# chiy48308/audio_feature_extraction

Hardware: AMD Instinct MI355X
Metric: audio frames/sec (sr=22050, n_fft=1024, hop=256, n_mfcc=13) (higher is better)
Workload: dtype f32; 1 GPU; 1000x10s clips @22050 Hz per GPU, frame_length=1024, hop_length=256, n_mfcc=13, n_mels=128, hamming, pre-emphasis 0.97 + trim 30 dB + RMS (BASELINE configs[1]); clips_per_gpu=1000, frames_per_gpu_step=862000, input=HBM-resident float32

## Files before the change

### audio_feature_extraction_amd/_native.py

```python
from __future__ import annotations

import ctypes as C
import weakref
import os
import threading

import numpy as np

_HERE = os.path.dirname(os.path.abspath(__file__))
LIB_PATH = os.environ.get("AFX_LIB") or os.path.join(_HERE, "libafx.so")

AFX_OK = 0
CLIP_OK, CLIP_TOO_SHORT, CLIP_NONFINITE = 0, 1, 2
WINDOW_HAMMING, WINDOW_HANN = 0, 1
FMT_F32, FMT_S16 = 0, 1
MEM_HOST, MEM_DEVICE = 0, 1
FLAG_PREEMPH, FLAG_TRIM = 1, 2
DTW_OK, DTW_NONFINITE, DTW_NO_PATH = 0, 1, 2
DTW_METRICS = {"euclidean": 0, "sqeuclidean": 1, "cosine": 2}
DTW_BACKTRACK, DTW_STORE_D = 1, 2
DTW_MAX_DIM = 128
HPSS_STORE_SPEC = 4
HPSS_BINS = 1025
CHROMA_STORE_HIST = 8
CHROMA_HIST = 102
SMP_U8, SMP_S16, SMP_S24, SMP_S32, SMP_F32, SMP_F64 = range(6)
SMP_KINDS = {"u8": SMP_U8, "s16": SMP_S16, "s24": SMP_S24, "s32": SMP_S32, "f32": SMP_F32, "f64": SMP_F64}
SMP_BYTES = np.array([1, 2, 3, 4, 4, 8], np.int64)
SMP_OF_WAV = {(1, 8): SMP_U8, (1, 16): SMP_S16, (1, 24): SMP_S24, (1, 32): SMP_S32, (3, 32): SMP_F32, (3, 64): SMP_F64}
DECODE_MAX_CHANNELS = 7
K_NAMES = ("trim_blocks", "trim_decide", "frames", "dct", "stats")
K_FRAMES = 2

SYMBOLS = (
    "afx_version", "afx_device_count", "afx_last_error", "afx_init", "afx_destroy",
    "afx_malloc", "afx_free", "afx_host_alloc", "afx_host_free", "afx_memcpy_h2d", "afx_memcpy_d2h", "afx_synchronize",
    "afx_default_params", "afx_plan_create", "afx_plan_destroy", "afx_build_tables", "afx_build_mel_schedule",
    "afx_extract_batch", "afx_extract_submit", "afx_extract_collect", "afx_f0_batch", "afx_zcr_batch", "afx_spectral_batch", "afx_f0_build_tables", "afx_f0_dispatch", "afx_preprocess", "afx_plan_set_timing", "afx_plan_get_timings", "afx_plan_get_intervals",
    "afx_wav_probe", "afx_wav_read_s16", "afx_batch_geometry", "afx_dtw_batch", "afx_hpss_batch",
    "afx_resample_design", "afx_resample_batch", "afx_rfft_host", "afx_wav_read_raw", "afx_decode_batch",
    "afx_chroma_batch", "afx_chroma_filters",
)


class AfxError(RuntimeError):
    pass


class Params(C.Structure):
    _fields_ = [
        ("sr", C.c_int32), ("n_fft", C.c_int32), ("hop", C.c_int32), ("n_mfcc", C.c_int32),
        ("n_mels", C.c_int32), ("window", C.c_int32), ("preemph", C.c_float),
        ("trim_top_db", C.c_float), ("trim_frame", C.c_int32), ("trim_hop", C.c_int32),
        ("top_db", C.c_float), ("amin", C.c_float), ("delta_width", C.c_int32),
        ("reserved", C.c_int32),
        ("fmin", C.c_float), ("fmax", C.c_float), ("htk", C.c_int32), ("lifter", C.c_float),
    ]


_lib = None
_lock = threading.Lock()


def lib() -> C.CDLL:
    global _lib
    if _lib is not None:
        return _lib
    with _lock:
        if _lib is not None:
            return _lib
        if not os.path.exists(LIB_PATH):
            raise AfxError(
                f"{LIB_PATH} not found: build it with `python -c 'import __graft_entry__ as g; g.build()'` "
                "or `make -C audio_feature_extraction_amd/csrc` (no CPU fallback exists)")
        L = C.CDLL(LIB_PATH)
        vp, i32, i64p, f32p, i32p = C.c_void_p, C.c_int, C.POINTER(C.c_int64), C.POINTER(C.c_float), C.POINTER(C.c_int32)
        L.afx_version.restype = i32
        L.afx_device_count.restype = i32
        L.afx_last_error.restype = C.c_char_p
        L.afx_init.argtypes = [i32, C.POINTER(vp)]
        L.afx_destroy.argtypes = [vp]; L.afx_destroy.restype = None
        L.afx_malloc.argtypes = [vp, C.c_size_t, C.POINTER(vp)]
        L.afx_free.argtypes = [vp, vp]
        L.afx_host_alloc.argtypes = [vp, C.c_size_t, C.POINTER(vp)]
        L.afx_host_free.argtypes = [vp, vp]
        L.afx_memcpy_h2d.argtypes = [vp, vp, vp, C.c_size_t]
        L.afx_memcpy_d2h.argtypes = [vp, vp, vp, C.c_size_t]
        L.afx_synchronize.argtypes = [vp]
        L.afx_default_params.argtypes = [C.POINTER(Params)]; L.afx_default_params.restype = None
        L.afx_plan_create.argtypes = [vp, C.POINTER(Params), C.POINTER(vp)]
        L.afx_plan_destroy.argtypes = [vp]; L.afx_plan_destroy.restype = None
        L.afx_build_tables.argtypes = [C.POINTER(Params), vp, vp, vp]
        L.afx_build_mel_schedule.argtypes = [C.POINTER(Params), vp, vp, vp]
        L.afx_extract_batch.argtypes = [vp, vp, i32, i32, vp, vp, i32, i32, vp, vp, vp, vp, vp, vp]
        L.afx_extract_submit.argtypes = [vp, vp, i32, i32, vp, vp, i32, i32, vp, vp, vp, vp, vp, vp]
        L.afx_extract_collect.argtypes = [vp]
        L.afx_f0_batch.argtypes = [vp, vp, i32, i32, vp, vp, i32, i32, C.c_double, C.c_double, vp, vp, vp, vp]
        L.afx_zcr_batch.argtypes = [vp, vp, i32, i32, vp, vp, i32, i32, vp, vp, vp]
        L.afx_spectral_batch.argtypes = [vp, vp, i32, i32, vp, vp, i32, i32, vp, vp, vp]
        L.afx_f0_build_tables.argtypes = [i32, i32, i32, C.c_double, C.c_double, vp, vp, vp, vp]
        L.afx_f0_dispatch.argtypes = [i32, i32, i32, C.c_double, C.c_double, vp]
        L.afx_preprocess.argtypes = [vp, vp, C.c_int64, vp, i64p, i64p, i32p]
        L.afx_plan_set_timing.argtypes = [vp, i32]
        L.afx_plan_get_timings.argtypes = [vp, vp, vp, i32]
        L.afx_plan_get_intervals.argtypes = [vp, i32, vp, vp, i32, i32p]
        L.afx_batch_geometry.argtypes = [C.POINTER(Params), vp, vp, i32, vp, vp]
        L.afx_wav_probe.argtypes = [vp, i32, i32, vp, vp, vp, vp]
        L.afx_wav_read_s16.argtypes = [vp, i32, i32, vp, vp, vp, C.c_int64, vp, vp]
        L.afx_dtw_batch.argtypes = [vp, vp, i32, vp, vp, vp, vp, vp, i32, i32, i32, vp, vp, vp, vp, vp, vp, vp]
        L.afx_hpss_batch.argtypes = [vp, vp, i32, i32, vp, vp, i32, i32, vp, vp, vp, vp, vp, vp]
        if hasattr(L, "afx_resample_batch"):
            L.afx_resample_design.argtypes = [i32, i32, vp, vp]
            L.afx_resample_batch.argtypes = [vp, vp, i32, i32, vp, vp, i32, i32, i32, vp, i32, vp, i32, vp, vp]
        if hasattr(L, "afx_decode_batch"):
            L.afx_wav_read_raw.argtypes = [vp, i32, i32, vp, vp, vp, C.c_int64, vp, vp]
            L.afx_decode_batch.argtypes = [vp, vp, i32, vp, vp, vp, vp, i32, vp, i32, vp]
        if hasattr(L, "afx_chroma_batch"):
            L.afx_chroma_batch.argtypes = [vp, vp, i32, i32, vp, vp, i32, i32, vp, vp, vp, vp, vp, vp, vp, vp, vp]
            L.afx_chroma_filters.argtypes = [i32, C.c_double, vp]
        if hasattr(L, "afx_rfft_host"):
            L.afx_rfft_host.argtypes = [i32, vp, vp]
        _lib = L
    return _lib


def _path_array(paths):
    arr = (C.c_char_p * len(paths))()
    arr[:] = [os.fsencode(p) for p in paths]
    return arr


def wav_probe(paths, threads: int = 16) -> dict:
    n = len(paths)
    info = np.zeros((n, 4), np.int32)
    frames, off, status = np.zeros(n, np.int64), np.zeros(n, np.int64), np.zeros(n, np.int32)
    if n:
        arr = _path_array(paths)
        _check(lib().afx_wav_probe(arr, n, int(threads), info.ctypes.data, frames.ctypes.data, off.ctypes.data,
                                   status.ctypes.data), "afx_wav_probe")
    return {"tag": info[:, 0], "channels": info[:, 1], "rate": info[:, 2], "bits": info[:, 3],
            "frames": frames, "data_off": off, "status": status}


def wav_read_s16(paths, data_off, frames, out: np.ndarray, offsets, threads: int = 16) -> np.ndarray:
    n = len(paths)
    status = np.zeros(n, np.int32)
    if n:
        if out.dtype != np.int16 or not out.flags.c_contiguous:
            raise ValueError("out must be C-contiguous int16")
        data_off = np.ascontiguousarray(data_off, np.int64)
        frames = np.ascontiguousarray(frames, np.int64)
        offsets = np.ascontiguousarray(offsets, np.int64)
        arr = _path_array(paths)
        _check(lib().afx_wav_read_s16(arr, n, int(threads), data_off.ctypes.data, frames.ctypes.data, out.ctypes.data,
                                      int(out.size), offsets.ctypes.data, status.ctypes.data), "afx_wav_read_s16")
    return status


def wav_read_raw(paths, data_off, nbytes, out: np.ndarray, offsets, threads: int = 16) -> np.ndarray:
    n = len(paths)
    status = np.zeros(n, np.int32)
    if not hasattr(lib(), "afx_wav_read_raw"):
        raise NotImplementedError("this libafx has no afx_wav_read_raw")
    if n:
        if out.dtype != np.uint8 or not out.flags.c_contiguous:
            raise ValueError("out must be C-contiguous uint8")
        data_off = np.ascontiguousarray(data_off, np.int64)
        nbytes = np.ascontiguousarray(nbytes, np.int64)
        offsets = np.ascontiguousarray(offsets, np.int64)
        if not (data_off.shape[0] == nbytes.shape[0] == offsets.shape[0] == n):
            raise ValueError("data_off, nbytes and offsets must have one entry per file")
        arr = _path_array(paths)
        _check(lib().afx_wav_read_raw(arr, n, int(threads), data_off.ctypes.data, nbytes.ctypes.data, out.ctypes.data,
                                      int(out.size), offsets.ctypes.data, status.ctypes.data), "afx_wav_read_raw")
    return status


def wav_sample_kinds(probe: dict) -> np.ndarray:
    kinds = np.full(probe["status"].shape[0], -1, np.int32)
    for (tag, bits), k in SMP_OF_WAV.items():
        kinds[(probe["tag"] == tag) & (probe["bits"] == bits)] = k
    kinds[(probe["status"] != 0) | (probe["channels"] < 1) | (probe["channels"] > DECODE_MAX_CHANNELS) | (probe["rate"] <= 0)] = -1
    return kinds


def batch_geometry(p: "Params", offsets, lengths) -> dict:
    offsets = np.ascontiguousarray(offsets, np.int64)
    lengths = np.ascontiguousarray(lengths, np.int64)
    n = int(offsets.shape[0])
    rec = np.zeros((max(n, 1), 4), np.int64)
    tot = np.zeros(4, np.int64)
    _check(lib().afx_batch_geometry(C.byref(p), offsets.ctypes.data, lengths.ctypes.data, n, rec.ctypes.data, tot.ctypes.data),
           "afx_batch_geometry")
    rec = rec[:n]
    return {"frame_base": rec[:, 0], "tmax": rec[:, 1], "tpad": rec[:, 2], "blk_base": rec[:, 3],
            "frame_slots": int(tot[0]), "blocks": int(tot[1]), "trim_blocks": int(tot[2]), "max_tmax": int(tot[3])}


def f0_build_tables(sr: int, n_fft: int, hop: int, fmin: float, fmax: float) -> dict:
    info = np.zeros(8, np.int32)
    _check(lib().afx_f0_build_tables(sr, n_fft, hop, fmin, fmax, info.ctypes.data, None, None, None), "afx_f0_build_tables")
    band, nb = int(info[3]), int(info[2])
    w = 2 * band + 1
    beta, lt, freqs = np.zeros(100), np.zeros(2 * w * w), np.zeros(nb)
    _check(lib().afx_f0_build_tables(sr, n_fft, hop, fmin, fmax, info.ctypes.data, beta.ctypes.data, lt.ctypes.data,
                                     freqs.ctypes.data), "afx_f0_build_tables")
    keys = ("min_period", "max_period", "n_bins", "band", "cap", "n_lag", "R", "slots")
    return {**{k: int(v) for k, v in zip(keys, info)}, "beta": beta, "lt": lt.reshape(2, w, w), "freqs": freqs}


F0_DISPATCH_KEYS = ("energy_lpw", "epb", "yin_n", "yin_fpb", "yin_sh", "vit_nbt", "vit_bandt", "vit_tpt", "bt_depth",
                    "band", "n_bins", "yin_lds")


def f0_dispatch(sr: int, n_fft: int, hop: int, fmin: float, fmax: float) -> dict:
    out = np.zeros(len(F0_DISPATCH_KEYS), np.int32)
    _check(lib().afx_f0_dispatch(int(sr), int(n_fft), int(hop), float(fmin), float(fmax), out.ctypes.data), "afx_f0_dispatch")
    return {k: int(v) for k, v in zip(F0_DISPATCH_KEYS, out)}


def resample_design(sr_in: int, sr_out: int) -> dict:
    info = np.zeros(4, np.int32)
    _check(lib().afx_resample_design(int(sr_in), int(sr_out), info.ctypes.data, None), "afx_resample_design")
    taps = np.zeros(int(info[2]), np.float64)
    _check(lib().afx_resample_design(int(sr_in), int(sr_out), info.ctypes.data, taps.ctypes.data), "afx_resample_design")
    return {"up": int(info[0]), "down": int(info[1]), "n_taps": int(info[2]), "half": int(info[3]), "taps": taps}


def rfft_host(x) -> np.ndarray:
    x = np.ascontiguousarray(x, np.float32).reshape(-1)
    out = np.zeros(2 * (x.size // 2 + 1), np.float32)
    _check(lib().afx_rfft_host(int(x.size), x.ctypes.data, out.ctypes.data), "afx_rfft_host")
    return out.view(np.complex64)


def chroma_filters(sr: int, tuning: float = 0.0) -> np.ndarray:
    if not hasattr(lib(), "afx_chroma_filters"):
        raise NotImplementedError("this libafx has no afx_chroma_filters")
    out = np.zeros((12, HPSS_BINS), np.float32)
    _check(lib().afx_chroma_filters(int(sr), float(tuning), out.ctypes.data), "afx_chroma_filters")
    return out


def resample_lengths(lengths, sr_in: int, sr_out: int) -> np.ndarray:
    sr_in = np.asarray(sr_in, np.int64)
    g = np.gcd(sr_in, int(sr_out))
    up, down = int(sr_out) // g, sr_in // g
    return (np.asarray(lengths, np.int64) * up + down - 1) // down


def _check(rc: int, what: str):
    if rc != AFX_OK:
        msg = lib().afx_last_error().decode("utf-8", "replace")
        if rc == -5:
            raise NotImplementedError(f"{what}: {msg}")
        if rc == -1:
            raise ValueError(f"{what}: {msg}")
        raise AfxError(f"{what} failed ({rc}): {msg}")


def device_count() -> int:
    return int(lib().afx_device_count())


def _ptr(a):
    return None if a is None else a.ctypes.data


def packed_offsets(counts, align: int = 1) -> np.ndarray:
    counts = np.asarray(counts, np.int64).reshape(-1)
    if align > 1:
        counts = (counts + (align - 1)) // align * align
    out = np.zeros(counts.shape[0], np.int64)
    if counts.shape[0] > 1:
        np.cumsum(counts[:-1], out=out[1:])
    return out


def _clip_arrays(offsets, lengths):
    offsets = np.ascontiguousarray(offsets, np.int64).reshape(-1)
    lengths = np.ascontiguousarray(lengths, np.int64).reshape(-1)
    n = int(offsets.shape[0])
    if lengths.shape[0] != n:
        raise ValueError("offsets and lengths must have one entry per clip")
    return offsets, lengths, n


def _sample_fmt(samples, fmt):
    if fmt is not None:
        return fmt
    if isinstance(samples, np.ndarray):
        return FMT_S16 if samples.dtype == np.int16 else FMT_F32
    raise ValueError("fmt is required for device-resident samples")


def _sample_source(samples, fmt, offsets, lengths, mem=None):
    if mem is None:
        mem = MEM_HOST if isinstance(samples, np.ndarray) else MEM_DEVICE
    if mem != MEM_HOST:
        return (samples.ptr if isinstance(samples, DeviceBuffer) else int(samples)), MEM_DEVICE
    want = np.int16 if fmt == FMT_S16 else np.float32
# ... 449 lines not shown
```

### audio_feature_extraction_amd/csrc/afx_api.cpp

```cpp
#include <algorithm>
#include <cmath>
#include <cstdio>
#include <cstdlib>
#include <cstring>
#include <atomic>
#include <mutex>
#include <string>
#include <vector>

#include <hip/hip_runtime.h>

#include "afx_device.h"
#include "afx_devenv.h"
#include "afx_frames3.h"
#include "afx_internal.h"
#include "afx_plan.h"

namespace afx {
DevEnv::DevEnv() {
  if (const char* v = getenv("AFX_DEBUG_SKIP")) debug_skip = atoi(v) & 127;
  if (const char* v = getenv("AFX_F0_DEBUG")) f0_debug = atoi(v);
  stamps = getenv("AFX_DEBUG_STAMPS") != nullptr;
  f3_debug = getenv("AFX_F3_DEBUG") != nullptr;
  no_spec = getenv("AFX_NO_SPEC") != nullptr;
  no_tickets = getenv("AFX_NO_TICKETS") != nullptr;
  no_frames3 = getenv("AFX_NO_FRAMES3") != nullptr;
  no_frames3s = getenv("AFX_NO_FRAMES3S") != nullptr;
  no_frames3d = getenv("AFX_NO_FRAMES3D") != nullptr;
  f3_generic_mel = getenv("AFX_F3_GENERIC_MEL") != nullptr;
  no_dct16l = getenv("AFX_NO_DCT16L") != nullptr;
  host_blocks = getenv("AFX_HOST_BLOCKS") != nullptr;
  no_fused_tail = getenv("AFX_NO_FUSED_TAIL") != nullptr;
  if (const char* v = getenv("AFX_F3_WAVES")) f3_waves = atoi(v);
  if (const char* v = getenv("AFX_TAIL_MODE")) tail_mode = atoi(v);
  if (const char* v = getenv("AFX_TAIL_SKIP")) tail_skip = atoi(v) & 7;
  if (const char* v = getenv("AFX_TEST_CHUNK_CLIPS")) chunk_clips = std::max(1, std::min(32768, atoi(v)));
  if (const char* v = getenv("AFX_TEST_F0_CHUNK_FRAMES")) f0_chunk_frames = std::max<int64_t>(64, atoll(v));
  if (const char* v = getenv("AFX_TEST_DTW_BUDGET")) dtw_budget = std::max<int64_t>(1, atoll(v));
  if (const char* v = getenv("AFX_TEST_HPSS_BUDGET")) hpss_budget = std::max<int64_t>(1, atoll(v));
  if (const char* v = getenv("AFX_TEST_CHROMA_BUDGET")) chroma_budget = std::max<int64_t>(1, atoll(v));
  f0_dump = getenv("AFX_F0_DUMP");
}
const DevEnv& dev_env() { static const DevEnv e; return e; }
}

extern "C" int afx_device_count(void) {
  int n = 0;
  if (hipGetDeviceCount(&n) != hipSuccess) return 0;
  return n;
}

extern "C" int afx_init(int device, afx_ctx** out) {
  if (!out) { set_error("afx_init: null out"); return AFX_ERR_INVALID; }
  *out = nullptr;
  int n = afx_device_count();
  if (n <= 0) { set_error("no HIP device visible"); return AFX_ERR_NO_DEVICE; }
  if (device < 0 || device >= n) { set_error("device index out of range"); return AFX_ERR_INVALID; }
  HIP_TRY(hipSetDevice(device));
  afx_ctx* c = new afx_ctx();
  c->device = device;
  hipError_t e = hipStreamCreateWithFlags(&c->stream, hipStreamNonBlocking);
  if (e != hipSuccess) { delete c; set_error(std::string("hipStreamCreate: ") + hipGetErrorString(e)); return AFX_ERR_HIP; }
  *out = c;
  return AFX_OK;
}

extern "C" void afx_destroy(afx_ctx* ctx) {
  if (!ctx) return;
  (void)hipSetDevice(ctx->device);
  for (DevBuf* b : {&ctx->dtw_raw, &ctx->dtw_feats, &ctx->dtw_norms, &ctx->dtw_pairs, &ctx->dtw_codes, &ctx->dtw_rows, &ctx->dtw_d,
                    &ctx->dtw_path, &ctx->dtw_cost, &ctx->dtw_status, &ctx->dtw_len, &ctx->rs_g, &ctx->rs_tstart, &ctx->rs_clips,
                    &ctx->rs_in, &ctx->rs_out, &ctx->dc_clips, &ctx->dc_in, &ctx->dc_out})
    release(*b);
  if (ctx->stream) (void)hipStreamDestroy(ctx->stream);
  delete ctx;
}

extern "C" int afx_malloc(afx_ctx* ctx, size_t bytes, void** out) {
  if (!ctx || !out) { set_error("afx_malloc: null argument"); return AFX_ERR_INVALID; }
  HIP_TRY(hipSetDevice(ctx->device));
  hipError_t e = hipMalloc(out, bytes ? bytes : 1);
  if (e != hipSuccess) { set_error(std::string("hipMalloc: ") + hipGetErrorString(e)); return e == hipErrorOutOfMemory ? AFX_ERR_NOMEM : AFX_ERR_HIP; }
  return AFX_OK;
}

extern "C" int afx_free(afx_ctx* ctx, void* d) {
  if (!ctx) { set_error("afx_free: null ctx"); return AFX_ERR_INVALID; }
  HIP_TRY(hipSetDevice(ctx->device));
  if (d) HIP_TRY(hipFree(d));
  return AFX_OK;
}

extern "C" int afx_host_alloc(afx_ctx* ctx, size_t bytes, void** out) {
  if (!ctx || !out) { set_error("afx_host_alloc: null argument"); return AFX_ERR_INVALID; }
  *out = nullptr;
  HIP_TRY(hipSetDevice(ctx->device));
  hipError_t e = hipHostMalloc(out, bytes ? bytes : 1, hipHostMallocPortable);
  if (e != hipSuccess) { set_error(std::string("hipHostMalloc: ") + hipGetErrorString(e)); *out = nullptr; return e == hipErrorOutOfMemory ? AFX_ERR_NOMEM : AFX_ERR_HIP; }
  return AFX_OK;
}

extern "C" int afx_host_free(afx_ctx* ctx, void* h) {
  if (!ctx) { set_error("afx_host_free: null ctx"); return AFX_ERR_INVALID; }
  HIP_TRY(hipSetDevice(ctx->device));
  if (h) HIP_TRY(hipHostFree(h));
  return AFX_OK;
}

extern "C" int afx_memcpy_h2d(afx_ctx* ctx, void* dst, const void* src, size_t bytes) {
  if (!ctx || (!dst && bytes) || (!src && bytes)) { set_error("afx_memcpy_h2d: null argument"); return AFX_ERR_INVALID; }
  HIP_TRY(hipSetDevice(ctx->device));
  HIP_TRY(hipMemcpyAsync(dst, src, bytes, hipMemcpyHostToDevice, ctx->stream));
  HIP_TRY(hipStreamSynchronize(ctx->stream));
  return AFX_OK;
}

// ... 148 lines not shown

static int device_ref(afx_plan* pl, hipEvent_t* out) {
  std::lock_guard<std::mutex> lk(g_ref_mu);
  const int d = pl->device;
  if (d < 0 || d >= 64) { set_error("device index out of range for timing"); return AFX_ERR_INVALID; }
  if (!g_ref_set[d]) {
    HIP_TRY(hipEventCreate(&g_ref[d]));
    HIP_TRY(hipEventRecord(g_ref[d], pl->ctx->stream));
    HIP_TRY(hipEventSynchronize(g_ref[d]));
    g_ref_set[d] = true;
  }
  *out = g_ref[d];
  return AFX_OK;
}

extern "C" int afx_plan_set_timing(afx_plan* pl, int enable) {
  if (!pl) { set_error("afx_plan_set_timing: null plan"); return AFX_ERR_INVALID; }
  HIP_TRY(hipSetDevice(pl->device));
  if (enable) { hipEvent_t r; int rc = device_ref(pl, &r); if (rc != AFX_OK) return rc; }
  if (enable && !pl->ev_ready) {
    for (int k = 0; k < AFX_K_COUNT; ++k) { HIP_TRY(hipEventCreate(&pl->ev[k][0])); HIP_TRY(hipEventCreate(&pl->ev[k][1])); }
    pl->ev_ready = true;
  }
  pl->timing = enable != 0;
  pl->timing_frames_only = enable == 2;
  return AFX_OK;
}

extern "C" int afx_plan_get_timings(afx_plan* pl, float* ms, int32_t* launches, int reset) {
  if (!pl) { set_error("afx_plan_get_timings: null plan"); return AFX_ERR_INVALID; }
  for (int k = 0; k < AFX_K_COUNT; ++k) {
    if (ms) ms[k] = (float)pl->ms_sum[k];
    if (launches) launches[k] = pl->launches[k];
    if (reset) { pl->ms_sum[k] = 0.0; pl->launches[k] = 0; pl->spans[k].clear(); }
  }
  return AFX_OK;
}

extern "C" int afx_plan_get_intervals(afx_plan* pl, int slot, double* start_ms, double* end_ms, int cap, int32_t* count) {
  if (!pl || slot < 0 || slot >= AFX_K_COUNT || cap < 0 || !count) { set_error("afx_plan_get_intervals: invalid argument"); return AFX_ERR_INVALID; }
  const auto& v = pl->spans[slot];
  const int n = (int)std::min<size_t>(v.size(), (size_t)cap);
  for (int i = 0; i < n; ++i) {
    if (start_ms) start_ms[i] = v[v.size() - n + i].first;
    if (end_ms) end_ms[i] = v[v.size() - n + i].second;
  }
  *count = (int32_t)v.size();
  return AFX_OK;
}

int prepare_descriptors(afx_plan* pl, const int64_t* offsets, const int64_t* lengths, int n) {
  const bool same = (int)pl->c_len.size() == n &&
                    std::memcmp(pl->c_len.data(), lengths, n * sizeof(int64_t)) == 0 &&
                    std::memcmp(pl->c_off.data(), offsets, n * sizeof(int64_t)) == 0;
  if (same) return AFX_OK;
  const int hop = pl->p.hop, th = pl->p.trim_hop;
  pl->h_clips.resize(n);
  BatchGeom g;
  {
    std::string why;
    if (!build_clip_descs(hop, th, offsets, lengths, n, pl->h_clips.data(), g, why)) { set_error(why); return AFX_ERR_INVALID; }
  }
  const int64_t nblk = g.nblocks;
  pl->total_tpad = g.total_tpad; pl->total_tblk = g.total_tblk; pl->max_tblocks = g.max_tblocks; pl->max_tmax = g.max_tmax;
  pl->nblocks = g.nblocks;
  int rc;
  if ((rc = ensure(pl->clips, n * sizeof(ClipDesc))) != AFX_OK) return rc;
  if ((rc = ensure(pl->blocks, std::max<size_t>((size_t)nblk, 1) * sizeof(BlockDesc))) != AFX_OK) return rc;
  hipStream_t s = pl->ctx->stream;
  if (pl->clips_ev_pending) { HIP_TRY(hipEventSynchronize(pl->clips_ev)); pl->clips_ev_pending = false; }
  if (pl->h_clips_pin_cap < (size_t)n) {
    if (pl->h_clips_pin) (void)hipHostFree(pl->h_clips_pin);
    pl->h_clips_pin = nullptr; pl->h_clips_pin_cap = 0;
    const size_t want = (size_t)n + (size_t)n / 4 + 64;
    HIP_TRY(hipHostMalloc((void**)&pl->h_clips_pin, want * sizeof(ClipDesc), hipHostMallocDefault));
    pl->h_clips_pin_cap = want;
  }
  if (!pl->clips_ev) HIP_TRY(hipEventCreateWithFlags(&pl->clips_ev, hipEventDisableTiming));
  std::memcpy(pl->h_clips_pin, pl->h_clips.data(), (size_t)n * sizeof(ClipDesc));
  HIP_TRY(hipMemcpyAsync(pl->clips.p, pl->h_clips_pin, n * sizeof(ClipDesc), hipMemcpyHostToDevice, s));
  HIP_TRY(hipEventRecord(pl->clips_ev, s));
  pl->clips_ev_pending = true;
  if (pl->use_f3) {
    const size_t nb_alloc = (size_t)std::max<int64_t>(nblk, 1);
    if ((rc = ensure(pl->blocks_spec, nb_alloc * sizeof(BlockDesc))) != AFX_OK) return rc;
    if ((rc = ensure(pl->blockmax, nb_alloc * sizeof(float))) != AFX_OK) return rc;
    if ((rc = ensure(pl->items, (size_t)n * kF3ItemsPerClip * sizeof(BlockDesc))) != AFX_OK) return rc;
    if ((rc = ensure(pl->n_items, 16)) != AFX_OK) return rc;
    if (!dev_env().host_blocks) {
      HIP_TRY(launch_build_blocks3(s, (const ClipDesc*)pl->clips.p, n, (int)nblk, (BlockDesc*)pl->blocks_spec.p, pl->kp));
    } else {
      const int per = pl->kp.rms_sub, half = pl->p.n_fft / 2;
      pl->h_blocks.resize(nb_alloc);
      for (int i = 0; i < n; ++i) {
        const ClipDesc& c = pl->h_clips[i];
        const int64_t ntb = (c.len + th - 1) / th;
        for (int b = 0; b < c.tpad / kFramesPerBlock; ++b) {
          const int64_t gs = (int64_t)b * kFramesPerBlock * hop - half;
          const int t0 = b * kFramesPerBlock;
          pl->h_blocks[(size_t)c.blk_base + b] = make_block(c, i, gs, t0, 0, c.len, c.len, t0, c.tmax, c.len >= 2 && t0 < c.tmax,
                                                            (int32_t)(c.tblk_base * per), (int32_t)(ntb * per));
        }
      }
      HIP_TRY(hipMemcpyAsync(pl->blocks_spec.p, pl->h_blocks.data(), pl->h_blocks.size() * sizeof(BlockDesc), hipMemcpyHostToDevice, s));
      HIP_TRY(hipStreamSynchronize(s));
    }
  }
  pl->c_off.assign(offsets, offsets + n);
  pl->c_len.assign(lengths, lengths + n);
  return AFX_OK;
}

int null_arg(const char* who) {
  set_error(std::string(who) + ": null/invalid argument");
  return AFX_ERR_INVALID;
}

int check_sample_format(const char* who, int sample_fmt, int mem_kind) {
  if (sample_fmt != AFX_FMT_F32 && sample_fmt != AFX_FMT_S16) { set_error(std::string(who) + ": unknown sample format"); return AFX_ERR_INVALID; }
  if (mem_kind != AFX_MEM_HOST && mem_kind != AFX_MEM_DEVICE) { set_error(std::string(who) + ": unknown mem_kind"); return AFX_ERR_INVALID; }
  return AFX_OK;
}

int check_batch_args(const char* who, afx_plan* pl, const void* samples, int sample_fmt, int mem_kind,
                     const int64_t* offsets, const int64_t* lengths, int n_clips, bool empty_ok) {
  const bool need = n_clips > 0 || !empty_ok;
  if (!pl || n_clips < 0 || (need && (!offsets || !lengths)) || (!samples && n_clips > 0)) return null_arg(who);
  return check_sample_format(who, sample_fmt, mem_kind);
}

int check_clip_ranges(const char* who, const int64_t* offsets, const int64_t* lengths, const int64_t* out_offsets, int n_clips,
                      int64_t max_off) {
  for (int i = 0; i < n_clips; ++i) {
    if (offsets[i] < 0 || lengths[i] < 0 || offsets[i] > max_off || (out_offsets && (out_offsets[i] < 0 || out_offsets[i] > max_off))) {
      set_error(std::string(who) + ": clip " + std::to_string(i) + ": offsets and lengths must be >= 0");
      return AFX_ERR_INVALID;
    }
    if (lengths[i] > ((int64_t)1 << 31)) {
      set_error(std::string(who) + ": clip " + std::to_string(i) + ": more than 2^31 samples is not supported");
      return AFX_ERR_UNSUPPORTED;
    }
  }
  return AFX_OK;
}

int begin_plan_call(const char* who, afx_plan* pl) {
  (void)hipGetLastError();
  HIP_TRY(hipSetDevice(pl->device));
  if (pl->pend.active) { set_error(std::string(who) + ": the plan has a submitted batch that has not been collected"); return AFX_ERR_INVALID; }
  return AFX_OK;
}

int stage_samples(afx_plan* pl, DevBuf& buf, const void* samples, int sample_fmt, int mem_kind, const int64_t* offsets,
                  const int64_t* lengths, int n, const void** d_samples) {
  *d_samples = samples;
  if (mem_kind != AFX_MEM_HOST) return AFX_OK;
  const size_t esz = sample_fmt == AFX_FMT_S16 ? 2 : 4;
  int64_t hi = 0;
  for (int i = 0; i < n; ++i) hi = std::max(hi, offsets[i] + lengths[i]);
  int rc;
  if ((rc = ensure(buf, (size_t)hi * esz + 16)) != AFX_OK) return rc;
  if (hi > 0) HIP_TRY(hipMemcpyAsync(buf.p, samples, (size_t)hi * esz, hipMemcpyHostToDevice, pl->ctx->stream));
  *d_samples = buf.p;
  return AFX_OK;
}

int run_preprocess(afx_plan* pl, const void* d_samples, int n, const KParams& kp, bool f0_prep) {
  hipStream_t s = pl->ctx->stream;
  int64_t hi = 0, max_len = 0;
  for (int i = 0; i < n; ++i) { hi = std::max(hi, pl->c_off[i] + pl->c_len[i]); max_len = std::max(max_len, pl->c_len[i]); }
  int rc;
  if ((rc = ensure(pl->info, n * sizeof(ClipInfo))) != AFX_OK) return rc;
  if ((rc = ensure(pl->bsum, std::max<int64_t>(pl->total_tblk, 1) * 4 * sizeof(float))) != AFX_OK) return rc;
  if (f0_prep && (rc = ensure(pl->f0_ysig, (size_t)std::max<int64_t>(hi, 1) * sizeof(float))) != AFX_OK) return rc;
  const ClipDesc* d_clips = (const ClipDesc*)pl->clips.p;
  ClipInfo* d_info = (ClipInfo*)pl->info.p;
  HIP_TRY(hipMemsetAsync(d_info, 0, n * sizeof(ClipInfo), s));
  pl->info_clean_n = 0;
  HIP_TRY(launch_trim_blocks(s, d_samples, d_clips, d_info, (float*)pl->bsum.p, n, pl->max_tblocks, kp));
  HIP_TRY(launch_trim_decide(s, d_clips, d_info, (const float*)pl->bsum.p, (BlockDesc*)pl->blocks.p, nullptr, n, kp));
  if (f0_prep) HIP_TRY(launch_f0_prep(s, d_samples, d_clips, d_info, (float*)pl->f0_ysig.p, n, max_len, kp));
  return AFX_OK;
}

int rebase_offsets(const afx_plan* pl, const char* what, const int64_t* offs, int n, int64_t per_frame,
                   std::vector<int64_t>& rebased, int64_t* lo, int64_t* hi) {
// ... 8 lines not shown
  return AFX_OK;
}

int upload_frame_range(afx_plan* pl, const int64_t* rebased, int n, DevBuf& d_offs, DevBuf& out, size_t bytes, int fill) {
  hipStream_t s = pl->ctx->stream;
  int rc;
  if ((rc = ensure(out, bytes)) != AFX_OK) return rc;
  if ((rc = ensure(d_offs, n * sizeof(int64_t))) != AFX_OK) return rc;
  HIP_TRY(hipMemcpyAsync(d_offs.p, rebased, n * sizeof(int64_t), hipMemcpyHostToDevice, s));
  HIP_TRY(hipMemsetAsync(out.p, fill, bytes, s));
  return AFX_OK;
}

int run_spectral(afx_plan* pl, const void* d_signal, int n, const KParams& kp, const int64_t* h_offsets, size_t count,
                 const SpecBands& sb) {
  hipStream_t s = pl->ctx->stream;
  int rc;
  if ((rc = ensure(pl->info, n * sizeof(ClipInfo))) != AFX_OK) return rc;
  if ((rc = upload_frame_range(pl, h_offsets, n, pl->frame_offs, pl->frames, count * sizeof(float), 0)) != AFX_OK) return rc;
  HIP_TRY(hipMemsetAsync(pl->info.p, 0, n * sizeof(ClipInfo), s));
  pl->info_clean_n = 0;
  if (pl->nblocks > 0)
    HIP_TRY(launch_spectral(s, d_signal, (ClipInfo*)pl->info.p, (const BlockDesc*)pl->blocks_spec.p, pl->nblocks, pl->f3, kp,
                            (float*)pl->frames.p, (const int64_t*)pl->frame_offs.p, sb, pl->n_cu));
  return AFX_OK;
}

int statuses_from_info(afx_plan* pl, int n, int32_t* out_status) {
  hipStream_t s = pl->ctx->stream;
  std::vector<ClipInfo> h_info(n);
  HIP_TRY(hipMemcpyAsync(h_info.data(), pl->info.p, n * sizeof(ClipInfo), hipMemcpyDeviceToHost, s));
  HIP_TRY(hipStreamSynchronize(s));
  for (int i = 0; i < n; ++i) out_status[i] = h_info[i].nonfinite ? AFX_CLIP_NONFINITE : AFX_CLIP_OK;
  return AFX_OK;
}

#define TIMED(slot, call)                                                      \
  do {                                                                         \
    const bool timed_ = pl->timing && (!pl->timing_frames_only || (slot) == AFX_K_FRAMES);   \
    if (timed_) HIP_TRY(hipEventRecord(pl->ev[slot][0], s));                   \
    HIP_TRY(call);                                                             \
    if (timed_) { HIP_TRY(hipEventRecord(pl->ev[slot][1], s)); pl->launches[slot]++; } \
  } while (0)

static int chunk_enqueue(afx_plan* pl, const void* samples, int fmt, int mem_kind,
                         const int64_t* offsets, const int64_t* lengths, int n, int flags,
                         float* out_stats, int32_t* out_status, int64_t* out_trim, int32_t* out_nframes,
                         float* out_frames, const int64_t* frame_offsets, bool by_event) {
  hipStream_t s = pl->ctx->stream;
  if (pl->pend.active) { set_error("the plan has a submitted batch that has not been collected (afx_extract_collect)"); return AFX_ERR_INVALID; }
  const int K = pl->p.n_mfcc, M = pl->p.n_mels;
  const int nstat = 4 * K + 3;
  int rc;
  if ((rc = prepare_descriptors(pl, offsets, lengths, n)) != AFX_OK) return rc;

  const void* d_samples = nullptr;
  if ((rc = stage_samples(pl, pl->samples, samples, fmt, mem_kind, offsets, lengths, n, &d_samples)) != AFX_OK) return rc;
  {
    const size_t before = pl->info.cap;
    if ((rc = ensure(pl->info, n * sizeof(ClipInfo))) != AFX_OK) return rc;
    if (pl->info.cap != before) pl->info_clean_n = 0;
  }
  if ((rc = ensure(pl->bsum, std::max<int64_t>(pl->total_tblk, 1) * 4 * sizeof(float))) != AFX_OK) return rc;
  if ((rc = ensure(pl->logmel, (size_t)(pl->total_tpad + kFramesPerBlock) * M * sizeof(float))) != AFX_OK) return rc;
  if ((rc = ensure(pl->rms, (size_t)pl->total_tpad * sizeof(float))) != AFX_OK) return rc;
  if ((rc = ensure(pl->mfcc, (size_t)pl->total_tpad * K * sizeof(float))) != AFX_OK) return rc;
  float* d_frames = nullptr;
  int64_t f_lo = 0, f_hi = 0;
  if (out_frames) {
    if (!frame_offsets) { set_error("out_frames given without frame_offsets"); return AFX_ERR_INVALID; }
    if ((rc = rebase_offsets(pl, "frame", frame_offsets, n, 3 * K + 1, pl->h_rebased, &f_lo, &f_hi)) != AFX_OK) return rc;
    if ((rc = upload_frame_range(pl, pl->h_rebased.data(), n, pl->frame_offs, pl->frames, (size_t)(f_hi - f_lo) * sizeof(float), 0)) != AFX_OK) return rc;
    d_frames = (float*)pl->frames.p;
  }

  KParams kp = pl->kp;
  kp.flags = flags; kp.fmt = fmt;
  kp.flags |= dev_env().debug_skip << 8;
  const ClipDesc* d_clips = (const ClipDesc*)pl->clips.p;
  ClipInfo* d_info = (ClipInfo*)pl->info.p;

  {
    const size_t before = pl->n_items.cap;
    if ((rc = ensure(pl->n_items, 16)) != AFX_OK) return rc;
    if (pl->n_items.cap != before) pl->info_clean_n = 0;
  }
  if (pl->info_clean_n < n) {
    HIP_TRY(hipMemsetAsync(d_info, 0, n * sizeof(ClipInfo), s));
    HIP_TRY(hipMemsetAsync(pl->n_items.p, 0, 16, s));
  }
  pl->info_clean_n = 0;
  const bool want_stamps = dev_env().stamps && !frames_mr_shape(kp.n_fft);
  const bool f3 = pl->use_f3 && !want_stamps && (!(kp.flags & 0x7f00) || dev_env().f3_debug);
  bool no_spec = dev_env().no_spec;
  if (f3 && no_spec && kp.rms_sub > 1 && kp.trim_hop / kp.rms_sub != 256) no_spec = false;
  if (!f3) kp.rms_sub = 0;
  const bool fused_tail = f3 && pl->nblocks > 0 && !out_frames && !dev_env().no_fused_tail && tail_eligible(kp, pl->dt) &&
                          (n >= 32 || pl->max_tmax <= 2048);
  const F3Launch f3l{s, d_samples, d_info, pl->f3, kp, (float*)pl->logmel.p, pl->n_cu};
  if (f3 && !no_spec && pl->nblocks > 0) {
    const int max_items = n * kF3ItemsPerClip;
    F3Launch spec = f3l;
    spec.blocks = (const BlockDesc*)pl->blocks_spec.p; spec.nblocks = pl->nblocks; spec.spec = true;
    spec.blockmax = (float*)pl->blockmax.p; spec.bsum = (float*)pl->bsum.p;
    spec.work_ctr = dev_env().no_tickets ? nullptr : (int*)pl->n_items.p + 1;
    TIMED(AFX_K_FRAMES, launch_frames3_any(spec));
    TIMED(AFX_K_TRIM_DECIDE, launch_trim_decide3(s, d_clips, d_info, (const float*)pl->bsum.p, (const float*)pl->blockmax.p,
                                                 (BlockDesc*)pl->items.p, (int*)pl->n_items.p, max_items, (float*)pl->rms.p, n, kp));
    F3Launch redo = f3l;
    redo.blocks = (const BlockDesc*)pl->items.p; redo.nblocks = max_items; redo.nblocks_dev = (const int*)pl->n_items.p;
    TIMED(AFX_K_TRIM_BLOCKS, launch_frames3_any(redo));
    if (!fused_tail)
      TIMED(AFX_K_DCT, launch_dct(s, d_clips, d_info, pl->dt, kp, (const float*)pl->logmel.p, (float*)pl->mfcc.p, n, pl->max_tmax, true, true));
  } else {
  TIMED(AFX_K_TRIM_BLOCKS, launch_trim_blocks(s, d_samples, d_clips, d_info, (float*)pl->bsum.p, n, pl->max_tblocks, kp));
  TIMED(AFX_K_TRIM_DECIDE, launch_trim_decide(s, d_clips, d_info, (const float*)pl->bsum.p, (BlockDesc*)pl->blocks.p, (float*)pl->rms.p, n, kp, d_samples));
  if (pl->nblocks > 0) {
    const int grid = std::min(pl->nblocks, pl->n_cu * 2);
    unsigned long long* d_stamps = nullptr;
    if (want_stamps) {
      if ((rc = ensure(pl->stamps, (size_t)grid * kWaves * kStampPhases * 8)) != AFX_OK) return rc;
      d_stamps = (unsigned long long*)pl->stamps.p;
      HIP_TRY(hipMemsetAsync(d_stamps, 0, (size_t)grid * kWaves * kStampPhases * 8, s));
    }
    if (f3) {
      F3Launch all = f3l;
      all.blocks = (const BlockDesc*)pl->blocks.p; all.nblocks = pl->nblocks;
      TIMED(AFX_K_FRAMES, launch_frames3_any(all));
    }
    else if (frames_mr_shape(kp.n_fft))
      TIMED(AFX_K_FRAMES, launch_frames_mr(s, d_samples, d_info, (const BlockDesc*)pl->blocks.p, pl->nblocks,
                                           pl->dt, kp, (float*)pl->logmel.p, (float*)pl->rms.p, grid));
    else
      TIMED(AFX_K_FRAMES, launch_frames(s, d_samples, d_info, (const BlockDesc*)pl->blocks.p, pl->nblocks,
                                        pl->dt, kp, (float*)pl->logmel.p, (float*)pl->rms.p, grid, d_stamps));
    if (want_stamps) {
      std::vector<unsigned long long> h((size_t)grid * kWaves * kStampPhases);
      HIP_TRY(hipMemcpyAsync(h.data(), d_stamps, h.size() * 8, hipMemcpyDeviceToHost, s));
      HIP_TRY(hipStreamSynchronize(s));
      static const char* names[kStampPhases] = {"stage", "bar1", "fft", "prefetch", "bar2", "mel", "bar3", "melfin", "x0", "x1", "x2", "x3"};
      double tot[kStampPhases] = {}, wv[kWaves][kStampPhases] = {};
      for (int g = 0; g < grid; ++g)
        for (int w = 0; w < kWaves; ++w)
          for (int ph = 0; ph < kStampPhases; ++ph) {
            const double v = (double)h[((size_t)g * kWaves + w) * kStampPhases + ph];
            tot[ph] += v; wv[w][ph] += v;
          }
      const double per = (double)pl->nblocks * kWaves;
      fprintf(stderr, "[afx stamps] cycles per block (avg over waves):");
      double all = 0;
      for (int ph = 0; ph < kStampPhases; ++ph) { fprintf(stderr, " %s=%.0f", names[ph], tot[ph] / per); all += tot[ph] / per; }
      fprintf(stderr, " total=%.0f\n", all);
      for (int w = 0; w < kWaves; ++w) {
        fprintf(stderr, "[afx stamps]   wave %d:", w);
        for (int ph = 0; ph < kStampPhases; ++ph) fprintf(stderr, " %s=%.0f", names[ph], wv[w][ph] / pl->nblocks);
        fprintf(stderr, "\n");
      }
    }
    if (!fused_tail)
      TIMED(AFX_K_DCT, launch_dct(s, d_clips, d_info, pl->dt, kp, (const float*)pl->logmel.p, (float*)pl->mfcc.p, n, pl->max_tmax, f3));
  }
  }
  const int tail_spec = (f3 && !no_spec) ? 1 : 0;
  const size_t stats_bytes = (size_t)n * nstat * sizeof(float), info_bytes = (size_t)n * sizeof(ClipInfo);
  if (pl->h_pin_cap < stats_bytes + info_bytes) {
    HIP_TRY(hipStreamSynchronize(s));
    if (pl->h_pin) (void)hipHostFree(pl->h_pin);
    pl->h_pin = nullptr; pl->h_pin_cap = 0; pl->h_pin_dev = nullptr;
    const size_t want = (stats_bytes + info_bytes) * 5 / 4 + 256;
    HIP_TRY(hipHostMalloc(&pl->h_pin, want, hipHostMallocMapped));
    HIP_TRY(hipHostGetDevicePointer(&pl->h_pin_dev, pl->h_pin, 0));
    pl->h_pin_cap = want;
  }
  const size_t info_at = (stats_bytes + 15) & ~(size_t)15;
  if (fused_tail)
    TIMED(AFX_K_DCT, launch_tail(s, d_clips, d_info, pl->dt, kp, (const float*)pl->logmel.p, (const float*)pl->rms.p,
                                 (float*)pl->h_pin_dev, (ClipInfo*)((char*)pl->h_pin_dev + info_at), n, tail_spec, pl->n_cu));
  else
  TIMED(AFX_K_STATS, launch_stats(s, d_clips, d_info, kp, (const float*)pl->mfcc.p, (const float*)pl->rms.p,
                                  (float*)pl->h_pin_dev, d_frames, (const int64_t*)pl->frame_offs.p, n,
                                  (ClipInfo*)((char*)pl->h_pin_dev + info_at)));
  if (out_frames && f_hi > f_lo)
    HIP_TRY(hipMemcpyAsync(out_frames + f_lo, d_frames, (size_t)(f_hi - f_lo) * sizeof(float), hipMemcpyDeviceToHost, s));
  if (by_event) {
    if (!pl->done) HIP_TRY(hipEventCreateWithFlags(&pl->done, hipEventDisableTiming));
    if (!pl->flag) {
      void* h = nullptr;
      HIP_TRY(hipHostMalloc(&h, 64, hipHostMallocMapped));
      std::memset(h, 0, 64);
      pl->flag = (volatile unsigned*)h;
      HIP_TRY(hipHostGetDevicePointer((void**)&pl->flag_dev, h, 0));
    }
  }
  HIP_TRY(launch_finish(s, d_info, n, (int*)pl->n_items.p, by_event ? pl->flag_dev : nullptr, by_event ? ++pl->seq : 0u));
  pl->info_clean_n = n;
  if (by_event) HIP_TRY(hipEventRecord(pl->done, s));
  pl->pend.active = true; pl->pend.n = n; pl->pend.stats_bytes = stats_bytes;
  pl->pend.out_stats = out_stats; pl->pend.out_status = out_status; pl->pend.out_trim = out_trim; pl->pend.out_nframes = out_nframes;
  return AFX_OK;
}

static int chunk_finish(afx_plan* pl, bool by_event) {
  if (!pl->pend.active) { set_error("afx_extract_collect: nothing submitted"); return AFX_ERR_INVALID; }
  hipStream_t s = pl->ctx->stream;
  pl->pend.active = false;
  if (by_event) {
    for (unsigned it = 1; *pl->flag != pl->seq; ++it) {
      if ((it & 0xfff) == 0) {
        const hipError_t q = hipEventQuery(pl->done);
        if (q == hipSuccess) break;
        if (q != hipErrorNotReady) { set_error(std::string("afx_extract_collect: ") + hipGetErrorString(q)); return AFX_ERR_HIP; }
      }
#if defined(__x86_64__)
      __builtin_ia32_pause();
#endif
    }
    std::atomic_thread_fence(std::memory_order_acquire);
  } else {
    HIP_TRY(hipStreamSynchronize(s));
  }
  const int n = pl->pend.n;
  const size_t stats_bytes = pl->pend.stats_bytes;
  float* out_stats = pl->pend.out_stats; int32_t* out_status = pl->pend.out_status;
  int64_t* out_trim = pl->pend.out_trim; int32_t* out_nframes = pl->pend.out_nframes;
  const float* h_stats = (const float*)pl->h_pin;
  const ClipInfo* h_info = (const ClipInfo*)((char*)pl->h_pin + ((stats_bytes + 15) & ~(size_t)15));
  if (pl->timing) {
    for (int k = 0; k < AFX_K_COUNT; ++k) {
      if (pl->nblocks == 0 && (k == AFX_K_FRAMES || k == AFX_K_DCT)) continue;
      if (pl->launches[k] == 0) continue;
      float ms = 0.f, t0 = 0.f;
      if (hipEventElapsedTime(&ms, pl->ev[k][0], pl->ev[k][1]) == hipSuccess) {
        pl->ms_sum[k] += ms;
        hipEvent_t ref;
        if (device_ref(pl, &ref) == AFX_OK && hipEventElapsedTime(&t0, ref, pl->ev[k][0]) == hipSuccess) {
          if (pl->spans[k].size() >= kMaxSpans) pl->spans[k].erase(pl->spans[k].begin(), pl->spans[k].begin() + kMaxSpans / 2);
          pl->spans[k].emplace_back((double)t0, (double)t0 + (double)ms);
        }
      }
    }
  }
  std::memcpy(out_stats, h_stats, stats_bytes);
  for (int i = 0; i < n; ++i) {
    const ClipInfo& ci = h_info[i];
    out_status[i] = ci.status;
    if (out_trim) { out_trim[2 * i] = ci.start; out_trim[2 * i + 1] = ci.end; }
    if (out_nframes) out_nframes[i] = ci.T;
  }
  return AFX_OK;
}

static int extract_chunk(afx_plan* pl, const void* samples, int fmt, int mem_kind,
                         const int64_t* offsets, const int64_t* lengths, int n, int flags,
                         float* out_stats, int32_t* out_status, int64_t* out_trim, int32_t* out_nframes,
                         float* out_frames, const int64_t* frame_offsets) {
  int rc = chunk_enqueue(pl, samples, fmt, mem_kind, offsets, lengths, n, flags, out_stats, out_status, out_trim, out_nframes,
                         out_frames, frame_offsets, false);
  if (rc != AFX_OK) return rc;
  return chunk_finish(pl, false);
}

extern "C" int afx_extract_submit(afx_plan* pl, const void* samples, int sample_fmt, int mem_kind,
                                  const int64_t* offsets, const int64_t* lengths, int n_clips, int flags,
                                  float* out_stats, int32_t* out_status, int64_t* out_trim,
                                  int32_t* out_nframes, float* out_frames, const int64_t* frame_offsets) {
  if (!out_stats || !out_status) return null_arg("afx_extract_submit");
  int rc = check_batch_args("afx_extract_submit", pl, samples, sample_fmt, mem_kind, offsets, lengths, n_clips);
  if (rc != AFX_OK) return rc;
  if (n_clips == 0) { set_error("afx_extract_submit: empty batch"); return AFX_ERR_INVALID; }
  if (n_clips > dev_env().chunk_clips) { set_error("afx_extract_submit: more clips than one chunk holds; use afx_extract_batch"); return AFX_ERR_UNSUPPORTED; }
  if (pl->pend.active) { set_error("afx_extract_submit: the plan's previous batch has not been collected"); return AFX_ERR_INVALID; }
  (void)hipGetLastError();
  HIP_TRY(hipSetDevice(pl->device));
  rc = chunk_enqueue(pl, samples, sample_fmt, mem_kind, offsets, lengths, n_clips, flags, out_stats, out_status, out_trim,
                     out_nframes, out_frames, frame_offsets, true);
  return rc;
}
// ... 31 lines not shown
```

### audio_feature_extraction_amd/csrc/afx_devenv.h

```cpp
#pragma once
#include <cstdint>

namespace afx {

struct DevEnv {
  int debug_skip = 0, f0_debug = 0;
  bool stamps = false, f3_debug = false, no_spec = false, no_tickets = false;
  bool no_frames3 = false, no_frames3s = false, no_frames3d = false;
  bool f3_generic_mel = false;
  bool no_dct16l = false;
  bool host_blocks = false;
  bool no_fused_tail = false;
  int tail_mode = 0;
  int tail_skip = 0;
  int f3_waves = 0;
  int chunk_clips = 32768;
  int64_t f0_chunk_frames = 1280 * 1024;
  int64_t dtw_budget = (int64_t)2 << 30;
  int64_t hpss_budget = (int64_t)2 << 30;
  int64_t chroma_budget = (int64_t)2 << 30;
  const char* f0_dump = nullptr;
  DevEnv();
};
const DevEnv& dev_env();

}
```

### audio_feature_extraction_amd/csrc/afx_device.h

```cpp
#pragma once
#include <cstddef>
#include <cstdint>

#include <hip/hip_runtime_api.h>

#include "afx.h"
#include "afx_consts.h"

namespace afx {

constexpr int kFramesPerBlock = 16;
constexpr int kWaves = 4;

struct ClipDesc {
  int64_t off;
  int64_t len;
  int64_t frame_base;
  int64_t tblk_base;
  int32_t tmax;
  int32_t tpad;
  int32_t blk_base;
  int32_t pad_;
};

// ... 13 lines not shown
__host__ __device__ inline BlockDesc make_block(const ClipDesc& cd, int clip, int64_t gs, int64_t frame, int64_t start,
                                                int64_t end, int64_t N, int t0, int T, bool active, int32_t bsum_base,
                                                int32_t bsum_n) {
  const int64_t lim = (int64_t)1 << 30;
  auto rel = [&](int64_t x) { const int64_t r = x - gs; return (int32_t)(r < -lim ? -lim : (r > lim ? lim : r)); };
  BlockDesc d;
  d.sample_base = cd.off + gs; d.frame_slot = cd.frame_base + frame; d.clip_off = cd.off;
  d.keep_lo = rel(start); d.keep_hi = rel(end);
  d.have_lo = rel(0); d.have_hi = rel(N);
  d.clip = clip; d.t0 = t0; d.T = T;
  d.active = active ? 1 : 0;
  d.bsum_base = bsum_base; d.bsum_n = bsum_n;
  return d;
}

struct ClipInfo {
  int64_t start, end;
  int32_t T;
  int32_t status;
  uint32_t lmax_ord;
  uint32_t nonfinite;
};

struct DevTables {
  const float* window;
  const float* tw;
  const float* post;
  const float4* mel_coef;
  const float* mel_koff;
  const int4* mel_grp;
  const int4* mel_items;
  int32_t mel_item_cnt[4];
  int32_t mel_n_slots;
  const float* dctA;
  const float* dctP;
  const float* dctS;
  int32_t n_groups;
  int32_t n_cgroups;
};

struct KParams {
  int32_t n_fft, hop, n_mels, n_mfcc;
  int32_t trim_frame, trim_hop;
  float preemph_b1;
  float trim_top_db, top_db, amin;
  int32_t flags;
  int32_t fmt;
  int32_t rms_sub;
};

template <typename K>
inline hipError_t set_lds_limit(K kernel, size_t bytes) {
  return hipFuncSetAttribute(reinterpret_cast<const void*>(kernel), hipFuncAttributeMaxDynamicSharedMemorySize, (int)bytes);
}
template <auto Kernel>
inline hipError_t allow_lds_once() {
  static bool done[64] = {};
  int dev = 0;
  hipError_t e = hipGetDevice(&dev);
  if (e != hipSuccess) return e;
  if (dev < 0 || dev >= 64 || done[dev]) return hipSuccess;
  if ((e = set_lds_limit(Kernel, 160 * 1024)) == hipSuccess) done[dev] = true;
  return e;
}

size_t frames_lds_bytes(int n_fft, int hop);

hipError_t launch_trim_blocks(hipStream_t s, const void* samples, const ClipDesc* clips, ClipInfo* info,
                              float* bsum, int n_clips, int max_tblocks, const KParams& kp);
hipError_t launch_trim_decide(hipStream_t s, const ClipDesc* clips, ClipInfo* info, const float* bsum,
                              BlockDesc* blocks, float* rms_rows, int n_clips, const KParams& kp,
                              const void* samples = nullptr);
hipError_t launch_frames(hipStream_t s, const void* samples, ClipInfo* info,
                         const BlockDesc* blocks, int nblocks, const DevTables& tb, const KParams& kp,
                         float* logmel, float* rms_rows, int grid, unsigned long long* stamps = nullptr);
constexpr int kStampPhases = 12;
bool frames_mr_shape(int n_fft);
size_t frames_mr_lds_bytes(int n_fft, int hop);
hipError_t launch_frames_mr(hipStream_t s, const void* samples, ClipInfo* info, const BlockDesc* blocks, int nblocks,
                            const DevTables& tb, const KParams& kp, float* logmel, float* rms_rows, int grid);
hipError_t launch_dct(hipStream_t s, const ClipDesc* clips, const ClipInfo* info, const DevTables& tb,
                      const KParams& kp, const float* logmel, float* mfcc, int n_clips, int max_tmax,
                      bool frame_major = false, bool spec = false);
hipError_t launch_finish(hipStream_t s, ClipInfo* info, int n_clips, int* counters, unsigned* flag_dev, unsigned seq);
hipError_t launch_stats(hipStream_t s, const ClipDesc* clips, const ClipInfo* info, const KParams& kp,
                        const float* mfcc, const float* rms_rows, float* stats, float* frames_out,
                        const int64_t* frame_offsets, int n_clips, ClipInfo* info_out = nullptr);
hipError_t launch_preemph(hipStream_t s, const float* y, float* out, int64_t n, float b1);
bool tail_eligible(const KParams& kp, const DevTables& tb);
hipError_t launch_tail(hipStream_t s, const ClipDesc* clips, const ClipInfo* info, const DevTables& tb, const KParams& kp,
                       const float* logmel, const float* rms_rows, float* stats, ClipInfo* info_out, int n_clips, int spec,
                       int n_cu);

}
```

### audio_feature_extraction_amd/csrc/afx_frames3.h

```cpp
#pragma once
#include <cstdint>
#include <vector>

#include <hip/hip_runtime_api.h>

#include "afx_device.h"

namespace afx {

constexpr int kF3ExFloats = 2176;
constexpr int kF3TabFloats = 2048;
constexpr int kF3MaxRounds = 8;
constexpr int kF3KernelRounds = 4;
constexpr int kF3MaxBatches = 8;

struct HostF3Mel {
  int32_t rounds = 0;
  int32_t nb[kF3MaxRounds] = {};
  int32_t width[kF3MaxRounds] = {};
  int32_t woff[kF3MaxRounds] = {};
  std::vector<float> w;
  std::vector<int32_t> meta;
  bool usable = false;
};

struct F3Tables {
  const float* window;
  const float* w1024;
  const float* w2048;
  const float* mel_w;
  const int32_t* mel_meta;
  int32_t mel_rounds;
  int32_t mel_wfloats;
  int32_t mel_all_own;
  int32_t mel_own_w1;
  uint32_t mel_rp[kF3MaxRounds];
};

void build_f3_mel(const std::vector<float>& mel_dense, int n_mels, int n_bins, int max_slot, int lanes, int align, HostF3Mel& out);

size_t frames3_lds_bytes(int waves, const F3Tables& ft);
bool frames3_eligible(const KParams& kp, const F3Tables& ft);
int frames3_waves(const F3Tables& ft);
struct F3Launch {
  hipStream_t s;
  const void* samples;
  ClipInfo* info;
  const F3Tables& ft;
  const KParams& kp;
  float* logmel;
  int n_cu;
  const BlockDesc* blocks = nullptr;
  int nblocks = 0;
  const int* nblocks_dev = nullptr;
  float* blockmax = nullptr;
  float* bsum = nullptr;
  bool spec = false;
  int* work_ctr = nullptr;
};
inline int f3_grid(const F3Launch& L, int waves) {
  const int want = (L.nblocks + waves - 1) / waves;
  return want < 1 ? 1 : (want < L.n_cu ? want : L.n_cu);
}
size_t frames3s_lds_bytes(int waves, const F3Tables& ft);
size_t frames3d_lds_bytes(int waves, const F3Tables& ft);
hipError_t launch_frames3(const F3Launch& L);
hipError_t launch_frames3s(const F3Launch& L);
hipError_t launch_frames3d(const F3Launch& L);
hipError_t launch_frames3_any(const F3Launch& L);
struct SpecBands {
  int32_t lo[8], hi[8], cnt[8];
  float hz_per_bin, roll_percent;
};
constexpr int kSpecFloats = 17;
hipError_t launch_spectral(hipStream_t s, const void* samples, ClipInfo* info, const BlockDesc* blocks, int nblocks,
                           const F3Tables& ft, const KParams& kp, float* desc_out, const int64_t* desc_offs,
                           const SpecBands& sb, int n_cu);
hipError_t launch_build_blocks3(hipStream_t s, const ClipDesc* clips, int n_clips, int nblocks, BlockDesc* blocks,
                                const KParams& kp);
constexpr int kF3ItemsPerClip = 6;
hipError_t launch_trim_decide3(hipStream_t s, const ClipDesc* clips, ClipInfo* info, const float* bsum, const float* blockmax,
                               BlockDesc* items, int* n_items, int max_items, float* rms_rows, int n_clips, const KParams& kp);

}
```

### audio_feature_extraction_amd/csrc/afx_frames3.hip

```cpp
#include <hip/hip_runtime.h>

#include <cstdlib>
#include <type_traits>

#include "afx_device.h"
#include "afx_devenv.h"
#include "afx_frames3.h"
#include "afx_frames3_dev.h"

namespace afx {

size_t frames3_lds_bytes(int waves, const F3Tables& ft) {
  return (size_t)(waves * kF3ExFloats + kF3TabFloats + ft.mel_wfloats + ft.mel_rounds * 64 + 1024) * sizeof(float);
}

#ifdef AFX_F3_DEBUG
__device__ unsigned long long g_f3_stamps[4 * 8192];
__device__ unsigned long long g_f3_blk[65536];
#endif

template <int FMT, int WAVES, int NB0, int NB1, bool SPEC>
__global__ __launch_bounds__(WAVES * 64) void k_frames3(const void* __restrict__ samples,
                                                        ClipInfo* __restrict__ info,
                                                        const BlockDesc* __restrict__ blocks, int nblocks,
                                                        const int* __restrict__ nblocks_dev,
                                                        F3Tables ft, KParams kp,
                                                        float* __restrict__ logmel,
                                                        float* __restrict__ blockmax,
                                                        float* __restrict__ bsum,
                                                        int* __restrict__ work_ctr) {
  constexpr int N = 1024, HOP = 256;
  extern __shared__ __attribute__((aligned(16))) float smem[];
  if (nblocks_dev) {
    nblocks = *nblocks_dev;
    if (nblocks <= 0) return;
  }
  const int tid = threadIdx.x, lane = tid & 63;
  const int wave = __builtin_amdgcn_readfirstlane(tid >> 6);
#ifdef AFX_F3_DEBUG
  const unsigned long long stamp0 = wall_clock64();
#endif
  float* const tabs = smem + WAVES * kF3ExFloats;
  float4* const T2q = reinterpret_cast<float4*>(tabs);
  float4* const T3q = reinterpret_cast<float4*>(tabs + 256);
  const int mel_wfloats = NB0 > 0 ? (NB0 + NB1) * 256 : ft.mel_wfloats;
  const int mel_rounds = NB0 > 0 ? 2 : ft.mel_rounds;
  float* const MW = tabs + kF3TabFloats;
  int* const MM = reinterpret_cast<int*>(MW + mel_wfloats);
  v2* const E = reinterpret_cast<v2*>(smem + wave * kF3ExFloats);
  float* const XB = reinterpret_cast<float*>(E);

  {
    const v2* w1024 = reinterpret_cast<const v2*>(ft.w1024);
    auto W = [&](int m) { const v2 v = w1024[m & 511]; return (m & 512) ? -v : v; };
    if (tid < 64) {
      const int rr = tid >> 4, c = tid & 15;
      const v2 a = W(8 * (2 * rr) * c), b = W(8 * (2 * rr + 1) * c);
      T2q[tid] = float4{a.x, a.y, b.x, b.y};
      const int jbt = tid ? 128 - tid : 64;
#pragma unroll
      for (int r = 1; r < 8; ++r) { const v2 ta = W(tid * r), tb = W(jbt * r); T3q[(r - 1) * 64 + tid] = float4{ta.x, ta.y, tb.x, tb.y}; }
    }
    for (int i = tid; i < mel_wfloats; i += WAVES * 64) MW[i] = ft.mel_w[i];
    for (int i = tid; i < mel_rounds * 64; i += WAVES * 64) MM[i] = ft.mel_meta[i];
    for (int i = lane; i < kF3ExFloats; i += 64) XB[i] = 0.f;
  }
  float4* const WT = reinterpret_cast<float4*>(MM + mel_rounds * 64);
  if (tid < 64) {
    float wreg[16];
#pragma unroll
    for (int u = 0; u < 16; ++u) wreg[u] = 0.5f * ft.window[u < 8 ? lane + 64 * u : (64 - lane) + 64 * (15 - u)];
#pragma unroll
    for (int v = 0; v < 4; ++v) WT[v * 64 + lane] = float4{wreg[4 * v], wreg[4 * v + 1], wreg[4 * v + 2], wreg[4 * v + 3]};
  }
  __syncthreads();
  const v2 H = {0.70710678118654752440f, 0.70710678118654752440f};
  const v2 W1 = {0.92387953251128675613f, -0.38268343236508977173f};
  const v2 W3 = {0.38268343236508977173f, -0.92387953251128675613f};
  const bool pre = (kp.flags & AFX_FLAG_PREEMPH) != 0;
  const float b1 = pre ? kp.preemph_b1 : 0.f;
  const int M = kp.n_mels;
  const int jb = lane ? 128 - lane : 64;
  v2* const e1w = E + lane;
  const v2* const e1r = E + 66 * (lane & 15) + (lane >> 4);
  v2* const e2w = E + 128 * (lane >> 4) + (lane & 15);
  v2* const ea = E + lane;
  v2* const eb = E + jb;

  using sample_t = sample_of<FMT>;
  const int n_rounds = mel_rounds;
  const int meta0 = MM[lane], meta1 = MM[64 + lane];
  const unsigned mf0 = (meta0 >> 11) & 511, mf1 = (meta1 >> 11) & 511;
  const float amin = kp.amin;

  float bs = 0.f;
  unsigned long long bsmask = 0;
  auto sub2 = [&](float x, float y, int idx, unsigned long long two) -> bool {
    const float m = f3_sum2(x, y);
    const unsigned long long sel = two << idx;
    bs = f3_sel(bs, m, sel);
    bsmask |= sel;
    return __any(!(fabsf(m) < INFINITY));
  };
  auto flag_nonfinite = [&](const BlockDesc& bd, bool bad_rows) {
    if (__any(bad_rows) && lane == 0) atomicOr(&info[bd.clip].nonfinite, 1u);
  };
  auto sub_store = [&](const BlockDesc& bd) {
    const int j = bd.t0 + lane;
    if (((bsmask >> lane) & 1) && j < bd.bsum_n) bsum[bd.bsum_base + j] = bs;
    bsmask = 0;
  };

  const int total_waves = gridDim.x * WAVES, wg = blockIdx.x * WAVES + wave;
#ifdef AFX_F3_DEBUG
  const unsigned long long stamp1 = wall_clock64();
#endif
  F3Runs runs = f3_runs_init(work_ctr, nblocks, total_waves, wg, true);
  do {
  const int b_hi = runs.b_hi;
  for (int b = runs.b_lo; b < b_hi; ++b) {
    BlockDesc bd = blocks[b];
    if (!bd.active) continue;
    bool first = true;
    v2 Ra[8], Rb[8];
    for (;;) {
    const int Tleft = bd.T - bd.t0;
    const int npairs = Tleft >= 16 ? 8 : (Tleft + 1) >> 1;
    bool chain = false;
    if (SPEC && npairs == 8 && b + 1 < b_hi) {
      const BlockDesc* nx = blocks + b + 1;
      chain = nx->active && nx->clip == bd.clip && nx->t0 == bd.t0 + 16;
    }
    const int64_t sbase = bd.sample_base;
    const sample_t* const sp = (const sample_t*)samples + sbase;
    auto interior = [&](int j0, int j1) -> bool {
      return (j0 - 1 >= bd.have_lo) && (j1 <= bd.have_hi) && (j0 >= bd.keep_lo) && (j1 <= bd.keep_hi);
    };
    auto interior_r = [&](int j0, int j1) -> bool {
      const BlockDesc& r = blocks[f3_opaque(b)];
      return (j0 - 1 >= r.have_lo) && (j1 <= r.have_hi) && (j0 >= r.keep_lo) && (j1 <= r.keep_hi);
    };
    auto edge_sample = [&](int j) -> float {
      const BlockDesc& bd = blocks[f3_opaque(b)];
      const int lo = bd.have_lo, hi = bd.have_hi - 1;
      const int jc = j < lo ? lo : (j > hi ? hi : j), jp = (j - 1) < lo ? lo : ((j - 1) > hi ? hi : (j - 1));
      const float y = (jc == j) ? ld_raw<FMT>(samples, sbase + jc) : 0.f;
      const float yp = (jp == j - 1) ? ld_raw<FMT>(samples, sbase + jp) : 0.f;
      float v = y;
      if (pre) {
        v = preemph1(y, yp, b1);
        if (j == lo) v = preemph0(ld_raw<FMT>(samples, bd.clip_off), ld_raw<FMT>(samples, bd.clip_off + 1));
      }
      return (j >= bd.keep_lo && j < bd.keep_hi) ? v : 0.f;
    };

    if (first) {
      float rows[20];
      if (interior(0, N + HOP)) {
        float y[20], yp[20];
#pragma unroll
        for (int u = 0; u < 20; ++u) { y[u] = ld_row<FMT>(sp, 64 * u + lane); yp[u] = ld_row<FMT>(sp - 1, 64 * u + lane); }
#pragma unroll
        for (int u = 0; u < 20; ++u) rows[u] = preemph1(y[u], yp[u], b1);
      } else {
#pragma unroll 1
        for (int u = 0; u < 20; ++u) XB[64 * u + lane] = edge_sample(64 * u + lane);
#pragma unroll
        for (int u = 0; u < 20; ++u) rows[u] = XB[64 * u + lane];
      }
#pragma unroll
      for (int u = 0; u < 8; ++u) { Ra[u] = v2{rows[u], rows[u + 4]}; Rb[u] = v2{rows[u + 8], rows[u + 12]}; }
      if constexpr (SPEC) {
        auto sq4 = [&](int r) { float q = rows[r] * rows[r]; q = fmaf(rows[r + 1], rows[r + 1], q); q = fmaf(rows[r + 2], rows[r + 2], q); return fmaf(rows[r + 3], rows[r + 3], q); };
        auto bad4 = [&](int r) { return !(isfinite(rows[r]) && isfinite(rows[r + 1]) && isfinite(rows[r + 2]) && isfinite(rows[r + 3])); };
        if (sub2(sq4(12), sq4(16), 1, 3ull)) flag_nonfinite(bd, bad4(12) || bad4(16));
        if (bd.t0 == 0 && sub2(0.f, sq4(8), 0, 1ull)) flag_nonfinite(bd, bad4(8));
      }
    }
    float lmax = -INFINITY;
    float* const tile = logmel + bd.frame_slot * (int64_t)M;
    const bool blk_int = interior(0, 512 * 8 + 768 + 512);

    auto pair_body = [&](v2 (&P)[8], v2 (&Q)[8], const int p) __attribute__((always_inline)) {
      v2 z[16];
#pragma unroll
      for (int v = 0; v < 4; ++v) {
        const float4 w = ldv4(WT + v * 64 + lane);
        const v2* const src = v < 2 ? P + 4 * v : Q + 4 * (v - 2);
        z[4 * v] = src[0] * v2{w.x, w.x}; z[4 * v + 1] = src[1] * v2{w.y, w.y};
        z[4 * v + 2] = src[2] * v2{w.z, w.z}; z[4 * v + 3] = src[3] * v2{w.w, w.w};
      }
      const bool more = p + 1 < npairs || chain;
      const int jn = 512 * (p + 1) + 768;
      const bool nint = more && (blk_int || interior_r(jn, jn + 512));

      f3_dft16(z, H, W1, W3);
      if (!F3_SKIP(0x200)) {
#pragma unroll
      for (int k = 0; k < 16; ++k) stv(e1w + 66 * k, z[k]);
#pragma unroll
// ... 107 lines not shown
        }
        }
      } else {
#pragma unroll 1
      for (int rd = 0; rd < (F3_SKIP(0x400) ? 0 : n_rounds); ++rd) {
        const uint32_t rp = ft.mel_rp[rd];
        const int meta = MM[rd * 64 + lane];
        const float4* pp = reinterpret_cast<const float4*>(E + (meta & 2047));
        const float4* ww = reinterpret_cast<const float4*>(MW + (rp >> 8)) + lane;
        const int nb = rp & 15, wd = (rp >> 4) & 15;
        v2 a0 = {0.f, 0.f}, a1 = {0.f, 0.f};
#define F3_BATCH(i)                                                                  \
        if (nb > (i)) {                                                              \
          const float4 c = ww[64 * (i)];                                             \
          const float4 q0 = pp[2 * (i)], q1 = pp[2 * (i) + 1];                       \
          a0 = v2{q0.x, q0.y} * v2{c.x, c.x} + a0; a1 = v2{q0.z, q0.w} * v2{c.y, c.y} + a1; \
          a0 = v2{q1.x, q1.y} * v2{c.z, c.z} + a0; a1 = v2{q1.z, q1.w} * v2{c.w, c.w} + a1; \
        }
        F3_BATCH(0) F3_BATCH(1) F3_BATCH(2) F3_BATCH(3) F3_BATCH(4) F3_BATCH(5) F3_BATCH(6) F3_BATCH(7)
#undef F3_BATCH
        v2 acc = a0 + a1;
        if (wd >= 2) { acc.x += AFX_DPP_F(acc.x, 0xB1, false); acc.y += AFX_DPP_F(acc.y, 0xB1, false); }
        if (wd >= 4) { acc.x += AFX_DPP_F(acc.x, 0x4E, false); acc.y += AFX_DPP_F(acc.y, 0x4E, false); }
        if (wd >= 8) { acc.x += AFX_DPP_F(acc.x, 0x141, false); acc.y += AFX_DPP_F(acc.y, 0x141, false); }
        const float L0 = 3.01029995663981195f * __builtin_amdgcn_logf(f3_max(acc.x, amin));
        const float L1 = 3.01029995663981195f * __builtin_amdgcn_logf(f3_max(acc.y, amin));
        if (meta & (1 << 20)) {
          const unsigned m = (meta >> 11) & 511;
          if (vA) rowA[m] = L0;
          if (vB) rowA[M + m] = L1;
          if (vA) lmax = f3_max(lmax, L0);
          if (vB) lmax = f3_max(lmax, L1);
        }
      }
      }

      __builtin_amdgcn_s_setprio(0);
      if (more) {
        float n[8];
        if (nint) {
#pragma unroll
          for (int u = 0; u < 8; ++u) n[u] = preemph1(ny[u], nyp[u], b1);
        } else {
          const int jn_e = f3_opaque(jn);
#pragma unroll 1
          for (int u = 0; u < 8; ++u) XB[64 * u + lane] = edge_sample(jn_e + 64 * u + lane);
#pragma unroll
          for (int u = 0; u < 8; ++u) n[u] = XB[64 * u + lane];
        }
#pragma unroll
        for (int i = 0; i < 4; ++i) { P[i] = v2{Q[4 + i].y, n[i]}; P[4 + i] = v2{n[i], n[4 + i]}; }
        if constexpr (SPEC) {
          v2 q = P[4] * P[4]; q = P[5] * P[5] + q; q = P[6] * P[6] + q; q = P[7] * P[7] + q;
          if (sub2(q.x, q.y, 2 * p + 3, 3ull)) {
            bool bad = false;
#pragma unroll
            for (int u = 0; u < 8; ++u) bad |= !isfinite(n[u]);
            flag_nonfinite(blocks[f3_opaque(b)], bad);
          }
        }
      }
    };

#pragma unroll 1
    for (int p = 0; p < npairs; p += 2) {
      pair_body(Ra, Rb, p);
      if (p + 1 < npairs) pair_body(Rb, Ra, p + 1);
    }
    {
      const float mx = f3_wave_max(lmax);
      const BlockDesc& be = blocks[f3_opaque(b)];
      if constexpr (SPEC) { if (lane == 0) blockmax[b] = mx; sub_store(be); }
      else { if (lane == 0 && mx > -INFINITY) atomicMax(&info[be.clip].lmax_ord, f2ord(mx)); }
    }
#ifdef AFX_F3_DEBUG
    if (SPEC && lane == 0 && b < 65536) g_f3_blk[b] = wall_clock64();
#endif
    if (!chain) break;
    first = false;
    ++b;
    bd = blocks[b];
    }
  }
  } while (f3_runs_next(runs, work_ctr, nblocks, (int)(gridDim.x * WAVES), lane));
#ifdef AFX_F3_DEBUG
  if (SPEC && lane == 0 && wg < 8192) {
    g_f3_stamps[4 * wg] = stamp0; g_f3_stamps[4 * wg + 1] = stamp1; g_f3_stamps[4 * wg + 2] = wall_clock64();
    g_f3_stamps[4 * wg + 3] = (unsigned long long)__builtin_amdgcn_s_getreg((31 << 11) | 4) |
                              ((unsigned long long)__builtin_amdgcn_s_getreg((31 << 11) | 20) << 32);
  }
#endif
}

#ifdef AFX_F3_DEBUG
extern "C" __attribute__((visibility("default"))) int afx_debug_f3_stamps(unsigned long long* out, int n_waves) {
  return (int)hipMemcpyFromSymbol(out, HIP_SYMBOL(g_f3_stamps), sizeof(unsigned long long) * 4 * (size_t)n_waves);
}
extern "C" __attribute__((visibility("default"))) int afx_debug_f3_blocks(unsigned long long* out, int n_blocks) {
  return (int)hipMemcpyFromSymbol(out, HIP_SYMBOL(g_f3_blk), sizeof(unsigned long long) * (size_t)n_blocks);
}
#endif

bool frames3_eligible(const KParams& kp, const F3Tables& ft) {
  const int per = kp.hop > 0 ? kp.trim_hop / kp.hop : 0;
  if (!(ft.mel_rounds > 0 && kp.n_mels <= 512 && kp.hop > 0 && kp.trim_hop % kp.hop == 0 && per >= 1 && per <= 4) ||
      dev_env().no_frames3)
    return false;
  if (kp.n_fft == 1024 && kp.hop == 256) return frames3_lds_bytes(12, ft) <= 160 * 1024;
  if (kp.n_fft == 2048 && kp.hop == 512) return frames3s_lds_bytes(12, ft) <= 160 * 1024 && !dev_env().no_frames3s;
  if (kp.n_fft == 512 && kp.hop == 128) return frames3d_lds_bytes(12, ft) <= 160 * 1024 && !dev_env().no_frames3d;
  return false;
}

hipError_t launch_frames3_any(const F3Launch& L) {
  if (L.kp.n_fft == 2048) return launch_frames3s(L);
  if (L.kp.n_fft == 512) return launch_frames3d(L);
  return launch_frames3(L);
}

int frames3_waves(const F3Tables& ft) {
  const int forced = dev_env().f3_waves;
  if (forced == 12 || forced == 16) return frames3_lds_bytes(forced, ft) <= 160 * 1024 ? forced : 12;
  return frames3_lds_bytes(16, ft) <= 160 * 1024 ? 16 : 12;
}

template <int FMT, int WAVES, int NB0, int NB1, bool SPEC>
static hipError_t launch_frames3_t(const F3Launch& L) {
  const hipError_t e = allow_lds_once<k_frames3<FMT, WAVES, NB0, NB1, SPEC>>();
  if (e != hipSuccess) return e;
  hipLaunchKernelGGL((k_frames3<FMT, WAVES, NB0, NB1, SPEC>), dim3(f3_grid(L, WAVES)), dim3(WAVES * 64), frames3_lds_bytes(WAVES, L.ft), L.s,
                     L.samples, L.info, L.blocks, L.nblocks, L.nblocks_dev, L.ft, L.kp, L.logmel, L.blockmax, L.bsum, L.work_ctr);
  return hipGetLastError();
}

template <int FMT, int WAVES, bool SPEC>
static hipError_t launch_frames3_w(const F3Launch& L) {
  const F3Tables& ft = L.ft;
  const bool two = ft.mel_rounds == 2 && ((ft.mel_rp[0] >> 4) & 15) == 1 && ((ft.mel_rp[1] >> 4) & 15) == 1 && ft.mel_all_own &&
                   ft.mel_wfloats == (int)((ft.mel_rp[0] & 15) + (ft.mel_rp[1] & 15)) * 256 && (ft.mel_rp[1] >> 8) == (ft.mel_rp[0] & 15) * 256 &&
                   !dev_env().f3_generic_mel;
  const int nb0 = ft.mel_rp[0] & 15, nb1 = ft.mel_rp[1] & 15;
  if (two && nb0 == 2 && nb1 == 7)
    return launch_frames3_t<FMT, WAVES, 2, 7, SPEC>(L);
  return launch_frames3_t<FMT, WAVES, 0, 0, SPEC>(L);
}

hipError_t launch_frames3(const F3Launch& L) {
  const int waves = frames3_waves(L.ft);
#define AFX_F3_GO(FMT, W) (L.spec ? launch_frames3_w<FMT, W, true>(L) : launch_frames3_w<FMT, W, false>(L))
  if (L.kp.fmt == AFX_FMT_S16) return waves == 16 ? AFX_F3_GO(AFX_FMT_S16, 16) : AFX_F3_GO(AFX_FMT_S16, 12);
  return waves == 16 ? AFX_F3_GO(AFX_FMT_F32, 16) : AFX_F3_GO(AFX_FMT_F32, 12);
#undef AFX_F3_GO
}

}
```

### audio_feature_extraction_amd/csrc/afx_frames3_dev.h

```cpp
#pragma once
#include <hip/hip_runtime.h>

#include <cstdint>

#include "afx_device.h"
#include "afx_frames3.h"
#include "afx_wave.h"

namespace afx {

typedef float v2 __attribute__((ext_vector_type(2)));

__device__ __forceinline__ v2 add_mi(v2 a, v2 b) {
  v2 d; asm("v_pk_add_f32 %0, %1, %2 op_sel:[0,1] op_sel_hi:[1,0] neg_hi:[0,1]" : "=v"(d) : "v"(a), "v"(b)); return d;
}
__device__ __forceinline__ v2 add_pi(v2 a, v2 b) {
  v2 d; asm("v_pk_add_f32 %0, %1, %2 op_sel:[0,1] op_sel_hi:[1,0] neg_lo:[0,1]" : "=v"(d) : "v"(a), "v"(b)); return d;
}
__device__ __forceinline__ v2 cmul(v2 v, v2 w) {
  v2 t, d;
  asm("v_pk_mul_f32 %0, %1, %2 op_sel_hi:[1,0]" : "=v"(t) : "v"(v), "v"(w));
  asm("v_pk_fma_f32 %0, %1, %2, %3 op_sel:[1,1,0] op_sel_hi:[0,1,1] neg_lo:[1,0,0]" : "=v"(d) : "v"(v), "v"(w), "v"(t));
  return d;
}
__device__ __forceinline__ void cmul2(v2& a, v2 wa, v2& b, v2 wb) {
  v2 ta, tb, da, db;
  asm("v_pk_mul_f32 %0, %1, %2 op_sel_hi:[1,0]" : "=v"(ta) : "v"(a), "v"(wa));
  asm("v_pk_mul_f32 %0, %1, %2 op_sel_hi:[1,0]" : "=v"(tb) : "v"(b), "v"(wb));
  asm("v_pk_fma_f32 %0, %1, %2, %3 op_sel:[1,1,0] op_sel_hi:[0,1,1] neg_lo:[1,0,0]" : "=v"(da) : "v"(a), "v"(wa), "v"(ta));
  asm("v_pk_fma_f32 %0, %1, %2, %3 op_sel:[1,1,0] op_sel_hi:[0,1,1] neg_lo:[1,0,0]" : "=v"(db) : "v"(b), "v"(wb), "v"(tb));
  a = da; b = db;
}
__device__ __forceinline__ v2 cmul_s(v2 v, v2 w) {
  v2 t, d;
  asm("v_pk_mul_f32 %0, %1, %2 op_sel_hi:[1,0]" : "=v"(t) : "v"(v), "s"(w));
  asm("v_pk_fma_f32 %0, %1, %2, %3 op_sel:[1,1,0] op_sel_hi:[0,1,1] neg_lo:[1,0,0]" : "=v"(d) : "v"(v), "s"(w), "v"(t));
  return d;
}
__device__ __forceinline__ void cmul2_s(v2& a, v2 wa, v2& b, v2 wb) {
  v2 ta, tb, da, db;
  asm("v_pk_mul_f32 %0, %1, %2 op_sel_hi:[1,0]" : "=v"(ta) : "v"(a), "s"(wa));
  asm("v_pk_mul_f32 %0, %1, %2 op_sel_hi:[1,0]" : "=v"(tb) : "v"(b), "s"(wb));
  asm("v_pk_fma_f32 %0, %1, %2, %3 op_sel:[1,1,0] op_sel_hi:[0,1,1] neg_lo:[1,0,0]" : "=v"(da) : "v"(a), "s"(wa), "v"(ta));
  asm("v_pk_fma_f32 %0, %1, %2, %3 op_sel:[1,1,0] op_sel_hi:[0,1,1] neg_lo:[1,0,0]" : "=v"(db) : "v"(b), "s"(wb), "v"(tb));
  a = da; b = db;
}
__device__ __forceinline__ v2 fma_mi(v2 e, v2 H, v2 b) {
  v2 d; asm("v_pk_fma_f32 %0, %1, %2, %3 op_sel:[1,0,0] op_sel_hi:[0,0,1] neg_hi:[1,0,0]" : "=v"(d) : "v"(e), "s"(H), "v"(b)); return d;
}
__device__ __forceinline__ v2 fma_pi(v2 e, v2 H, v2 b) {
  v2 d; asm("v_pk_fma_f32 %0, %1, %2, %3 op_sel:[1,0,0] op_sel_hi:[0,0,1] neg_lo:[1,0,0]" : "=v"(d) : "v"(e), "s"(H), "v"(b)); return d;
}
__device__ __forceinline__ v2 sqsum(v2 s, v2 d) {
  v2 t, r;
  asm("v_pk_mul_f32 %0, %1, %1" : "=v"(t) : "v"(s));
  asm("v_pk_fma_f32 %0, %1, %1, %2 op_sel:[1,1,0] op_sel_hi:[0,0,1]" : "=v"(r) : "v"(d), "v"(t));
  return r;
}

__device__ __forceinline__ void sqsum2(v2 s0, v2 d0, v2 s1, v2 d1, v2& r0, v2& r1) {
  v2 t0, t1;
  asm("v_pk_mul_f32 %0, %1, %1" : "=v"(t0) : "v"(s0));
  asm("v_pk_mul_f32 %0, %1, %1" : "=v"(t1) : "v"(s1));
  asm("v_pk_fma_f32 %0, %1, %1, %2 op_sel:[1,1,0] op_sel_hi:[0,0,1]" : "=v"(r0) : "v"(d0), "v"(t0));
  asm("v_pk_fma_f32 %0, %1, %1, %2 op_sel:[1,1,0] op_sel_hi:[0,0,1]" : "=v"(r1) : "v"(d1), "v"(t1));
}
__device__ __forceinline__ float f3_max(float a, float b) {
  float r; asm("v_max_f32 %0, %1, %2" : "=v"(r) : "v"(a), "v"(b)); return r;
}

typedef const volatile v2 __attribute__((address_space(3))) * f3_lds_cv2;
__device__ __forceinline__ v2 ldv(const v2* p) { return *(f3_lds_cv2)(p); }
typedef volatile v2 __attribute__((address_space(3))) * f3_lds_v2;
__device__ __forceinline__ void stv(v2* p, v2 v) { *(f3_lds_v2)(p) = v; }
typedef const volatile float4 __attribute__((address_space(3))) * f3_lds_cv4;
__device__ __forceinline__ float4 ldv4(const float4* p) {
  const float __attribute__((ext_vector_type(4))) v = *(const volatile float __attribute__((ext_vector_type(4))) __attribute__((address_space(3)))*)(p);
  return float4{v.x, v.y, v.z, v.w};
}

__device__ __forceinline__ v2 f3_mel_mul_lo(v2 q, v2 c) {
  v2 d; asm("v_pk_mul_f32 %0, %1, %2 op_sel_hi:[1,0]" : "=v"(d) : "v"(q), "v"(c)); return d;
}
__device__ __forceinline__ v2 f3_mel_mul_hi(v2 q, v2 c) {
  v2 d; asm("v_pk_mul_f32 %0, %1, %2 op_sel:[0,1] op_sel_hi:[1,1]" : "=v"(d) : "v"(q), "v"(c)); return d;
}
__device__ __forceinline__ v2 f3_mel_fma_lo(v2 q, v2 c, v2 a) {
  v2 d; asm("v_pk_fma_f32 %0, %1, %2, %3 op_sel_hi:[1,0,1]" : "=v"(d) : "v"(q), "v"(c), "v"(a)); return d;
}
__device__ __forceinline__ v2 f3_mel_fma_hi(v2 q, v2 c, v2 a) {
  v2 d; asm("v_pk_fma_f32 %0, %1, %2, %3 op_sel:[0,1,0] op_sel_hi:[1,1,1]" : "=v"(d) : "v"(q), "v"(c), "v"(a)); return d;
}

__device__ __forceinline__ void f3_dft4(v2& x0, v2& x1, v2& x2, v2& x3) {
  const v2 a = x0 + x2, b = x0 - x2, c = x1 + x3, e = x1 - x3;
  x0 = a + c; x2 = a - c; x1 = add_mi(b, e); x3 = add_pi(b, e);
}

__device__ __forceinline__ void f3_dft8(v2* x, const v2 H) {
  v2 e0 = x[0], e1 = x[2], e2 = x[4], e3 = x[6];
  v2 o0 = x[1], o1 = x[3], o2 = x[5], o3 = x[7];
  f3_dft4(e0, e1, e2, e3);
  f3_dft4(o0, o1, o2, o3);
  const v2 q1 = add_mi(o1, o1);
  const v2 q3 = add_pi(o3, o3);
  x[0] = e0 + o0; x[4] = e0 - o0;
  x[1] = q1 * H + e1; x[5] = e1 - q1 * H;
  x[2] = add_mi(e2, o2); x[6] = add_pi(e2, o2);
  x[3] = e3 - q3 * H; x[7] = q3 * H + e3;
}

__device__ __forceinline__ void f3_dft16(v2* x, const v2 H, const v2 W1, const v2 W3) {
  v2 t0[4], t1[4], t2[4], t3[4];
#pragma unroll
  for (int n2 = 0; n2 < 4; ++n2) {
    v2 a = x[n2], b = x[n2 + 4], c = x[n2 + 8], d = x[n2 + 12];
    f3_dft4(a, b, c, d);
    t0[n2] = a; t1[n2] = b; t2[n2] = c; t3[n2] = d;
  }
  {
    f3_dft4(t0[0], t0[1], t0[2], t0[3]);
    x[0] = t0[0]; x[4] = t0[1]; x[8] = t0[2]; x[12] = t0[3];
  }
  {
    v2 p1 = t1[1], p3 = t1[3];
    cmul2_s(p1, W1, p3, W3);
    const v2 q = add_mi(t1[2], t1[2]);
    const v2 a = q * H + t1[0], b = t1[0] - q * H, c = p1 + p3, e = p1 - p3;
    x[1] = a + c; x[9] = a - c; x[5] = add_mi(b, e); x[13] = add_pi(b, e);
  }
  {
    const v2 q1 = add_mi(t2[1], t2[1]), q3 = add_pi(t2[3], t2[3]);
    const v2 a = add_mi(t2[0], t2[2]), b = add_pi(t2[0], t2[2]);
    const v2 c = q1 - q3, e = q1 + q3;
    x[2] = c * H + a; x[10] = a - c * H; x[6] = fma_mi(e, H, b); x[14] = fma_pi(e, H, b);
  }
  {
    v2 p1 = t3[1], m3 = t3[3];
    cmul2_s(p1, W3, m3, W1);
    const v2 q = add_pi(t3[2], t3[2]);
    const v2 a = t3[0] - q * H, b = q * H + t3[0], c = p1 - m3, e = p1 + m3;
    x[3] = a + c; x[11] = a - c; x[7] = add_mi(b, e); x[15] = add_pi(b, e);
  }
}

__device__ __forceinline__ int f3_opaque(int x) { asm volatile("" : "+s"(x)); return x; }
#ifdef AFX_F3_DEBUG
#define F3_SKIP(bit) ((kp.flags & (bit)) != 0)
#else
#define F3_SKIP(bit) false
#endif
struct F3Runs {
  int b_lo, b_hi, stride;
};
__device__ __forceinline__ F3Runs f3_runs_init(const int* work_ctr, int nblocks, int total_waves, int wg, bool contiguous) {
  F3Runs r;
  r.stride = 1;
  if (work_ctr) {
    const int C0 = nblocks / (2 * total_waves);
    r.b_lo = wg * C0; r.b_hi = r.b_lo + C0;
  } else if (contiguous) {
    r.b_lo = (int)((long long)wg * nblocks / total_waves); r.b_hi = (int)((long long)(wg + 1) * nblocks / total_waves);
  } else {
    r.b_lo = wg; r.b_hi = nblocks; r.stride = total_waves;
  }
  return r;
}
__device__ __forceinline__ bool f3_runs_next(F3Runs& r, int* work_ctr, int nblocks, int total_waves, int lane) {
  if (!work_ctr) return false;
  int t = 0;
  if (lane == 0) t = atomicAdd(work_ctr, 1);
  t = __builtin_amdgcn_readfirstlane(t);
  const int C0 = nblocks / (2 * total_waves), dyn0 = total_waves * C0;
  const int cA = C0 / 2 > 1 ? C0 / 2 : 1, cB = C0 / 3 > 1 ? C0 / 3 : 1;
  int c = 1;
  if (t < total_waves) { r.b_lo = dyn0 + cA * t; c = cA; }
  else if (t < 2 * total_waves) { r.b_lo = dyn0 + cA * total_waves + cB * (t - total_waves); c = cB; }
  else r.b_lo = dyn0 + (cA + cB) * total_waves + (t - 2 * total_waves);
  if (r.b_lo >= nblocks) return false;
  r.b_hi = r.b_lo + c < nblocks ? r.b_lo + c : nblocks;
  return true;
}

__device__ __forceinline__ float f3_add_xor16(float v) {
  const auto r = __builtin_amdgcn_permlane16_swap(__float_as_uint(v), __float_as_uint(v), false, false);
  return __uint_as_float(r[0]) + __uint_as_float(r[1]);
}
__device__ __forceinline__ float f3_add_xor32(float v) {
  const auto r = __builtin_amdgcn_permlane32_swap(__float_as_uint(v), __float_as_uint(v), false, false);
  return __uint_as_float(r[0]) + __uint_as_float(r[1]);
}
__device__ __forceinline__ float f3_sel(float a, float b, unsigned long long mask) {
  float d; asm("v_cndmask_b32_e64 %0, %1, %2, %3" : "=v"(d) : "v"(a), "v"(b), "s"(mask)); return d;
}
__device__ __forceinline__ float f3_sum2(float x, float y) {
  x += AFX_DPP_F(x, 0xB1, false); y += AFX_DPP_F(y, 0xB1, false);
  float m = f3_sel(y, x, 0xAAAAAAAAAAAAAAAAull);
  m += AFX_DPP_F(m, 0x4E, false);
  m += AFX_DPP_F(m, 0x124, false); m += AFX_DPP_F(m, 0x128, false);
  return f3_add_xor32(f3_add_xor16(m));
}

template <int FMT>
__device__ __forceinline__ float f3_edge_sample(const void* samples, const BlockDesc& bd, int64_t sbase, bool pre, float b1, int j) {
  const int lo = bd.have_lo, hi = bd.have_hi - 1;
  const int jc = j < lo ? lo : (j > hi ? hi : j), jp = (j - 1) < lo ? lo : ((j - 1) > hi ? hi : (j - 1));
  const float y = (jc == j) ? ld_raw<FMT>(samples, sbase + jc) : 0.f;
  const float yp = (jp == j - 1) ? ld_raw<FMT>(samples, sbase + jp) : 0.f;
  float v = y;
  if (pre) {
    v = preemph1(y, yp, b1);
    if (j == lo) v = preemph0(ld_raw<FMT>(samples, bd.clip_off), ld_raw<FMT>(samples, bd.clip_off + 1));
  }
  return (j >= bd.keep_lo && j < bd.keep_hi) ? v : 0.f;
}
struct F3Max { __device__ float operator()(float a, float b) const { return f3_max(a, b); } };
__device__ __forceinline__ float f3_wave_max(float v) {
  v = row_reduce(v, F3Max());
  return fmaxf(fmaxf(row_total(v, 0), row_total(v, 1)), fmaxf(row_total(v, 2), row_total(v, 3)));
}

}
```

### audio_feature_extraction_amd/csrc/afx_frames3d.hip

```cpp
#include <hip/hip_runtime.h>

#include <cstdlib>
#include <type_traits>

#include "afx_device.h"
#include "afx_devenv.h"
#include "afx_frames3.h"
#include "afx_frames3_dev.h"

namespace afx {

constexpr int kF3dTabFloats = 256 + 768 + 512;

size_t frames3d_lds_bytes(int waves, const F3Tables& ft) {
  return (size_t)(waves * kF3ExFloats + kF3dTabFloats + ft.mel_wfloats + ft.mel_rounds * 64) * sizeof(float);
}

template <int FMT, int WAVES, bool SPEC, int NBS>
__global__ __launch_bounds__(WAVES * 64) void k_frames3d(const void* __restrict__ samples,
                                                         ClipInfo* __restrict__ info,
                                                         const BlockDesc* __restrict__ blocks, int nblocks,
                                                         const int* __restrict__ nblocks_dev,
                                                         F3Tables ft, KParams kp,
                                                         float* __restrict__ logmel,
                                                         float* __restrict__ blockmax,
                                                         float* __restrict__ bsum, int* __restrict__ work_ctr) {
  constexpr int N = 512, HOP = 128;
  extern __shared__ __attribute__((aligned(16))) float smem[];
  if (nblocks_dev) {
    nblocks = *nblocks_dev;
    if (nblocks <= 0) return;
  }
  const int tid = threadIdx.x, lane = tid & 63;
  const int wave = __builtin_amdgcn_readfirstlane(tid >> 6);
  const int lp = lane & 31, half = lane >> 5;
  float* const tabs = smem + WAVES * kF3ExFloats;
  v2* const T2 = reinterpret_cast<v2*>(tabs);
  v2* const T3 = reinterpret_cast<v2*>(tabs + 256);
  v2* const WT = reinterpret_cast<v2*>(tabs + 256 + 768);
  float* const MW = tabs + kF3dTabFloats;
  int* const MM = reinterpret_cast<int*>(MW + ft.mel_wfloats);
  v2* const Ew = reinterpret_cast<v2*>(smem + wave * kF3ExFloats);
  v2* const E = Ew + half * (kF3ExFloats / 4);
  float* const XBw = reinterpret_cast<float*>(Ew);

  {
    const v2* w512 = reinterpret_cast<const v2*>(ft.w1024);
    auto W = [&](int m) { const v2 v = w512[m & 255]; return (m & 256) ? -v : v; };
    if (tid < 128) T2[tid] = W(4 * (tid >> 4) * (tid & 15));
    if (tid < 32) {
      const int j[4] = {tid, tid ? 128 - tid : 64, tid + 32, 96 - tid};
#pragma unroll
      for (int a = 1; a < 4; ++a)
#pragma unroll
        for (int k = 0; k < 4; ++k) T3[((a - 1) * 4 + k) * 32 + tid] = W(a * j[k]);
#pragma unroll
      for (int v = 0; v < 8; ++v) {
        auto wn = [&](int u) { const int n = tid + 32 * u; return 0.5f * ft.window[n < N ? n : 0]; };
        WT[v * 32 + tid] = v2{wn(2 * v), wn(2 * v + 1)};
      }
    }
    for (int i = tid; i < ft.mel_wfloats; i += WAVES * 64) MW[i] = ft.mel_w[i];
    for (int i = tid; i < ft.mel_rounds * 64; i += WAVES * 64) MM[i] = ft.mel_meta[i];
    for (int i = lane; i < kF3ExFloats; i += 64) XBw[i] = 0.f;
  }
  __syncthreads();

  const v2 H = {0.70710678118654752440f, 0.70710678118654752440f};
  const v2 W1 = {0.92387953251128675613f, -0.38268343236508977173f};
  const v2 W3 = {0.38268343236508977173f, -0.92387953251128675613f};
  const bool pre = (kp.flags & AFX_FLAG_PREEMPH) != 0;
  const float b1 = kp.preemph_b1;
  const int M = kp.n_mels;
  const int jb0 = lp ? 128 - lp : 64, ja1 = lp + 32, jb1 = 96 - lp;
  v2* const e1w = E + lp;
  const v2* const e1r = E + 34 * (lp & 15) + (lp >> 4);
  v2* const e2w = E + 128 * (lp >> 4) + (lp & 15);

  using sample_t = sample_of<FMT>;
  const int n_rounds = ft.mel_rounds;
  const float amin = kp.amin;

  auto rowsum4 = [&](float r0, float r1, float r2, float r3, bool upper, bool& bad) -> float {
    float q = r0 * r0; q = fmaf(r1, r1, q); q = fmaf(r2, r2, q); q = fmaf(r3, r3, q);
    bad = !(isfinite(r0) && isfinite(r1) && isfinite(r2) && isfinite(r3));
    q = row_reduce(q, OpAdd());
    return upper ? row_total(q, 2) + row_total(q, 3) : row_total(q, 0) + row_total(q, 1);
  };
  auto put_sum = [&](float t, bool bad, bool upper, const BlockDesc& bd, int j) {
    if (j >= 0 && j < bd.bsum_n) {
      if (lane == 0) bsum[bd.bsum_base + j] = t;
      if (!(fabsf(t) < INFINITY)) {
        const bool mine = bad && ((lane >> 5) == (upper ? 1 : 0));
        if (__any(mine) && lane == 0) atomicOr(&info[bd.clip].nonfinite, 1u);
      }
    }
  };

  const int total_waves = gridDim.x * WAVES;
  F3Runs runs = f3_runs_init(work_ctr, nblocks, total_waves, blockIdx.x * WAVES + wave, false);
  do {
  for (int b = runs.b_lo; b < runs.b_hi; b += runs.stride) {
    const BlockDesc bd = blocks[b];
    if (!bd.active) continue;
    const int Tleft = bd.T - bd.t0;
    const int nit = Tleft >= 16 ? 4 : (Tleft + 3) >> 2;
    const int64_t sbase = bd.sample_base;
    const sample_t* const sp = (const sample_t*)samples + sbase;
    auto interior = [&](int j0, int j1) -> bool {
      return (j0 - 1 >= bd.have_lo) && (j1 <= bd.have_hi) && (j0 >= bd.keep_lo) && (j1 <= bd.keep_hi);
    };
    auto edge_sample = [&](int j) { return f3_edge_sample<FMT>(samples, bd, sbase, pre, b1, j); };
    float lmax = -INFINITY;
    float* const tile = logmel + bd.frame_slot * (int64_t)M;

#pragma unroll 1
    for (int it = 0; it < nit; ++it) {
      const int j0 = 512 * it;
      float rows[20];
      if (interior(j0, j0 + 256 + N + HOP)) {
        float y[20], yp[20];
#pragma unroll
        for (int u = 0; u < 20; ++u) {
          y[u] = ld_row<FMT>(sp + j0, 256 * half + 32 * u + lp); yp[u] = ld_row<FMT>(sp + j0 - 1, 256 * half + 32 * u + lp);
        }
#pragma unroll
        for (int u = 0; u < 20; ++u) rows[u] = pre ? preemph1(y[u], yp[u], b1) : y[u];
      } else {
#pragma unroll 1
        for (int u = 0; u < 20; ++u) XBw[640 * half + 32 * u + lp] = edge_sample(j0 + 256 * half + 32 * u + lp);
#pragma unroll
        for (int u = 0; u < 20; ++u) rows[u] = XBw[640 * half + 32 * u + lp];
      }
      if constexpr (SPEC) {
        const int g = bd.t0 + 4 * it;
        bool bad;
        if (g == 0) { const float t = rowsum4(rows[8], rows[9], rows[10], rows[11], false, bad); put_sum(t, bad, false, bd, 0); }
        float q[4];
#pragma unroll
        for (int k = 0; k < 4; ++k) {
          q[k] = rows[4 + 4 * k] * rows[4 + 4 * k];
          q[k] = fmaf(rows[5 + 4 * k], rows[5 + 4 * k], q[k]); q[k] = fmaf(rows[6 + 4 * k], rows[6 + 4 * k], q[k]);
          q[k] = fmaf(rows[7 + 4 * k], rows[7 + 4 * k], q[k]);
        }
        const unsigned long long odd = 0xAAAAAAAAAAAAAAAAull, hi2 = 0xCCCCCCCCCCCCCCCCull;
        float s01 = f3_sel(q[0], q[1], odd) + AFX_DPP_F(f3_sel(q[1], q[0], odd), 0xB1, false);
        float s23 = f3_sel(q[2], q[3], odd) + AFX_DPP_F(f3_sel(q[3], q[2], odd), 0xB1, false);
        float sq = f3_sel(s01, s23, hi2) + AFX_DPP_F(f3_sel(s23, s01, hi2), 0x4E, false);
        sq += AFX_DPP_F(sq, 0x124, false); sq += AFX_DPP_F(sq, 0x128, false);
        sq = f3_add_xor16(sq);
        const int jk = g + 1 + (lane & 3);
        if (lane >= 32 && lane < 36 && jk < bd.bsum_n) bsum[bd.bsum_base + jk] = sq;
        if (__any(lane >= 32 && !(fabsf(sq) < INFINITY))) {
#pragma unroll
          for (int k = 0; k < 4; ++k) {
            const bool badk = !(isfinite(rows[4 + 4 * k]) && isfinite(rows[5 + 4 * k]) && isfinite(rows[6 + 4 * k]) && isfinite(rows[7 + 4 * k]));
            if (g + 1 + k < bd.bsum_n && __any(badk && lane >= 32) && lane == 0) atomicOr(&info[bd.clip].nonfinite, 1u);
          }
        }
      }
      v2 z[16];
#pragma unroll
      for (int v = 0; v < 8; ++v) {
        const v2 w = ldv(WT + v * 32 + lp);
        z[2 * v] = v2{rows[2 * v], rows[2 * v + 4]} * v2{w.x, w.x};
        z[2 * v + 1] = v2{rows[2 * v + 1], rows[2 * v + 5]} * v2{w.y, w.y};
      }
      f3_dft16(z, H, W1, W3);
#pragma unroll
      for (int k = 0; k < 16; ++k) stv(e1w + 34 * k, z[k]);
#pragma unroll
      for (int u = 0; u < 16; ++u) z[u] = ldv(e1r + 2 * u);
      {
        v2 tw[8];
#pragma unroll
        for (int r = 1; r < 8; ++r) tw[r] = ldv(T2 + r * 16 + (lp & 15));
        v2 xa[8], xb[8];
#pragma unroll
        for (int r = 0; r < 8; ++r) { xa[r] = z[2 * r]; xb[r] = z[2 * r + 1]; }
#pragma unroll
        for (int r = 1; r < 8; ++r) cmul2(xa[r], tw[r], xb[r], tw[r]);
        f3_dft8(xa, H); f3_dft8(xb, H);
#pragma unroll
// ... 22 lines not shown
        E[jb0 + 128] = p0; E[jb0] = p1;
        sqsum2(A1[0] + B1[3], A1[0] - B1[3], A1[1] + B1[2], A1[1] - B1[2], p0, p1);
        E[ja1] = p0; E[ja1 + 128] = p1;
        sqsum2(A1[2] + B1[1], A1[2] - B1[1], A1[3] + B1[0], A1[3] - B1[0], p0, p1);
        E[jb1 + 128] = p0; E[jb1] = p1;
        if (lp == 0) E[256] = v2{4.f * nyq.x * nyq.x, 4.f * nyq.y * nyq.y};
      }
      const int fA = 4 * it + 2 * half;
      const bool vA = fA < Tleft, vB = fA + 1 < Tleft;
      float* const rowA = tile + (unsigned)(fA * M);
      __builtin_amdgcn_s_setprio(1);
      if constexpr (NBS > 0) {
        int woff = 0;
#pragma unroll
        for (int rd = 0; rd < 4; ++rd) {
          constexpr int kNbs = NBS;
          const int nb = (kNbs >> (4 * rd)) & 15;
          if (nb == 0) break;
          const int meta = MM[rd * 64 + lane];
          const float4* pp = reinterpret_cast<const float4*>(E + (meta & 2047));
          const float4* ww = reinterpret_cast<const float4*>(MW + woff) + lane;
          woff += nb * 256;
          v2 sa[4];
#pragma unroll
          for (int i = 0; i < 8; ++i) {
            if (i < nb) {
              const float4 c = ww[64 * i], q0 = pp[2 * i], q1 = pp[2 * i + 1];
              const v2 c01 = {c.x, c.y}, c23 = {c.z, c.w};
              if (i == 0) {
                sa[0] = f3_mel_mul_lo(v2{q0.x, q0.y}, c01); sa[1] = f3_mel_mul_hi(v2{q0.z, q0.w}, c01);
                sa[2] = f3_mel_mul_lo(v2{q1.x, q1.y}, c23); sa[3] = f3_mel_mul_hi(v2{q1.z, q1.w}, c23);
              } else {
                sa[0] = f3_mel_fma_lo(v2{q0.x, q0.y}, c01, sa[0]); sa[1] = f3_mel_fma_hi(v2{q0.z, q0.w}, c01, sa[1]);
                sa[2] = f3_mel_fma_lo(v2{q1.x, q1.y}, c23, sa[2]); sa[3] = f3_mel_fma_hi(v2{q1.z, q1.w}, c23, sa[3]);
              }
            }
          }
          const v2 acc = (sa[0] + sa[1]) + (sa[2] + sa[3]);
          const float L0 = 3.01029995663981195f * __builtin_amdgcn_logf(f3_max(acc.x, amin));
          const float L1 = 3.01029995663981195f * __builtin_amdgcn_logf(f3_max(acc.y, amin));
          const unsigned m = (meta >> 11) & 511;
          if (vA) { rowA[m] = L0; lmax = f3_max(lmax, L0); }
          if (vB) { rowA[M + m] = L1; lmax = f3_max(lmax, L1); }
        }
      } else {
#pragma unroll 1
      for (int rd = 0; rd < n_rounds; ++rd) {
        const uint32_t rp = ft.mel_rp[rd];
        const int meta = MM[rd * 64 + lane];
        const float4* pp = reinterpret_cast<const float4*>(E + (meta & 2047));
        const float4* ww = reinterpret_cast<const float4*>(MW + (rp >> 8)) + lane;
        const int nb = rp & 15, wd = (rp >> 4) & 15;
        v2 a0 = {0.f, 0.f}, a1 = {0.f, 0.f};
#define F3_BATCH(i)                                                                  \
        if (nb > (i)) {                                                              \
          const float4 c = ww[64 * (i)];                                             \
          const float4 q0 = pp[2 * (i)], q1 = pp[2 * (i) + 1];                       \
          a0 = v2{q0.x, q0.y} * v2{c.x, c.x} + a0; a1 = v2{q0.z, q0.w} * v2{c.y, c.y} + a1; \
          a0 = v2{q1.x, q1.y} * v2{c.z, c.z} + a0; a1 = v2{q1.z, q1.w} * v2{c.w, c.w} + a1; \
        }
        F3_BATCH(0) F3_BATCH(1) F3_BATCH(2) F3_BATCH(3) F3_BATCH(4) F3_BATCH(5) F3_BATCH(6) F3_BATCH(7)
#undef F3_BATCH
        v2 acc = a0 + a1;
        if (wd >= 2) { acc.x += AFX_DPP_F(acc.x, 0xB1, false); acc.y += AFX_DPP_F(acc.y, 0xB1, false); }
        if (wd >= 4) { acc.x += AFX_DPP_F(acc.x, 0x4E, false); acc.y += AFX_DPP_F(acc.y, 0x4E, false); }
        if (wd >= 8) { acc.x += AFX_DPP_F(acc.x, 0x141, false); acc.y += AFX_DPP_F(acc.y, 0x141, false); }
        const float L0 = 3.01029995663981195f * __builtin_amdgcn_logf(f3_max(acc.x, amin));
        const float L1 = 3.01029995663981195f * __builtin_amdgcn_logf(f3_max(acc.y, amin));
        if (meta & (1 << 20)) {
          const unsigned m = (meta >> 11) & 511;
          if (vA) { rowA[m] = L0; lmax = f3_max(lmax, L0); }
          if (vB) { rowA[M + m] = L1; lmax = f3_max(lmax, L1); }
        }
      }
      }
      __builtin_amdgcn_s_setprio(0);
    }
    {
      const float mx = f3_wave_max(lmax);
      if constexpr (SPEC) { if (lane == 0) blockmax[b] = mx; }
      else { if (lane == 0 && mx > -INFINITY) atomicMax(&info[bd.clip].lmax_ord, f2ord(mx)); }
    }
  }
  } while (f3_runs_next(runs, work_ctr, nblocks, (int)(gridDim.x * WAVES), lane));
}

int frames3d_waves(const F3Tables& ft) {
  const int forced = dev_env().f3_waves;
  if (forced == 12 || forced == 16) return frames3d_lds_bytes(forced, ft) <= 160 * 1024 ? forced : 12;
  return frames3d_lds_bytes(16, ft) <= 160 * 1024 ? 16 : 12;
}

template <int FMT, int WAVES, bool SPEC, int NBS>
static hipError_t launch_frames3d_t(const F3Launch& L) {
  const hipError_t e = allow_lds_once<k_frames3d<FMT, WAVES, SPEC, NBS>>();
  if (e != hipSuccess) return e;
  hipLaunchKernelGGL((k_frames3d<FMT, WAVES, SPEC, NBS>), dim3(f3_grid(L, WAVES)), dim3(WAVES * 64), frames3d_lds_bytes(WAVES, L.ft), L.s,
                     L.samples, L.info, L.blocks, L.nblocks, L.nblocks_dev, L.ft, L.kp, L.logmel, L.blockmax, L.bsum, L.work_ctr);
  return hipGetLastError();
}

hipError_t launch_frames3d(const F3Launch& L) {
  const F3Tables& ft = L.ft;
  const int waves = frames3d_waves(ft);
  bool fixed = ft.mel_rounds == 4 && ft.mel_all_own && !dev_env().f3_generic_mel;
  const int want_nb[4] = {1, 1, 2, 4};
  int woff = 0;
  for (int r = 0; r < 4 && fixed; ++r) {
    fixed = (int)(ft.mel_rp[r] & 15) == want_nb[r] && ((ft.mel_rp[r] >> 4) & 15) == 1 && (int)(ft.mel_rp[r] >> 8) == woff;
    woff += want_nb[r] * 256;
  }
#define AFX_F3D_GO2(FMT, W, NBS) (L.spec ? launch_frames3d_t<FMT, W, true, NBS>(L) : launch_frames3d_t<FMT, W, false, NBS>(L))
#define AFX_F3D_GO(FMT, W) (fixed ? AFX_F3D_GO2(FMT, W, 0x4211) : AFX_F3D_GO2(FMT, W, 0))
  if (L.kp.fmt == AFX_FMT_S16) return waves == 16 ? AFX_F3D_GO(AFX_FMT_S16, 16) : AFX_F3D_GO(AFX_FMT_S16, 12);
  return waves == 16 ? AFX_F3D_GO(AFX_FMT_F32, 16) : AFX_F3D_GO(AFX_FMT_F32, 12);
#undef AFX_F3D_GO
#undef AFX_F3D_GO2
}

}
```

### audio_feature_extraction_amd/csrc/afx_frames3s.hip

```cpp
#include <hip/hip_runtime.h>

#include <cstdlib>
#include <type_traits>

#include "afx_device.h"
#include "afx_devenv.h"
#include "afx_frames3.h"
#include "afx_frames3_dev.h"

namespace afx {

constexpr int kF3sTabFloats = 2048 + 1024 + 2048;

size_t frames3s_lds_bytes(int waves, const F3Tables& ft) {
  return (size_t)(waves * kF3ExFloats + kF3sTabFloats + ft.mel_wfloats + ft.mel_rounds * 64) * sizeof(float);
}

template <int FMT, int WAVES, bool SPEC, bool DESC, int NBS = 0, int WDS = 0>
__global__ __launch_bounds__(WAVES * 64) void k_frames3s(const void* __restrict__ samples,
                                                         ClipInfo* __restrict__ info,
                                                         const BlockDesc* __restrict__ blocks, int nblocks,
                                                         const int* __restrict__ nblocks_dev,
                                                         F3Tables ft, KParams kp,
                                                         float* __restrict__ logmel,
                                                         float* __restrict__ blockmax,
                                                         float* __restrict__ bsum,
                                                         float* __restrict__ desc_out,
                                                         const int64_t* __restrict__ desc_offs,
                                                         SpecBands sb, int* __restrict__ work_ctr) {
  constexpr int N = 2048, HOP = 512;
  extern __shared__ __attribute__((aligned(16))) float smem[];
  if (nblocks_dev) {
    nblocks = *nblocks_dev;
    if (nblocks <= 0) return;
  }
  const int tid = threadIdx.x, lane = tid & 63;
  const int wave = __builtin_amdgcn_readfirstlane(tid >> 6);
  float* const tabs = smem + WAVES * kF3ExFloats;
  v2* const T2 = reinterpret_cast<v2*>(tabs);
  v2* const T3a = reinterpret_cast<v2*>(tabs + 256);
  v2* const T3b = reinterpret_cast<v2*>(tabs + 256 + 896);
  v2* const TS = reinterpret_cast<v2*>(tabs + 2048);
  v2* const WT = reinterpret_cast<v2*>(tabs + 2048 + 1024);
  float* const MW = tabs + kF3sTabFloats;
  int* const MM = reinterpret_cast<int*>(MW + ft.mel_wfloats);
  v2* const E = reinterpret_cast<v2*>(smem + wave * kF3ExFloats);
  float* const XB = reinterpret_cast<float*>(E);

  {
    const v2* w1024 = reinterpret_cast<const v2*>(ft.w1024);
    const v2* w2048 = reinterpret_cast<const v2*>(ft.w2048);
    auto W = [&](int m) { const v2 v = w1024[m & 511]; return (m & 512) ? -v : v; };
    if (tid < 128) T2[tid] = W(8 * (tid >> 4) * (tid & 15));
    if (tid < 64) {
      const int jbt = tid ? 128 - tid : 64;
#pragma unroll
      for (int r = 1; r < 8; ++r) { T3a[(r - 1) * 64 + tid] = W(tid * r); T3b[(r - 1) * 64 + tid] = W(jbt * r); }
#pragma unroll
      for (int s = 0; s < 8; ++s) TS[s * 64 + tid] = w2048[((tid == 0 && s >= 4) ? 64 : tid) + 128 * s];
#pragma unroll
      for (int u = 0; u < 16; ++u) {
        const int n = 2 * (tid + 64 * u);
        WT[u * 64 + tid] = v2{0.5f * ft.window[n], 0.5f * ft.window[n + 1]};
      }
    }
    for (int i = tid; i < ft.mel_wfloats; i += WAVES * 64) MW[i] = ft.mel_w[i];
    for (int i = tid; i < ft.mel_rounds * 64; i += WAVES * 64) MM[i] = ft.mel_meta[i];
    for (int i = lane; i < kF3ExFloats; i += 64) XB[i] = 0.f;
  }
  __syncthreads();

  const v2 H = {0.70710678118654752440f, 0.70710678118654752440f};
  const v2 W1 = {0.92387953251128675613f, -0.38268343236508977173f};
  const v2 W3 = {0.38268343236508977173f, -0.92387953251128675613f};
  const bool pre = (kp.flags & AFX_FLAG_PREEMPH) != 0;
  const float b1 = kp.preemph_b1;
  const int M = kp.n_mels;
  const int jb = lane ? 128 - lane : 64;
  const int lq = lane ? lane : 64;
  v2* const e1w = E + lane;
  const v2* const e1r = E + 66 * (lane & 15) + (lane >> 4);
  v2* const e2w = E + 128 * (lane >> 4) + (lane & 15);
  const v2* const ea = E + lane;
  const v2* const eb = E + jb;

  using sample_t = sample_of<FMT>;
  const int n_rounds = ft.mel_rounds;
  const float amin = kp.amin;

  auto subblock = [&](v2 r0, v2 r1, v2 r2, v2 r3, const BlockDesc& bd, int j) {
    v2 a = r0 * r0; a = r1 * r1 + a; a = r2 * r2 + a; a = r3 * r3 + a;
    const float t = wave_sum(a.x + a.y);
    if (j >= 0 && j < bd.bsum_n) {
      if (lane == 0) bsum[bd.bsum_base + j] = t;
      if (!(fabsf(t) < INFINITY)) {
        const bool bad = !(isfinite(r0.x) && isfinite(r0.y) && isfinite(r1.x) && isfinite(r1.y) &&
                           isfinite(r2.x) && isfinite(r2.y) && isfinite(r3.x) && isfinite(r3.y));
        if (__any(bad) && lane == 0) atomicOr(&info[bd.clip].nonfinite, 1u);
      }
    }
  };

  const int total_waves = gridDim.x * WAVES;
  F3Runs runs = f3_runs_init(work_ctr, nblocks, total_waves, blockIdx.x * WAVES + wave, false);
  do {
  for (int b = runs.b_lo; b < runs.b_hi; b += runs.stride) {
    BlockDesc bd = blocks[b];
    if (!bd.active) continue;
    bool first = true;
    v2 R[16];
    for (;;) {
    const int Tleft = bd.T - bd.t0;
    const int nfr = Tleft >= 16 ? 16 : Tleft;
    bool chain = false;
    if (SPEC && nfr == 16 && runs.stride == 1 && b + 1 < runs.b_hi) {
      const BlockDesc* nx = blocks + b + 1;
      chain = nx->active && nx->clip == bd.clip && nx->t0 == bd.t0 + 16;
    }
    const int64_t sbase = bd.sample_base;
    const sample_t* const sp = (const sample_t*)samples + sbase;
    auto interior = [&](int j0, int j1) -> bool {
      return (j0 - 1 >= bd.have_lo) && (j1 <= bd.have_hi) && (j0 >= bd.keep_lo) && (j1 <= bd.keep_hi);
    };
    auto edge_sample = [&](int j) { return f3_edge_sample<FMT>(samples, bd, sbase, pre, b1, j); };
    auto pre_row = [&](float x0, float x1, float xp) -> v2 {
      return pre ? v2{preemph1(x0, xp, b1), preemph1(x1, x0, b1)} : v2{x0, x1};
    };

    if (first) {
    if (interior(0, N)) {
      float x0[16], x1[16], xp[16];
#pragma unroll
      for (int u = 0; u < 16; ++u) {
        x0[u] = ld_row<FMT>(sp, 128 * u + 2 * lane); x1[u] = ld_row<FMT>(sp, 128 * u + 2 * lane + 1); xp[u] = ld_row<FMT>(sp - 1, 128 * u + 2 * lane);
      }
#pragma unroll
      for (int u = 0; u < 16; ++u) R[u] = pre_row(x0[u], x1[u], xp[u]);
    } else {
#pragma unroll 1
      for (int u = 0; u < 16; ++u) {
        XB[128 * u + 2 * lane] = edge_sample(128 * u + 2 * lane);
        XB[128 * u + 2 * lane + 1] = edge_sample(128 * u + 2 * lane + 1);
      }
#pragma unroll
      for (int u = 0; u < 16; ++u) R[u] = E[64 * u + lane];
    }
    if constexpr (SPEC) {
      if (bd.t0 == 0) subblock(R[8], R[9], R[10], R[11], bd, 0);
      subblock(R[12], R[13], R[14], R[15], bd, bd.t0 + 1);
    }
    }
    float lmax = -INFINITY;
    float* const tile = logmel + bd.frame_slot * (int64_t)M;

#pragma unroll 1
    for (int f = 0; f < nfr; ++f) {
      v2 z[16];
#pragma unroll
      for (int u = 0; u < 16; ++u) z[u] = R[u] * ldv(WT + u * 64 + lane);
#pragma unroll
      for (int u = 0; u < 12; ++u) R[u] = R[u + 4];
      const bool more = f + 1 < nfr || chain;
      const int jn = HOP * f + N;
      const bool nint = more && interior(jn, jn + HOP);

      f3_dft16(z, H, W1, W3);
#pragma unroll
      for (int k = 0; k < 16; ++k) stv(e1w + 66 * k, z[k]);
#pragma unroll
      for (int u = 0; u < 16; ++u) z[u] = ldv(e1r + 4 * u);
      {
        v2 tw[8];
#pragma unroll
        for (int r = 1; r < 8; ++r) tw[r] = ldv(T2 + r * 16 + (lane & 15));
        v2 xa[8], xb[8];
#pragma unroll
        for (int r = 0; r < 8; ++r) { xa[r] = z[2 * r]; xb[r] = z[2 * r + 1]; }
#pragma unroll
        for (int r = 1; r < 8; ++r) cmul2(xa[r], tw[r], xb[r], tw[r]);
        f3_dft8(xa, H); f3_dft8(xb, H);
#pragma unroll
        for (int r = 0; r < 8; ++r) { stv(e2w + 16 * r, xa[r]); stv(e2w + 16 * r + 512, xb[r]); }
      }
      v2 A[8], B[8];
#pragma unroll
      for (int r = 0; r < 8; ++r) { A[r] = ldv(ea + 128 * r); B[r] = ldv(eb + 128 * r); }
#pragma unroll
// ... 112 lines not shown
          const float4* pp = reinterpret_cast<const float4*>(XB + (meta & 2047));
          const float4* ww = reinterpret_cast<const float4*>(MW + woff) + lane;
          woff += nb * 256;
          v2 a0 = {0.f, 0.f}, a1 = {0.f, 0.f};
#pragma unroll
          for (int i = 0; i < 8; ++i) {
            if (i < nb) {
              const float4 c = ww[64 * i], q = pp[i];
              if (i == 0) { a0 = v2{q.x, q.y} * v2{c.x, c.y}; a1 = v2{q.z, q.w} * v2{c.z, c.w}; }
              else { a0 = v2{q.x, q.y} * v2{c.x, c.y} + a0; a1 = v2{q.z, q.w} * v2{c.z, c.w} + a1; }
            }
          }
          const v2 a = a0 + a1;
          float acc = a.x + a.y;
          if (wd >= 2) acc += AFX_DPP_F(acc, 0xB1, false);
          if (wd >= 4) acc += AFX_DPP_F(acc, 0x4E, false);
          if (wd >= 8) acc += AFX_DPP_F(acc, 0x141, false);
          const float L = 3.01029995663981195f * __builtin_amdgcn_logf(f3_max(acc, amin));
          if (wd == 1 || (meta & (1 << 20))) {
            const unsigned m = (meta >> 11) & 511;
            if (vF) { rowF[m] = L; lmax = f3_max(lmax, L); }
          }
        }
      } else {
#pragma unroll 1
      for (int rd = 0; rd < n_rounds; ++rd) {
        const uint32_t rp = ft.mel_rp[rd];
        const int meta = MM[rd * 64 + lane];
        const float4* pp = reinterpret_cast<const float4*>(XB + (meta & 2047));
        const float4* ww = reinterpret_cast<const float4*>(MW + (rp >> 8)) + lane;
        const int nb = rp & 15, wd = (rp >> 4) & 15;
        v2 a0 = {0.f, 0.f}, a1 = {0.f, 0.f};
#define F3_BATCH(i)                                                                  \
        if (nb > (i)) {                                                              \
          const float4 c = ww[64 * (i)];                                             \
          const float4 q = pp[(i)];                                                  \
          a0 = v2{q.x, q.y} * v2{c.x, c.y} + a0; a1 = v2{q.z, q.w} * v2{c.z, c.w} + a1; \
        }
        F3_BATCH(0) F3_BATCH(1) F3_BATCH(2) F3_BATCH(3) F3_BATCH(4) F3_BATCH(5) F3_BATCH(6) F3_BATCH(7)
#undef F3_BATCH
        const v2 a = a0 + a1;
        float acc = a.x + a.y;
        if (wd >= 2) acc += AFX_DPP_F(acc, 0xB1, false);
        if (wd >= 4) acc += AFX_DPP_F(acc, 0x4E, false);
        if (wd >= 8) acc += AFX_DPP_F(acc, 0x141, false);
        const float L = 3.01029995663981195f * __builtin_amdgcn_logf(f3_max(acc, amin));
        if (meta & (1 << 20)) {
          const unsigned m = (meta >> 11) & 511;
          if (vF) { rowF[m] = L; lmax = f3_max(lmax, L); }
        }
      }
      }
      __builtin_amdgcn_s_setprio(0);
      }

      if (more) {
        if (nint) {
#pragma unroll
          for (int i = 0; i < 4; ++i) R[12 + i] = pre_row(nx0[i], nx1[i], nxp[i]);
        } else {
#pragma unroll 1
          for (int i = 0; i < 4; ++i) {
            XB[128 * i + 2 * lane] = edge_sample(jn + 128 * i + 2 * lane);
            XB[128 * i + 2 * lane + 1] = edge_sample(jn + 128 * i + 2 * lane + 1);
          }
#pragma unroll
          for (int i = 0; i < 4; ++i) R[12 + i] = E[64 * i + lane];
        }
        if constexpr (SPEC) subblock(R[12], R[13], R[14], R[15], bd, bd.t0 + f + 2);
      }
    }
    {
      const float mx = f3_wave_max(lmax);
      if constexpr (DESC) { (void)mx; }
      else if constexpr (SPEC) { if (lane == 0) blockmax[b] = mx; }
      else { if (lane == 0 && mx > -INFINITY) atomicMax(&info[bd.clip].lmax_ord, f2ord(mx)); }
    }
    if (!chain) break;
    first = false;
    ++b;
    bd = blocks[b];
    }
  }
  } while (f3_runs_next(runs, work_ctr, nblocks, (int)(gridDim.x * WAVES), lane));
}

int frames3s_waves(const F3Tables& ft) {
  const int forced = dev_env().f3_waves;
  if (forced == 12 || forced == 16) return frames3s_lds_bytes(forced, ft) <= 160 * 1024 ? forced : 12;
  return frames3s_lds_bytes(16, ft) <= 160 * 1024 ? 16 : 12;
}

template <int FMT, int WAVES, bool SPEC, int NBS, int WDS>
static hipError_t launch_frames3s_t(const F3Launch& L) {
  const hipError_t e = allow_lds_once<k_frames3s<FMT, WAVES, SPEC, false, NBS, WDS>>();
  if (e != hipSuccess) return e;
  hipLaunchKernelGGL((k_frames3s<FMT, WAVES, SPEC, false, NBS, WDS>), dim3(f3_grid(L, WAVES)), dim3(WAVES * 64), frames3s_lds_bytes(WAVES, L.ft), L.s,
                     L.samples, L.info, L.blocks, L.nblocks, L.nblocks_dev, L.ft, L.kp, L.logmel, L.blockmax, L.bsum, nullptr, nullptr, SpecBands{}, L.work_ctr);
  return hipGetLastError();
}

template <int FMT>
static hipError_t launch_spectral_t(hipStream_t s, const void* samples, ClipInfo* info, const BlockDesc* blocks, int nblocks,
                                    const F3Tables& ft, const KParams& kp, float* desc_out, const int64_t* desc_offs,
                                    const SpecBands& sb, int n_cu) {
  const hipError_t e = allow_lds_once<k_frames3s<FMT, 12, false, true>>();
  if (e != hipSuccess) return e;
  const int grid = std::max(1, std::min(n_cu, (nblocks + 11) / 12));
  hipLaunchKernelGGL((k_frames3s<FMT, 12, false, true>), dim3(grid), dim3(12 * 64), frames3s_lds_bytes(12, ft), s,
                     samples, info, blocks, nblocks, nullptr, ft, kp, nullptr, nullptr, nullptr, desc_out, desc_offs, sb, nullptr);
  return hipGetLastError();
}

hipError_t launch_spectral(hipStream_t s, const void* samples, ClipInfo* info, const BlockDesc* blocks, int nblocks,
                           const F3Tables& ft, const KParams& kp, float* desc_out, const int64_t* desc_offs,
                           const SpecBands& sb, int n_cu) {
  if (kp.fmt == AFX_FMT_S16) return launch_spectral_t<AFX_FMT_S16>(s, samples, info, blocks, nblocks, ft, kp, desc_out, desc_offs, sb, n_cu);
  return launch_spectral_t<AFX_FMT_F32>(s, samples, info, blocks, nblocks, ft, kp, desc_out, desc_offs, sb, n_cu);
}

hipError_t launch_frames3s(const F3Launch& L) {
  const F3Tables& ft = L.ft;
  const int waves = frames3s_waves(ft);
  bool fixed = ft.mel_rounds == 4 && !dev_env().f3_generic_mel;
  const int want_nb[4] = {3, 1, 5, 5}, want_wd[4] = {1, 4, 2, 4};
  int woff = 0;
  for (int r = 0; r < 4 && fixed; ++r) {
    fixed = (int)(ft.mel_rp[r] & 15) == want_nb[r] && (int)((ft.mel_rp[r] >> 4) & 15) == want_wd[r] && (int)(ft.mel_rp[r] >> 8) == woff;
    woff += want_nb[r] * 256;
  }
  fixed = fixed && (ft.mel_own_w1 != 0);
#define AFX_F3S_GO2(FMT, W, NBS, WDS) (L.spec ? launch_frames3s_t<FMT, W, true, NBS, WDS>(L) : launch_frames3s_t<FMT, W, false, NBS, WDS>(L))
#define AFX_F3S_GO(FMT, W) (fixed ? AFX_F3S_GO2(FMT, W, 0x5513, 0x4241) : AFX_F3S_GO2(FMT, W, 0, 0))
  if (L.kp.fmt == AFX_FMT_S16) return waves == 16 ? AFX_F3S_GO(AFX_FMT_S16, 16) : AFX_F3S_GO(AFX_FMT_S16, 12);
  return waves == 16 ? AFX_F3S_GO(AFX_FMT_F32, 16) : AFX_F3S_GO(AFX_FMT_F32, 12);
#undef AFX_F3S_GO
#undef AFX_F3S_GO2
}

}
```

### audio_feature_extraction_amd/csrc/afx_host.cpp

```cpp
#include <algorithm>
#include <cfloat>
#include <cmath>
#include <cstring>
#include <string>

#include "afx_device.h"
#include "afx_f0.h"
#include "afx_internal.h"
#include "afx_mr.h"

namespace afx {

static thread_local std::string g_err;
void set_error(const std::string& s) { g_err = s; }

bool build_clip_descs(int hop, int trim_hop, const int64_t* offsets, const int64_t* lengths, int n, ClipDesc* out,
                      BatchGeom& g, std::string& why) {
  g = BatchGeom{};
  if (hop <= 0 || trim_hop <= 0) { why = "hop / trim hop must be positive"; return false; }
  int64_t fb = 0, tb = 0, nblk = 0;
  int max_tb = 0, max_tm = 0;
  const int64_t kMaxElems = (int64_t)1 << 46;
  for (int i = 0; i < n; ++i) {
    if (lengths[i] < 0 || offsets[i] < 0) { why = "negative clip offset/length"; return false; }
    if (offsets[i] > kMaxElems) { why = "clip offset too large"; return false; }
    if (lengths[i] / hop > (int64_t)1 << 30 || lengths[i] > kMaxElems) { why = "clip too long"; return false; }
    ClipDesc& c = out[i];
    c.off = offsets[i]; c.len = lengths[i];
    c.tmax = (int32_t)(1 + lengths[i] / hop);
    c.tpad = (c.tmax + kFramesPerBlock - 1) / kFramesPerBlock * kFramesPerBlock;
    c.frame_base = fb; c.tblk_base = tb;
    fb += c.tpad;
    const int64_t ntb = (lengths[i] + trim_hop - 1) / trim_hop;
    tb += ntb;
    max_tb = (int)std::max<int64_t>(max_tb, std::min<int64_t>(ntb, INT32_MAX));
    max_tm = std::max<int>(max_tm, c.tmax);
    c.blk_base = (int32_t)nblk; c.pad_ = 0;
    nblk += c.tpad / kFramesPerBlock;
    if (nblk > (int64_t)1 << 30 || tb > (int64_t)1 << 40) { why = "batch too large"; return false; }
  }
  g.total_tpad = fb; g.total_tblk = tb; g.max_tblocks = std::max(max_tb, 1); g.max_tmax = max_tm; g.nblocks = (int)nblk;
  return true;
}

template <int R>
static void mr_host_pass(const mrc* in, mrc* out, const mrc* tw, int N2, int NS) {
  const int nbf = N2 / R, step = N2 / (NS * R);
  for (int j = 0; j < nbf; ++j) {
    mrc x[R];
    for (int r = 0; r < R; ++r) x[r] = in[j + r * nbf];
    const int jm = j % NS;
    mr_butterfly<R>(x, tw, jm, step, NS == 1);
    for (int r = 0; r < R; ++r) out[(j - jm) * R + jm + r * NS] = x[r];
  }
}

}

using namespace afx;

extern "C" int afx_rfft_host(int n_fft, const float* x, float* out) {
  if (!x || !out) { set_error("afx_rfft_host: null argument"); return AFX_ERR_INVALID; }
  if (!mr_supported(n_fft)) {
    set_error("afx_rfft_host: frame_length must be a multiple of 16 in [256, 2048] with no prime factor other than 2, 3 and 5");
    return AFX_ERR_UNSUPPORTED;
  }
  const int N2 = n_fft / 2;
  std::vector<float> twf, postf;
  build_fft_tables(n_fft, twf, postf);
  const mrc* tw = reinterpret_cast<const mrc*>(twf.data());
  const mrc* post = reinterpret_cast<const mrc*>(postf.data());
  std::vector<mrc> a((size_t)N2), b((size_t)N2);
  for (int n = 0; n < N2; ++n) a[n] = mr_mk(x[2 * n], x[2 * n + 1]);
  const MrSchedule sc = mr_schedule(N2);
  int NS = 1;
  for (int p = 0; p < sc.n; ++p) {
    switch (sc.radix(p)) {
      case 3: mr_host_pass<3>(a.data(), b.data(), tw, N2, NS); break;
      case 4: mr_host_pass<4>(a.data(), b.data(), tw, N2, NS); break;
      case 5: mr_host_pass<5>(a.data(), b.data(), tw, N2, NS); break;
      default: mr_host_pass<8>(a.data(), b.data(), tw, N2, NS); break;
    }
    NS *= sc.radix(p);
    a.swap(b);
  }
  for (int k = 0; k < N2; ++k) {
    const mrc X2 = mr_split2(a[k], a[(N2 - k) % N2], post[k]);
    out[2 * k] = 0.5f * X2.x; out[2 * k + 1] = 0.5f * X2.y;
  }
  out[2 * N2] = a[0].x - a[0].y; out[2 * N2 + 1] = 0.f;
  return AFX_OK;
}

extern "C" int afx_version(void) { return AFX_VERSION; }

extern "C" const char* afx_last_error(void) { return g_err.c_str(); }

extern "C" int afx_batch_geometry(const afx_params* p, const int64_t* offsets, const int64_t* lengths, int n_clips,
                                  int64_t* records, int64_t* totals) {
  if (!p || n_clips < 0 || (n_clips > 0 && (!offsets || !lengths))) { set_error("afx_batch_geometry: null/invalid argument"); return AFX_ERR_INVALID; }
  std::string msg;
  int st = validate_params(*p, msg);
  if (st != AFX_OK) { set_error(msg); return st; }
  std::vector<ClipDesc> cd((size_t)std::max(n_clips, 1));
  BatchGeom g;
  if (!build_clip_descs(p->hop, p->trim_hop, offsets, lengths, n_clips, cd.data(), g, msg)) { set_error("afx_batch_geometry: " + msg); return AFX_ERR_INVALID; }
  if (records)
    for (int i = 0; i < n_clips; ++i) {
      int64_t* r = records + 4 * (size_t)i;
      r[0] = cd[i].frame_base; r[1] = cd[i].tmax; r[2] = cd[i].tpad; r[3] = cd[i].blk_base;
    }
  if (totals) { totals[0] = g.total_tpad; totals[1] = g.nblocks; totals[2] = g.total_tblk; totals[3] = g.max_tmax; }
  return AFX_OK;
}

extern "C" int afx_f0_build_tables(int sr, int n_fft, int hop, double fmin, double fmax, int32_t* info,
                                   double* beta, double* lt, double* freqs) {
  HostF0Tables t;
  std::string why;
  if (!build_f0_tables(sr, n_fft, hop, fmin, fmax, t, why)) { set_error("afx_f0_build_tables: " + why); return AFX_ERR_UNSUPPORTED; }
  if (info) {
    const int32_t v[8] = {t.p.min_period, t.p.max_period, t.p.n_bins, t.p.band, t.p.cap, t.p.n_lag, t.p.R, t.p.slots};
    std::memcpy(info, v, sizeof(v));
  }
  if (beta) std::memcpy(beta, t.beta.data(), t.beta.size() * sizeof(double));
  if (lt) std::memcpy(lt, t.lt.data(), t.lt.size() * sizeof(double));
  if (freqs) std::memcpy(freqs, t.freqs.data(), t.freqs.size() * sizeof(double));
  return AFX_OK;
}


extern "C" int afx_f0_dispatch(int sr, int n_fft, int hop, double fmin, double fmax, int32_t* out) {
  if (!out) { set_error("afx_f0_dispatch: null argument"); return AFX_ERR_INVALID; }
  if (sr <= 0 || hop <= 0 || n_fft < 2 || n_fft > 4096) { set_error("afx_f0_dispatch: sr, hop_length must be positive and frame_length in [2, 4096]"); return AFX_ERR_INVALID; }
  HostF0Tables t;
  F0Dispatch d;
  std::string why;
  if (!f0_plan(sr, n_fft, hop, fmin, fmax, t, d, why)) { set_error("afx_f0_dispatch: " + why); return AFX_ERR_UNSUPPORTED; }
  const int32_t v[12] = {d.energy_lpw, d.epb, d.yin_n, d.yin_fpb, d.yin_sh, d.vit_nbt, d.vit_bandt, d.vit_tpt, d.bt_depth,
                         t.p.band, t.p.n_bins, d.yin_lds};
  std::memcpy(out, v, sizeof(v));
  return AFX_OK;
}

extern "C" int afx_chroma_filters(int sr, double tuning, float* out) {
  if (!out) { set_error("afx_chroma_filters: null argument"); return AFX_ERR_INVALID; }
  if (sr <= 0 || !std::isfinite(tuning)) { set_error("afx_chroma_filters: sr must be positive and tuning finite"); return AFX_ERR_INVALID; }
  constexpr int NB = 1025;
  const double a440 = 440.0 * std::pow(2.0, tuning / 12.0) / 16.0, step = (double)sr / 2048.0;
  double q[NB + 1];
  for (int j = 1; j <= NB; ++j) q[j] = 12.0 * std::log2(((double)j * step) / a440);
  q[0] = q[1] - 18.0;
  for (int j = 0; j < NB; ++j) {
    const double bw = std::max(q[j + 1] - q[j], 1.0);
    double w[12], ss = 0.0;
    for (int c = 0; c < 12; ++c) {
      const double d = std::fmod(q[j] - (double)c + 6.0 + 120.0, 12.0) - 6.0, e = 2.0 * d / bw;
      w[c] = std::exp(-0.5 * (e * e));
      ss += w[c] * w[c];
    }
    const double norm = std::max(std::sqrt(ss), DBL_MIN), o = (q[j] / 12.0 - 5.0) / 2.0, oct = std::exp(-0.5 * (o * o));
    for (int c = 0; c < 12; ++c) out[c * NB + j] = (float)(w[(c + 3) % 12] / norm * oct);
  }
  return AFX_OK;
}
```

### audio_feature_extraction_amd/csrc/afx_misc.hip

```cpp
#include <hip/hip_runtime.h>

#include <algorithm>

#include "afx_device.h"
#include "afx_f0.h"
#include "afx_wave.h"

namespace afx {

__global__ __launch_bounds__(256) void k_preemph(const float* __restrict__ y, float* __restrict__ out,
                                                 int64_t n, float b1) {
  const int64_t i = (int64_t)blockIdx.x * 256 + threadIdx.x;
  if (i >= n) return;
  out[i] = (i == 0) ? ((n > 1) ? preemph0(y[0], y[1]) : y[0]) : preemph1(y[i], y[i - 1], b1);
}

constexpr int kF0PrepPerThread = 8;
__global__ __launch_bounds__(256) void k_f0_prep(const void* __restrict__ samples,
                                                 const ClipDesc* __restrict__ clips,
                                                 const ClipInfo* __restrict__ info,
                                                 float* __restrict__ ysig, KParams kp) {
  const int clip = blockIdx.y;
  const ClipInfo ci = info[clip];
  const ClipDesc cd = clips[clip];
  const int64_t np = ci.end - ci.start;
  const bool pre = (kp.flags & AFX_FLAG_PREEMPH) != 0;
  for (int64_t n0 = (int64_t)blockIdx.x * (256 * kF0PrepPerThread); n0 < np; n0 += (int64_t)gridDim.x * (256 * kF0PrepPerThread)) {
#pragma unroll
    for (int u = 0; u < kF0PrepPerThread; ++u) {
      const int64_t n = n0 + u * 256 + threadIdx.x;
      if (n >= np) break;
      const int64_t i = ci.start + n;
      const float y = ld_sample(samples, kp.fmt, cd.off + i);
      float v = y;
      if (pre) {
        if (i == 0) v = (cd.len > 1) ? preemph0(y, ld_sample(samples, kp.fmt, cd.off + 1)) : y;
        else v = preemph1(y, ld_sample(samples, kp.fmt, cd.off + i - 1), kp.preemph_b1);
      }
      ysig[cd.off + n] = v;
    }
  }
}

__global__ __launch_bounds__(1024) void k_finish(uint4* info, int n_info16, int* counters, unsigned* flag, unsigned seq) {
  for (int i = threadIdx.x; i < n_info16; i += 1024) info[i] = uint4{0u, 0u, 0u, 0u};
  if (counters && threadIdx.x < 4) counters[threadIdx.x] = 0;
  __syncthreads();
  if (flag && threadIdx.x == 0) __hip_atomic_store(flag, seq, __ATOMIC_RELEASE, __HIP_MEMORY_SCOPE_SYSTEM);
}
hipError_t launch_finish(hipStream_t s, ClipInfo* info, int n_clips, int* counters, unsigned* flag_dev, unsigned seq) {
  static_assert(sizeof(ClipInfo) == 32, "k_finish clears ClipInfo as two 16-byte words");
  hipLaunchKernelGGL(k_finish, dim3(1), dim3(1024), 0, s, (uint4*)info, n_clips * 2, counters, flag_dev, seq);
  return hipGetLastError();
}

hipError_t launch_preemph(hipStream_t s, const float* y, float* out, int64_t n, float b1) {
  hipLaunchKernelGGL(k_preemph, dim3((unsigned)((n + 255) / 256)), dim3(256), 0, s, y, out, n, b1);
  return hipGetLastError();
}

hipError_t launch_f0_prep(hipStream_t s, const void* samples, const ClipDesc* clips, const ClipInfo* info,
                          float* ysig, int n_clips, int64_t max_len, const KParams& kp) {
  const int64_t per_wg = 256 * kF0PrepPerThread;
  const int gx = (int)std::min<int64_t>(std::max<int64_t>((max_len + per_wg - 1) / per_wg, 1), 1024);
  hipLaunchKernelGGL(k_f0_prep, dim3(gx, n_clips), dim3(256), 0, s, samples, clips, info, ysig, kp);
  return hipGetLastError();
}

}
```

### audio_feature_extraction_amd/csrc/afx_plan.h

```cpp
#pragma once
#include <algorithm>
#include <cstdint>
#include <string>
#include <utility>
#include <vector>

#include <hip/hip_runtime.h>

#include "afx_chroma.h"
#include "afx_decode.h"
#include "afx_device.h"
#include "afx_f0.h"
#include "afx_frames3.h"
#include "afx_internal.h"
#include "afx_resample.h"

namespace afx {

struct DevBuf {
  void* p = nullptr;
  size_t cap = 0;
};

}

using namespace afx;

struct afx_ctx {
  int device = 0;
  hipStream_t stream = nullptr;
  DevBuf dtw_raw, dtw_feats, dtw_norms, dtw_pairs, dtw_codes, dtw_rows, dtw_d, dtw_path, dtw_cost, dtw_status, dtw_len;
  struct {
    bool valid = false, custom = false;
    int up = 0, down = 0;
    std::vector<double> taps;
    RsTables t;
  } rs;
  DevBuf rs_g, rs_tstart, rs_clips, rs_in, rs_out;
  DevBuf dc_clips, dc_in, dc_out;
};

struct afx_plan {
  afx_ctx* ctx = nullptr;
  int device = 0;
  afx_params p{};
  KParams kp{};
  HostTables ht;
  DevTables dt{};
  F3Tables f3{};
  bool use_f3 = false;
  std::vector<void*> table_allocs;
  DevBuf samples, clips, info, blocks, bsum, logmel, rms, mfcc, frames, frame_offs, stamps;
  DevBuf blocks_spec, blockmax, items, n_items;
  std::vector<BlockDesc> h_blocks;
  ClipDesc* h_clips_pin = nullptr;
  size_t h_clips_pin_cap = 0;
  hipEvent_t clips_ev = nullptr;
  bool clips_ev_pending = false;
  bool f0_ready = false;
  double f0_fmin = 0.0, f0_fmax = 0.0;
  HostF0Tables f0_ht;
  F0Tables f0_dt{};
  std::vector<void*> f0_allocs;
  DevBuf f0_in, f0_ysig, f0_energy, f0_cnt, f0_vp, f0_bin, f0_prob, f0_lprob, f0_lu, f0_ptr, f0_best, f0_states, f0_stats, f0_out, f0_offs;
  DevBuf hp_clips, hp_y, hp_h, hp_p, hp_x, hp_yh, hp_yp, hp_bad, hp_stats, hp_spec;
  DevBuf ch_grid, ch_extra, ch_mel, ch_s, ch_mag, ch_bin, ch_slot, ch_hist, ch_chroma, ch_melout, ch_parts;
  ChromaMel ch_melrec{};
  std::vector<int64_t> c_off, c_len;
  std::vector<ClipDesc> h_clips;
  std::vector<int64_t> h_rebased;
  int nblocks = 0, max_tblocks = 0, max_tmax = 0;
  int64_t total_tpad = 0, total_tblk = 0;
  void* h_pin = nullptr;
  void* h_pin_dev = nullptr;
  size_t h_pin_cap = 0;
  int info_clean_n = 0;
  struct Pending {
    bool active = false;
    int n = 0;
    size_t stats_bytes = 0;
    float* out_stats = nullptr; int32_t* out_status = nullptr; int64_t* out_trim = nullptr; int32_t* out_nframes = nullptr;
  } pend;
  hipEvent_t done = nullptr;
  volatile unsigned* flag = nullptr;
  unsigned* flag_dev = nullptr;
  unsigned seq = 0;
  bool timing = false;
  bool timing_frames_only = false;
  hipEvent_t ev[AFX_K_COUNT][2] = {};
  bool ev_ready = false;
  double ms_sum[AFX_K_COUNT] = {};
  int32_t launches[AFX_K_COUNT] = {};
  std::vector<std::pair<double, double>> spans[AFX_K_COUNT];
  int n_cu = 256;
};

#pragma GCC visibility push(hidden)

#define HIP_TRY(expr)                                                                  \
  do {                                                                                 \
    hipError_t e__ = (expr);                                                           \
    if (e__ != hipSuccess) {                                                           \
      set_error(std::string(#expr) + ": " + hipGetErrorString(e__));                   \
      return AFX_ERR_HIP;                                                              \
    }                                                                                  \
  } while (0)

inline int ensure(DevBuf& b, size_t bytes) {
  if (bytes <= b.cap && b.p) return AFX_OK;
  if (b.p) { (void)hipFree(b.p); b.p = nullptr; b.cap = 0; }
  size_t want = std::max<size_t>(bytes + bytes / 8, 256);
  hipError_t e = hipMalloc(&b.p, want);
  if (e != hipSuccess) {
    set_error(std::string("hipMalloc(") + std::to_string(want) + "): " + hipGetErrorString(e));
    b.p = nullptr;
    return e == hipErrorOutOfMemory ? AFX_ERR_NOMEM : AFX_ERR_HIP;
  }
  b.cap = want;
  return AFX_OK;
}

inline void release(DevBuf& b) {
  if (b.p) (void)hipFree(b.p);
  b.p = nullptr; b.cap = 0;
}

int null_arg(const char* who);
int check_sample_format(const char* who, int sample_fmt, int mem_kind);
int check_batch_args(const char* who, afx_plan* pl, const void* samples, int sample_fmt, int mem_kind,
                     const int64_t* offsets, const int64_t* lengths, int n_clips, bool empty_ok = false);
int check_clip_ranges(const char* who, const int64_t* offsets, const int64_t* lengths, const int64_t* out_offsets, int n_clips,
                      int64_t max_off);
int begin_plan_call(const char* who, afx_plan* pl);
int stage_samples(afx_plan* pl, DevBuf& buf, const void* samples, int sample_fmt, int mem_kind, const int64_t* offsets,
                  const int64_t* lengths, int n, const void** d_samples);
int prepare_descriptors(afx_plan* pl, const int64_t* offsets, const int64_t* lengths, int n);
int run_preprocess(afx_plan* pl, const void* d_samples, int n, const KParams& kp, bool f0_prep);
int rebase_offsets(const afx_plan* pl, const char* what, const int64_t* offs, int n, int64_t per_frame,
                   std::vector<int64_t>& rebased, int64_t* lo, int64_t* hi);
int upload_frame_range(afx_plan* pl, const int64_t* rebased, int n, DevBuf& d_offs, DevBuf& out, size_t bytes, int fill);
int run_spectral(afx_plan* pl, const void* d_signal, int n, const KParams& kp, const int64_t* h_offsets, size_t count,
                 const SpecBands& sb);
int statuses_from_info(afx_plan* pl, int n, int32_t* out_status);

#pragma GCC visibility pop
```

### audio_feature_extraction_amd/csrc/afx_trim3.hip

```cpp
#include <hip/hip_runtime.h>

#include "afx_device.h"
#include "afx_frames3.h"
#include "afx_trim_dev.h"
#include "afx_wave.h"

namespace afx {

__global__ __launch_bounds__(256) void k_trim_decide3(const ClipDesc* __restrict__ clips, ClipInfo* __restrict__ info,
                                                      const float* __restrict__ bsum, const float* __restrict__ blockmax,
                                                      BlockDesc* __restrict__ items, int* __restrict__ n_items, int max_items,
                                                      float* __restrict__ rms_rows, KParams kp) {
  __shared__ float red_f[4];
  __shared__ long long red_a[4], red_b[4];
  const int clip = blockIdx.x, tid = threadIdx.x, wave = tid >> 6, lane = tid & 63;
  const ClipDesc cd = clips[clip];
  const int64_t N = cd.len;
  const uint32_t nonfinite = info[clip].nonfinite;
  int status = AFX_CLIP_OK;
  if (N < 2) status = AFX_CLIP_TOO_SHORT;
  else if (nonfinite) status = AFX_CLIP_NONFINITE;
  int64_t start = 0, end = N;
  const int per = kp.rms_sub;
  if ((kp.flags & AFX_FLAG_TRIM) && status == AFX_CLIP_OK)
    trim_search(bsum + cd.tblk_base * per, N, kp, per, red_f, red_a, red_b, true, start, end);
  const int hop = kp.hop;
  const int T = (int)(1 + (end - start) / hop);
  if (status == AFX_CLIP_OK && T < 9) status = AFX_CLIP_TOO_SHORT;
  const int g0 = (int)(start / hop), glast = g0 + T - 1;
  const int nblk = cd.tpad / kFramesPerBlock;
  const bool cutL = start > 0, cutR = end < N;
  const int bLo = cutL ? (g0 + 2 + 15) >> 4 : 0;
  const int bHi = cutR ? (glast >= 17 ? (glast - 17) >> 4 : -1) : nblk - 1;
  float cm = -INFINITY;
  if (status == AFX_CLIP_OK)
    for (int b = bLo + tid; b <= bHi; b += 256) cm = fmaxf(cm, blockmax[cd.blk_base + b]);
  cm = wave_max(cm);
  if (lane == 0) red_f[wave] = cm;
  __syncthreads();
  cm = fmaxf(fmaxf(red_f[0], red_f[1]), fmaxf(red_f[2], red_f[3]));
  if (tid == 0) {
    ClipInfo ci;
    ci.start = start; ci.end = end; ci.T = T; ci.status = status;
    ci.lmax_ord = cm > -INFINITY ? f2ord(cm) : 0u;
    ci.nonfinite = nonfinite;
    info[clip] = ci;
    if (status == AFX_CLIP_OK && (cutL || cutR)) {
      int r0[2], r1[2], nr = 0;
      if (bLo > bHi) { r0[0] = g0; r1[0] = glast + 1; nr = 1; }
      else {
        if (cutL && 16 * bLo > g0) { r0[nr] = g0; r1[nr] = 16 * bLo < glast + 1 ? 16 * bLo : glast + 1; ++nr; }
        if (cutR && 16 * (bHi + 1) <= glast) { r0[nr] = 16 * (bHi + 1) > g0 ? 16 * (bHi + 1) : g0; r1[nr] = glast + 1; ++nr; }
      }
      int cnt = 0;
      for (int r = 0; r < nr; ++r) cnt += (r1[r] - r0[r] + 15) / 16;
      if (cnt > 0) {
        const int at = atomicAdd(n_items, cnt);
        int k = 0;
        for (int r = 0; r < nr; ++r)
          for (int gf = r0[r]; gf < r1[r]; gf += 16, ++k) {
            if (at + k >= max_items) break;
            const int nfr = r1[r] - gf < 16 ? r1[r] - gf : 16;
            items[at + k] = make_block(cd, clip, (int64_t)gf * hop - kp.n_fft / 2, gf, start, end, N, 0, nfr, true, 0, 0);
          }
      }
    }
  }
  if (rms_rows && (status == AFX_CLIP_OK || (status == AFX_CLIP_TOO_SHORT && N >= 2)))
    trim_rms_rows(bsum + cd.tblk_base * per, start, end, T, kp, rms_rows + cd.frame_base);
}

__global__ __launch_bounds__(64) void k_build_blocks3(const ClipDesc* __restrict__ clips, int n_clips,
                                                      BlockDesc* __restrict__ blocks, int n_fft, int hop, int trim_hop, int per) {
  const int clip = blockIdx.x;
  if (clip >= n_clips) return;
  const ClipDesc c = clips[clip];
  const int nb = c.tpad / kFramesPerBlock;
  const int64_t ntb = (c.len + trim_hop - 1) / trim_hop;
  for (int b = threadIdx.x; b < nb; b += 64) {
    const int64_t gs = (int64_t)b * kFramesPerBlock * hop - n_fft / 2;
    const int t0 = b * kFramesPerBlock;
    blocks[c.blk_base + b] = make_block(c, clip, gs, t0, 0, c.len, c.len, t0, c.tmax, c.len >= 2 && t0 < c.tmax,
                                        (int32_t)(c.tblk_base * per), (int32_t)(ntb * per));
  }
}

hipError_t launch_build_blocks3(hipStream_t s, const ClipDesc* clips, int n_clips, int nblocks, BlockDesc* blocks,
                                const KParams& kp) {
  if (nblocks <= 0 || n_clips <= 0) return hipSuccess;
  hipLaunchKernelGGL(k_build_blocks3, dim3(n_clips), dim3(64), 0, s, clips, n_clips, blocks,
                     kp.n_fft, kp.hop, kp.trim_hop, kp.rms_sub);
  return hipGetLastError();
}

hipError_t launch_trim_decide3(hipStream_t s, const ClipDesc* clips, ClipInfo* info, const float* bsum, const float* blockmax,
                               BlockDesc* items, int* n_items, int max_items, float* rms_rows, int n_clips, const KParams& kp) {
  hipLaunchKernelGGL(k_trim_decide3, dim3(n_clips), dim3(256), 0, s, clips, info, bsum, blockmax, items, n_items, max_items,
                     rms_rows, kp);
  return hipGetLastError();
}

}
```

### include/afx.h

```cpp
#ifndef AFX_H
#define AFX_H

#include <stddef.h>
#include <stdint.h>

#ifdef __cplusplus
extern "C" {
#endif

#define AFX_VERSION 107

typedef enum afx_status {
  AFX_OK = 0,
  AFX_ERR_INVALID = -1,
  AFX_ERR_NO_DEVICE = -2,
  AFX_ERR_HIP = -3,
  AFX_ERR_NOMEM = -4,
  AFX_ERR_UNSUPPORTED = -5
} afx_status;

typedef enum afx_clip_status {
  AFX_CLIP_OK = 0,
  AFX_CLIP_TOO_SHORT = 1,
  AFX_CLIP_NONFINITE = 2
// ... 48 lines not shown

int afx_init(int device, afx_ctx** out);
void afx_destroy(afx_ctx* ctx);

int afx_malloc(afx_ctx* ctx, size_t bytes, void** out_dptr);
int afx_free(afx_ctx* ctx, void* dptr);
int afx_host_alloc(afx_ctx* ctx, size_t bytes, void** out);
int afx_host_free(afx_ctx* ctx, void* hptr);
int afx_memcpy_h2d(afx_ctx* ctx, void* dst_d, const void* src_h, size_t bytes);
int afx_memcpy_d2h(afx_ctx* ctx, void* dst_h, const void* src_d, size_t bytes);
int afx_synchronize(afx_ctx* ctx);

void afx_default_params(afx_params* p);
int afx_plan_create(afx_ctx* ctx, const afx_params* p, afx_plan** out);
void afx_plan_destroy(afx_plan* plan);

int afx_build_tables(const afx_params* p, float* window, float* mel_dense, float* dct);

int afx_build_mel_schedule(const afx_params* p, int32_t* info, float* weights, int32_t* meta);

int afx_batch_geometry(const afx_params* p, const int64_t* offsets, const int64_t* lengths, int n_clips,
                       int64_t* records, int64_t* totals);

int afx_extract_batch(afx_plan* plan,
                      const void* samples, int sample_fmt, int mem_kind,
                      const int64_t* offsets, const int64_t* lengths, int n_clips,
                      int flags,
                      float* out_stats, int32_t* out_status,
                      int64_t* out_trim, int32_t* out_nframes,
                      float* out_frames, const int64_t* frame_offsets);

int afx_extract_submit(afx_plan* plan,
                       const void* samples, int sample_fmt, int mem_kind,
                       const int64_t* offsets, const int64_t* lengths, int n_clips,
                       int flags,
                       float* out_stats, int32_t* out_status,
                       int64_t* out_trim, int32_t* out_nframes,
                       float* out_frames, const int64_t* frame_offsets);
int afx_extract_collect(afx_plan* plan);

int afx_f0_batch(afx_plan* plan,
                 const void* samples, int sample_fmt, int mem_kind,
                 const int64_t* offsets, const int64_t* lengths, int n_clips,
                 int flags, double fmin, double fmax,
                 double* out_f0stats, int32_t* out_status,
                 double* out_f0, const int64_t* f0_offsets);

int afx_zcr_batch(afx_plan* plan,
                  const void* samples, int sample_fmt, int mem_kind,
                  const int64_t* offsets, const int64_t* lengths, int n_clips, int flags,
                  double* out_zcr, const int64_t* zcr_offsets, int32_t* out_status);

int afx_spectral_batch(afx_plan* plan,
                       const void* samples, int sample_fmt, int mem_kind,
                       const int64_t* offsets, const int64_t* lengths, int n_clips, int flags,
                       float* out_desc, const int64_t* desc_offsets, int32_t* out_status);

int afx_dtw_batch(afx_ctx* ctx, const float* feats, int dim,
                  const int64_t* x_off, const int64_t* x_len, const int64_t* y_off, const int64_t* y_len,
                  const int32_t* band_r, int n_pairs, int metric, int flags,
                  double* out_cost, int32_t* out_status,
                  int32_t* out_path, const int64_t* path_off, int32_t* out_path_len,
                  double* out_D, const int64_t* d_off);

int afx_hpss_batch(afx_plan* plan, const void* samples, int sample_fmt, int mem_kind,
                   const int64_t* offsets, const int64_t* lengths, int n_clips, int flags,
                   float* out_harm, float* out_perc, double* out_stats,
                   float* out_spec, const int64_t* spec_off, int32_t* out_status);

enum { AFX_CHROMA_STORE_HIST = 8 };
int afx_chroma_batch(afx_plan* plan, const void* samples, int sample_fmt, int mem_kind,
                     const int64_t* offsets, const int64_t* lengths, int n_clips, int flags,
                     const double* tuning_in,
                     float* out_chroma, const int64_t* chroma_off,
                     float* out_mel, const int64_t* mel_off,
                     double* out_tuning, double* out_stats, int32_t* out_hist, int32_t* out_status);
int afx_chroma_filters(int sr, double tuning, float* out );

int afx_f0_build_tables(int sr, int n_fft, int hop, double fmin, double fmax, int32_t* info,
                        double* beta, double* lt, double* freqs);

int afx_f0_dispatch(int sr, int n_fft, int hop, double fmin, double fmax, int32_t* out);

int afx_wav_probe(const char* const* paths, int n, int threads, int32_t* info , int64_t* frames,
                  int64_t* data_off, int32_t* status);
int afx_wav_read_s16(const char* const* paths, int n, int threads, const int64_t* data_off, const int64_t* frames,
                     int16_t* out, int64_t out_len, const int64_t* offsets, int32_t* status);

enum { AFX_SMP_U8 = 0, AFX_SMP_S16 = 1, AFX_SMP_S24 = 2, AFX_SMP_S32 = 3, AFX_SMP_F32 = 4, AFX_SMP_F64 = 5 };
int afx_wav_read_raw(const char* const* paths, int n, int threads, const int64_t* data_off, const int64_t* nbytes,
                     uint8_t* out, int64_t out_len, const int64_t* offsets , int32_t* status);
int afx_decode_batch(afx_ctx* ctx, const void* raw, int mem_kind, const int64_t* byte_offsets, const int64_t* frames,
                     const int32_t* kinds, const int32_t* channels, int n_clips,
                     float* out, int out_mem_kind, const int64_t* out_offsets);

int afx_resample_design(int sr_in, int sr_out, int32_t* info , double* taps);
int afx_resample_batch(afx_ctx* ctx, const void* samples, int sample_fmt, int mem_kind,
                       const int64_t* offsets, const int64_t* lengths, int n_clips, int sr_in, int sr_out,
                       const double* taps, int n_taps, float* out, int out_mem_kind,
                       const int64_t* out_offsets, int64_t* out_lengths);

int afx_rfft_host(int n_fft, const float* x , float* out );

int afx_preprocess(afx_plan* plan, const float* y, int64_t n,
                   float* out_y, int64_t* start, int64_t* end, int32_t* status);

enum {
  AFX_K_TRIM_BLOCKS = 0,
  AFX_K_TRIM_DECIDE = 1,
  AFX_K_FRAMES = 2,
  AFX_K_DCT = 3,
  AFX_K_STATS = 4,
  AFX_K_COUNT = 5
};
int afx_plan_set_timing(afx_plan* plan, int enable);
int afx_plan_get_timings(afx_plan* plan, float* ms_sum ,
                         int32_t* launches , int reset);
int afx_plan_get_intervals(afx_plan* plan, int kernel_slot, double* start_ms, double* end_ms, int cap, int32_t* count);

#ifdef __cplusplus
}
#endif
#endif
```

Measured before the change: 1.293 billion frames/s.

## Rework frames3 work tickets with multi-head queues and split tail blocks

Replaces the single work counter of the speculative frames3 pass with a table of queue heads stored after the block list. Tail blocks can be split into smaller sub-item records, and waves hop between heads when one runs dry. The goal is better load balance at the end of the pass and less contention on one atomic counter. With the default split eighths set to 0 the split is effectively disabled, so the main change under defaults is the head-based dequeue, which adds some per-dequeue cost and complexity.

```diff
diff --git a/audio_feature_extraction_amd/_native.py b/audio_feature_extraction_amd/_native.py
--- a/audio_feature_extraction_amd/_native.py
+++ b/audio_feature_extraction_amd/_native.py
@@ -39,7 +39,7 @@
     "afx_extract_batch", "afx_extract_submit", "afx_extract_collect", "afx_f0_batch", "afx_zcr_batch", "afx_spectral_batch", "afx_f0_build_tables", "afx_f0_dispatch", "afx_preprocess", "afx_plan_set_timing", "afx_plan_get_timings", "afx_plan_get_intervals",
     "afx_wav_probe", "afx_wav_read_s16", "afx_batch_geometry", "afx_dtw_batch", "afx_hpss_batch",
     "afx_resample_design", "afx_resample_batch", "afx_rfft_host", "afx_wav_read_raw", "afx_decode_batch",
-    "afx_chroma_batch", "afx_chroma_filters",
+    "afx_chroma_batch", "afx_chroma_filters", "afx_f3_tickets", "afx_f3_ticket_runs", "afx_f3_next_head",
 )
 
 
@@ -118,6 +118,10 @@
         if hasattr(L, "afx_chroma_batch"):
             L.afx_chroma_batch.argtypes = [vp, vp, i32, i32, vp, vp, i32, i32, vp, vp, vp, vp, vp, vp, vp, vp, vp]
             L.afx_chroma_filters.argtypes = [i32, C.c_double, vp]
+        if hasattr(L, "afx_f3_tickets"):
+            L.afx_f3_tickets.argtypes = [i32, i32, i32, i32, i32, i32, vp, vp]
+            L.afx_f3_ticket_runs.argtypes = [vp, i32, i32, vp]
+            L.afx_f3_next_head.argtypes = [i32, C.c_uint32]
         if hasattr(L, "afx_rfft_host"):
             L.afx_rfft_host.argtypes = [i32, vp, vp]
         _lib = L
@@ -217,6 +221,31 @@
     out = np.zeros(len(F0_DISPATCH_KEYS), np.int32)
     _check(lib().afx_f0_dispatch(int(sr), int(n_fft), int(hop), float(fmin), float(fmax), out.ctypes.data), "afx_f0_dispatch")
     return {k: int(v) for k, v in zip(F0_DISPATCH_KEYS, out)}
+
+
+F3_HEAD_KEYS = ("lo", "hi", "waves", "run_a", "run_b", "upfront", "tickets", "empty")
+
+
+def f3_tickets(nblocks: int, split: int, item: int, min_item: int, grid: int, waves: int) -> dict:
+    if not hasattr(lib(), "afx_f3_tickets"):
+        raise NotImplementedError("this libafx has no afx_f3_tickets")
+    geom = np.zeros(6, np.int32)
+    heads = np.zeros((16, 8), np.int32)
+    _check(lib().afx_f3_tickets(int(nblocks), int(split), int(item), int(min_item), int(grid), int(waves),
+                                geom.ctypes.data, heads.ctypes.data), "afx_f3_tickets")
+    keys = ("nblocks", "whole", "per_block", "item", "qbase", "nrecords")
+    return dict({k: int(v) for k, v in zip(keys, geom)}, heads=heads)
+
+
+def f3_ticket_runs(head, t0: int, count: int) -> np.ndarray:
+    head = np.ascontiguousarray(head, np.int32).reshape(8)
+    out = np.zeros((int(count), 2), np.int32)
+    _check(lib().afx_f3_ticket_runs(head.ctypes.data, int(t0), int(count), out.ctypes.data), "afx_f3_ticket_runs")
+    return out
+
+
+def f3_next_head(head: int, mask: int) -> int:
+    return int(lib().afx_f3_next_head(int(head), int(mask) & 0xFFFFFFFF))
 
 
 def resample_design(sr_in: int, sr_out: int) -> dict:
diff --git a/audio_feature_extraction_amd/csrc/afx_api.cpp b/audio_feature_extraction_amd/csrc/afx_api.cpp
--- a/audio_feature_extraction_amd/csrc/afx_api.cpp
+++ b/audio_feature_extraction_amd/csrc/afx_api.cpp
@@ -32,6 +32,8 @@
   host_blocks = getenv("AFX_HOST_BLOCKS") != nullptr;
   no_fused_tail = getenv("AFX_NO_FUSED_TAIL") != nullptr;
   if (const char* v = getenv("AFX_F3_WAVES")) f3_waves = atoi(v);
+  if (const char* v = getenv("AFX_F3_SPLIT")) f3_split = std::max(0, atoi(v));
+  if (const char* v = getenv("AFX_F3_ITEM")) f3_item = std::max(0, atoi(v));
   if (const char* v = getenv("AFX_TAIL_MODE")) tail_mode = atoi(v);
   if (const char* v = getenv("AFX_TAIL_SKIP")) tail_skip = atoi(v) & 7;
   if (const char* v = getenv("AFX_TEST_CHUNK_CLIPS")) chunk_clips = std::max(1, std::min(32768, atoi(v)));
@@ -346,26 +348,30 @@
   HIP_TRY(hipEventRecord(pl->clips_ev, s));
   pl->clips_ev_pending = true;
   if (pl->use_f3) {
-    const size_t nb_alloc = (size_t)std::max<int64_t>(nblk, 1);
-    if ((rc = ensure(pl->blocks_spec, nb_alloc * sizeof(BlockDesc))) != AFX_OK) return rc;
-    if ((rc = ensure(pl->blockmax, nb_alloc * sizeof(float))) != AFX_OK) return rc;
+    const DevEnv& de = dev_env();
+    const int waves = frames3_any_waves(pl->kp, pl->f3);
+    pl->f3_spec_grid = f3_grid((int)nblk, pl->n_cu, waves);
+    const int item = de.f3_item > 0 ? de.f3_item : f3_default_item(pl->kp);
+    const int S = de.no_tickets ? 0 : (de.f3_split >= 0 ? de.f3_split : f3_default_split(pl->kp, (int)nblk, pl->f3_spec_grid * waves, item));
+    const F3Split sp = f3_split((int)nblk, S, item, frames3_min_item(pl->kp));
+    pl->f3_sp = sp;
+    F3HeadTable tab;
+    f3_build_heads(sp, pl->f3_spec_grid, waves, tab.h);
+    const size_t nrec = (size_t)sp.nrecords();
+    if ((rc = ensure(pl->blocks_spec, nrec * sizeof(BlockDesc))) != AFX_OK) return rc;
+    if ((rc = ensure(pl->blockmax, nrec * sizeof(float))) != AFX_OK) return rc;
     if ((rc = ensure(pl->items, (size_t)n * kF3ItemsPerClip * sizeof(BlockDesc))) != AFX_OK) return rc;
-    if ((rc = ensure(pl->n_items, 16)) != AFX_OK) return rc;
-    if (!dev_env().host_blocks) {
-      HIP_TRY(launch_build_blocks3(s, (const ClipDesc*)pl->clips.p, n, (int)nblk, (BlockDesc*)pl->blocks_spec.p, pl->kp));
+    if ((rc = ensure(pl->n_items, kF3CounterInts * sizeof(int))) != AFX_OK) return rc;
+    if (!de.host_blocks) {
+      HIP_TRY(launch_build_blocks3(s, (const ClipDesc*)pl->clips.p, n, (BlockDesc*)pl->blocks_spec.p, pl->kp, sp, tab));
     } else {
-      const int per = pl->kp.rms_sub, half = pl->p.n_fft / 2;
-      pl->h_blocks.resize(nb_alloc);
+      pl->h_blocks.assign(nrec, BlockDesc{});
       for (int i = 0; i < n; ++i) {
         const ClipDesc& c = pl->h_clips[i];
-        const int64_t ntb = (c.len + th - 1) / th;
-        for (int b = 0; b < c.tpad / kFramesPerBlock; ++b) {
-          const int64_t gs = (int64_t)b * kFramesPerBlock * hop - half;
-          const int t0 = b * kFramesPerBlock;
-          pl->h_blocks[(size_t)c.blk_base + b] = make_block(c, i, gs, t0, 0, c.len, c.len, t0, c.tmax, c.len >= 2 && t0 < c.tmax,
-                                                            (int32_t)(c.tblk_base * per), (int32_t)(ntb * per));
-        }
+        for (int b = 0; b < c.tpad / kFramesPerBlock; ++b)
+          f3_spec_records(c, i, b, pl->p.n_fft, hop, th, pl->kp.rms_sub, sp, pl->h_blocks.data());
       }
+      std::memcpy(pl->h_blocks.data() + sp.nb, tab.h, sizeof(tab.h));
       HIP_TRY(hipMemcpyAsync(pl->blocks_spec.p, pl->h_blocks.data(), pl->h_blocks.size() * sizeof(BlockDesc), hipMemcpyHostToDevice, s));
       HIP_TRY(hipStreamSynchronize(s));
     }
@@ -540,12 +546,12 @@
 
   {
     const size_t before = pl->n_items.cap;
-    if ((rc = ensure(pl->n_items, 16)) != AFX_OK) return rc;
+    if ((rc = ensure(pl->n_items, kF3CounterInts * sizeof(int))) != AFX_OK) return rc;
     if (pl->n_items.cap != before) pl->info_clean_n = 0;
   }
   if (pl->info_clean_n < n) {
     HIP_TRY(hipMemsetAsync(d_info, 0, n * sizeof(ClipInfo), s));
-    HIP_TRY(hipMemsetAsync(pl->n_items.p, 0, 16, s));
+    HIP_TRY(hipMemsetAsync(pl->n_items.p, 0, kF3CounterInts * sizeof(int), s));
   }
   pl->info_clean_n = 0;
   const bool want_stamps = dev_env().stamps && !frames_mr_shape(kp.n_fft);
@@ -561,10 +567,11 @@
     F3Launch spec = f3l;
     spec.blocks = (const BlockDesc*)pl->blocks_spec.p; spec.nblocks = pl->nblocks; spec.spec = true;
     spec.blockmax = (float*)pl->blockmax.p; spec.bsum = (float*)pl->bsum.p;
-    spec.work_ctr = dev_env().no_tickets ? nullptr : (int*)pl->n_items.p + 1;
+    spec.work_ctr = dev_env().no_tickets ? nullptr : (int*)pl->n_items.p;
+    spec.grid = pl->f3_spec_grid;
     TIMED(AFX_K_FRAMES, launch_frames3_any(spec));
     TIMED(AFX_K_TRIM_DECIDE, launch_trim_decide3(s, d_clips, d_info, (const float*)pl->bsum.p, (const float*)pl->blockmax.p,
-                                                 (BlockDesc*)pl->items.p, (int*)pl->n_items.p, max_items, (float*)pl->rms.p, n, kp));
+                                                 (BlockDesc*)pl->items.p, (int*)pl->n_items.p, max_items, (float*)pl->rms.p, n, kp, pl->f3_sp));
     F3Launch redo = f3l;
     redo.blocks = (const BlockDesc*)pl->items.p; redo.nblocks = max_items; redo.nblocks_dev = (const int*)pl->n_items.p;
     TIMED(AFX_K_TRIM_BLOCKS, launch_frames3_any(redo));
@@ -650,7 +657,7 @@
       HIP_TRY(hipHostGetDevicePointer((void**)&pl->flag_dev, h, 0));
     }
   }
-  HIP_TRY(launch_finish(s, d_info, n, (int*)pl->n_items.p, by_event ? pl->flag_dev : nullptr, by_event ? ++pl->seq : 0u));
+  HIP_TRY(launch_finish(s, d_info, n, (int*)pl->n_items.p, kF3CounterInts, by_event ? pl->flag_dev : nullptr, by_event ? ++pl->seq : 0u));
   pl->info_clean_n = n;
   if (by_event) HIP_TRY(hipEventRecord(pl->done, s));
   pl->pend.active = true; pl->pend.n = n; pl->pend.stats_bytes = stats_bytes;
diff --git a/audio_feature_extraction_amd/csrc/afx_devenv.h b/audio_feature_extraction_amd/csrc/afx_devenv.h
--- a/audio_feature_extraction_amd/csrc/afx_devenv.h
+++ b/audio_feature_extraction_amd/csrc/afx_devenv.h
@@ -14,6 +14,8 @@
   int tail_mode = 0;
   int tail_skip = 0;
   int f3_waves = 0;
+  int f3_split = -1;
+  int f3_item = 0;
   int chunk_clips = 32768;
   int64_t f0_chunk_frames = 1280 * 1024;
   int64_t dtw_budget = (int64_t)2 << 30;
diff --git a/audio_feature_extraction_amd/csrc/afx_device.h b/audio_feature_extraction_amd/csrc/afx_device.h
--- a/audio_feature_extraction_amd/csrc/afx_device.h
+++ b/audio_feature_extraction_amd/csrc/afx_device.h
@@ -119,7 +119,7 @@
 hipError_t launch_dct(hipStream_t s, const ClipDesc* clips, const ClipInfo* info, const DevTables& tb,
                       const KParams& kp, const float* logmel, float* mfcc, int n_clips, int max_tmax,
                       bool frame_major = false, bool spec = false);
-hipError_t launch_finish(hipStream_t s, ClipInfo* info, int n_clips, int* counters, unsigned* flag_dev, unsigned seq);
+hipError_t launch_finish(hipStream_t s, ClipInfo* info, int n_clips, int* counters, int n_counters, unsigned* flag_dev, unsigned seq);
 hipError_t launch_stats(hipStream_t s, const ClipDesc* clips, const ClipInfo* info, const KParams& kp,
                         const float* mfcc, const float* rms_rows, float* stats, float* frames_out,
                         const int64_t* frame_offsets, int n_clips, ClipInfo* info_out = nullptr);
diff --git a/audio_feature_extraction_amd/csrc/afx_frames3.h b/audio_feature_extraction_amd/csrc/afx_frames3.h
--- a/audio_feature_extraction_amd/csrc/afx_frames3.h
+++ b/audio_feature_extraction_amd/csrc/afx_frames3.h
@@ -5,6 +5,7 @@
 #include <hip/hip_runtime_api.h>
 
 #include "afx_device.h"
+#include "afx_tickets.h"
 
 namespace afx {
 
@@ -57,10 +58,21 @@
   float* bsum = nullptr;
   bool spec = false;
   int* work_ctr = nullptr;
+  int grid = 0;
 };
-inline int f3_grid(const F3Launch& L, int waves) {
-  const int want = (L.nblocks + waves - 1) / waves;
-  return want < 1 ? 1 : (want < L.n_cu ? want : L.n_cu);
+inline int f3_grid(int nblocks, int n_cu, int waves) {
+  const int want = (nblocks + waves - 1) / waves;
+  return want < 1 ? 1 : (want < n_cu ? want : n_cu);
+}
+inline int f3_grid(const F3Launch& L, int waves) { return L.grid > 0 ? L.grid : f3_grid(L.nblocks, L.n_cu, waves); }
+int frames3_any_waves(const KParams& kp, const F3Tables& ft);
+inline int frames3_min_item(const KParams& kp) { return kp.n_fft == 512 ? 4 : 2; }
+inline int f3_default_item(const KParams&) { return 4; }
+inline int f3_default_eighths(const KParams&) { return 0; }
+inline int f3_default_split(const KParams& kp, int nblocks, int total_waves, int item) {
+  const int64_t want = (int64_t)total_waves * f3_default_eighths(kp) * item / (8 * 16);
+  const int64_t cap = nblocks / 4;
+  return (int)(want < cap ? want : cap);
 }
 size_t frames3s_lds_bytes(int waves, const F3Tables& ft);
 size_t frames3d_lds_bytes(int waves, const F3Tables& ft);
@@ -76,10 +88,26 @@
 hipError_t launch_spectral(hipStream_t s, const void* samples, ClipInfo* info, const BlockDesc* blocks, int nblocks,
                            const F3Tables& ft, const KParams& kp, float* desc_out, const int64_t* desc_offs,
                            const SpecBands& sb, int n_cu);
-hipError_t launch_build_blocks3(hipStream_t s, const ClipDesc* clips, int n_clips, int nblocks, BlockDesc* blocks,
-                                const KParams& kp);
+struct F3HeadTable { F3Head h[kF3Heads]; };
+__host__ __device__ inline void f3_spec_records(const ClipDesc& c, int clip, int b, int n_fft, int hop, int trim_hop, int per,
+                                                const F3Split& sp, BlockDesc* blocks) {
+  const int64_t ntb = (c.len + trim_hop - 1) / trim_hop;
+  const int32_t bsum_base = (int32_t)(c.tblk_base * per), bsum_n = (int32_t)(ntb * per);
+  const int t0 = b * kFramesPerBlock, B = c.blk_base + b;
+  const int64_t gs = (int64_t)t0 * hop - n_fft / 2;
+  blocks[B] = make_block(c, clip, gs, t0, 0, c.len, c.len, t0, c.tmax, c.len >= 2 && t0 < c.tmax, bsum_base, bsum_n);
+  if (B < sp.U) return;
+  for (int q = 0; q < sp.R; ++q) {
+    const int tq = t0 + sp.item * q, Tq = tq + sp.item < c.tmax ? tq + sp.item : c.tmax;
+    blocks[sp.qbase() + (B - sp.U) * sp.R + q] = make_block(c, clip, gs + (int64_t)sp.item * q * hop, tq, 0, c.len, c.len, tq, Tq,
+                                                            c.len >= 2 && tq < c.tmax, bsum_base, bsum_n);
+  }
+}
+hipError_t launch_build_blocks3(hipStream_t s, const ClipDesc* clips, int n_clips, BlockDesc* blocks, const KParams& kp,
+                                const F3Split& sp, const F3HeadTable& tab);
 constexpr int kF3ItemsPerClip = 6;
 hipError_t launch_trim_decide3(hipStream_t s, const ClipDesc* clips, ClipInfo* info, const float* bsum, const float* blockmax,
-                               BlockDesc* items, int* n_items, int max_items, float* rms_rows, int n_clips, const KParams& kp);
+                               BlockDesc* items, int* n_items, int max_items, float* rms_rows, int n_clips, const KParams& kp,
+                               const F3Split& sp);
 
 }
diff --git a/audio_feature_extraction_amd/csrc/afx_frames3.hip b/audio_feature_extraction_amd/csrc/afx_frames3.hip
--- a/audio_feature_extraction_amd/csrc/afx_frames3.hip
+++ b/audio_feature_extraction_amd/csrc/afx_frames3.hip
@@ -17,6 +17,7 @@
 #ifdef AFX_F3_DEBUG
 __device__ unsigned long long g_f3_stamps[4 * 8192];
 __device__ unsigned long long g_f3_blk[65536];
+__device__ unsigned long long g_f3_deq[4 * 8192];
 #endif
 
 template <int FMT, int WAVES, int NB0, int NB1, bool SPEC>
@@ -115,7 +116,11 @@
 #ifdef AFX_F3_DEBUG
   const unsigned long long stamp1 = wall_clock64();
 #endif
-  F3Runs runs = f3_runs_init(work_ctr, nblocks, total_waves, wg, true);
+  F3Runs runs = f3_runs_init(work_ctr, blocks, nblocks, total_waves, wg, true);
+#ifdef AFX_F3_DEBUG
+  unsigned long long deq_t0, deq_sum = 0, deq_n = 0, deq_last = 0, deq_final = 0;
+  bool deq_ok;
+#endif
   do {
   const int b_hi = runs.b_hi;
   for (int b = runs.b_lo; b < b_hi; ++b) {
@@ -389,12 +394,20 @@
     bd = blocks[b];
     }
   }
-  } while (f3_runs_next(runs, work_ctr, nblocks, (int)(gridDim.x * WAVES), lane));
+  #ifdef AFX_F3_DEBUG
+  deq_t0 = wall_clock64();
+  deq_ok = f3_runs_next(runs, work_ctr, blocks, nblocks, lane);
+  { const unsigned long long dt = wall_clock64() - deq_t0; deq_sum += dt; ++deq_n; if (deq_ok) deq_last = dt; else deq_final = dt; }
+  } while (deq_ok);
+#else
+  } while (f3_runs_next(runs, work_ctr, blocks, nblocks, lane));
+#endif
 #ifdef AFX_F3_DEBUG
   if (SPEC && lane == 0 && wg < 8192) {
     g_f3_stamps[4 * wg] = stamp0; g_f3_stamps[4 * wg + 1] = stamp1; g_f3_stamps[4 * wg + 2] = wall_clock64();
     g_f3_stamps[4 * wg + 3] = (unsigned long long)__builtin_amdgcn_s_getreg((31 << 11) | 4) |
                               ((unsigned long long)__builtin_amdgcn_s_getreg((31 << 11) | 20) << 32);
+    g_f3_deq[4 * wg] = deq_sum; g_f3_deq[4 * wg + 1] = deq_n; g_f3_deq[4 * wg + 2] = deq_last; g_f3_deq[4 * wg + 3] = deq_final;
   }
 #endif
 }
@@ -402,6 +415,9 @@
 #ifdef AFX_F3_DEBUG
 extern "C" __attribute__((visibility("default"))) int afx_debug_f3_stamps(unsigned long long* out, int n_waves) {
   return (int)hipMemcpyFromSymbol(out, HIP_SYMBOL(g_f3_stamps), sizeof(unsigned long long) * 4 * (size_t)n_waves);
+}
+extern "C" __attribute__((visibility("default"))) int afx_debug_f3_dequeue(unsigned long long* out, int n_waves) {
+  return (int)hipMemcpyFromSymbol(out, HIP_SYMBOL(g_f3_deq), sizeof(unsigned long long) * 4 * (size_t)n_waves);
 }
 extern "C" __attribute__((visibility("default"))) int afx_debug_f3_blocks(unsigned long long* out, int n_blocks) {
   return (int)hipMemcpyFromSymbol(out, HIP_SYMBOL(g_f3_blk), sizeof(unsigned long long) * (size_t)n_blocks);
@@ -429,6 +445,14 @@
   const int forced = dev_env().f3_waves;
   if (forced == 12 || forced == 16) return frames3_lds_bytes(forced, ft) <= 160 * 1024 ? forced : 12;
   return frames3_lds_bytes(16, ft) <= 160 * 1024 ? 16 : 12;
+}
+
+int frames3s_waves(const F3Tables& ft);
+int frames3d_waves(const F3Tables& ft);
+int frames3_any_waves(const KParams& kp, const F3Tables& ft) {
+  if (kp.n_fft == 2048) return frames3s_waves(ft);
+  if (kp.n_fft == 512) return frames3d_waves(ft);
+  return frames3_waves(ft);
 }
 
 template <int FMT, int WAVES, int NB0, int NB1, bool SPEC>
diff --git a/audio_feature_extraction_amd/csrc/afx_frames3_dev.h b/audio_feature_extraction_amd/csrc/afx_frames3_dev.h
--- a/audio_feature_extraction_amd/csrc/afx_frames3_dev.h
+++ b/audio_feature_extraction_amd/csrc/afx_frames3_dev.h
@@ -5,6 +5,7 @@
 
 #include "afx_device.h"
 #include "afx_frames3.h"
+#include "afx_tickets.h"
 #include "afx_wave.h"
 
 namespace afx {
@@ -152,13 +153,19 @@
 #endif
 struct F3Runs {
   int b_lo, b_hi, stride;
+  int h;
 };
-__device__ __forceinline__ F3Runs f3_runs_init(const int* work_ctr, int nblocks, int total_waves, int wg, bool contiguous) {
+__device__ __forceinline__ const F3Head* f3_heads(const BlockDesc* blocks, int nblocks) {
+  return reinterpret_cast<const F3Head*>(blocks + nblocks);
+}
+__device__ __forceinline__ F3Runs f3_runs_init(const int* work_ctr, const BlockDesc* blocks, int nblocks, int total_waves, int wg,
+                                               bool contiguous) {
   F3Runs r;
-  r.stride = 1;
+  r.stride = 1; r.h = 0;
   if (work_ctr) {
-    const int C0 = nblocks / (2 * total_waves);
+    const int C0 = f3_heads(blocks, nblocks)[0].C0;
     r.b_lo = wg * C0; r.b_hi = r.b_lo + C0;
+    r.h = 2 * (int)(blockIdx.x & (kF3Groups - 1));
   } else if (contiguous) {
     r.b_lo = (int)((long long)wg * nblocks / total_waves); r.b_hi = (int)((long long)(wg + 1) * nblocks / total_waves);
   } else {
@@ -166,20 +173,22 @@
   }
   return r;
 }
-__device__ __forceinline__ bool f3_runs_next(F3Runs& r, int* work_ctr, int nblocks, int total_waves, int lane) {
+__device__ __forceinline__ bool f3_runs_next(F3Runs& r, int* work_ctr, const BlockDesc* blocks, int nblocks, int lane) {
   if (!work_ctr) return false;
-  int t = 0;
-  if (lane == 0) t = atomicAdd(work_ctr, 1);
-  t = __builtin_amdgcn_readfirstlane(t);
-  const int C0 = nblocks / (2 * total_waves), dyn0 = total_waves * C0;
-  const int cA = C0 / 2 > 1 ? C0 / 2 : 1, cB = C0 / 3 > 1 ? C0 / 3 : 1;
-  int c = 1;
-  if (t < total_waves) { r.b_lo = dyn0 + cA * t; c = cA; }
-  else if (t < 2 * total_waves) { r.b_lo = dyn0 + cA * total_waves + cB * (t - total_waves); c = cB; }
-  else r.b_lo = dyn0 + (cA + cB) * total_waves + (t - 2 * total_waves);
-  if (r.b_lo >= nblocks) return false;
-  r.b_hi = r.b_lo + c < nblocks ? r.b_lo + c : nblocks;
-  return true;
+  for (;;) {
+    const int h = __builtin_amdgcn_readfirstlane(r.h);
+    int t = 0;
+    if (lane == 0) t = atomicAdd(work_ctr + kF3HeadStride * (1 + h), 1);
+    const F3Head e = f3_heads(blocks, nblocks)[h];
+    t = __builtin_amdgcn_readfirstlane(t);
+    if (f3_head_run(e, t, r.b_lo, r.b_hi)) return true;
+    unsigned m = 0;
+    if (lane == 0) m = atomicOr(reinterpret_cast<unsigned*>(work_ctr) + 1, 1u << h);
+    m = __builtin_amdgcn_readfirstlane(m) | (1u << h) | (unsigned)e.empty;
+    const int nh = f3_next_head(h, m);
+    if (nh < 0) return false;
+    r.h = nh;
+  }
 }
 
 __device__ __forceinline__ float f3_add_xor16(float v) {
diff --git a/audio_feature_extraction_amd/csrc/afx_frames3d.hip b/audio_feature_extraction_amd/csrc/afx_frames3d.hip
--- a/audio_feature_extraction_amd/csrc/afx_frames3d.hip
+++ b/audio_feature_extraction_amd/csrc/afx_frames3d.hip
@@ -98,7 +98,7 @@
   };
 
   const int total_waves = gridDim.x * WAVES;
-  F3Runs runs = f3_runs_init(work_ctr, nblocks, total_waves, blockIdx.x * WAVES + wave, false);
+  F3Runs runs = f3_runs_init(work_ctr, blocks, nblocks, total_waves, blockIdx.x * WAVES + wave, false);
   do {
   for (int b = runs.b_lo; b < runs.b_hi; b += runs.stride) {
     const BlockDesc bd = blocks[b];
@@ -287,7 +287,7 @@
       else { if (lane == 0 && mx > -INFINITY) atomicMax(&info[bd.clip].lmax_ord, f2ord(mx)); }
     }
   }
-  } while (f3_runs_next(runs, work_ctr, nblocks, (int)(gridDim.x * WAVES), lane));
+  } while (f3_runs_next(runs, work_ctr, blocks, nblocks, lane));
 }
 
 int frames3d_waves(const F3Tables& ft) {
diff --git a/audio_feature_extraction_amd/csrc/afx_frames3s.hip b/audio_feature_extraction_amd/csrc/afx_frames3s.hip
--- a/audio_feature_extraction_amd/csrc/afx_frames3s.hip
+++ b/audio_feature_extraction_amd/csrc/afx_frames3s.hip
@@ -102,7 +102,7 @@
   };
 
   const int total_waves = gridDim.x * WAVES;
-  F3Runs runs = f3_runs_init(work_ctr, nblocks, total_waves, blockIdx.x * WAVES + wave, false);
+  F3Runs runs = f3_runs_init(work_ctr, blocks, nblocks, total_waves, blockIdx.x * WAVES + wave, false);
   do {
   for (int b = runs.b_lo; b < runs.b_hi; b += runs.stride) {
     BlockDesc bd = blocks[b];
@@ -381,7 +381,7 @@
     bd = blocks[b];
     }
   }
-  } while (f3_runs_next(runs, work_ctr, nblocks, (int)(gridDim.x * WAVES), lane));
+  } while (f3_runs_next(runs, work_ctr, blocks, nblocks, lane));
 }
 
 int frames3s_waves(const F3Tables& ft) {
diff --git a/audio_feature_extraction_amd/csrc/afx_host.cpp b/audio_feature_extraction_amd/csrc/afx_host.cpp
--- a/audio_feature_extraction_amd/csrc/afx_host.cpp
+++ b/audio_feature_extraction_amd/csrc/afx_host.cpp
@@ -8,6 +8,7 @@
 #include "afx_f0.h"
 #include "afx_internal.h"
 #include "afx_mr.h"
+#include "afx_tickets.h"
 
 namespace afx {
 
@@ -143,6 +144,38 @@
   return AFX_OK;
 }
 
+extern "C" int afx_f3_tickets(int nblocks, int split, int item, int min_item, int grid, int waves, int32_t* geom, int32_t* heads) {
+  if (!geom || !heads) { set_error("afx_f3_tickets: null argument"); return AFX_ERR_INVALID; }
+  if (nblocks < 0 || nblocks > (1 << 30) || split < 0 || grid < 1 || grid > (1 << 20) || waves < 1 || waves > 16) {
+    set_error("afx_f3_tickets: blocks in [0, 2^30], split >= 0, grid in [1, 2^20] and waves in [1, 16] wanted");
+    return AFX_ERR_INVALID;
+  }
+  const F3Split sp = f3_split(nblocks, split, item, min_item);
+  F3Head h[kF3Heads];
+  f3_build_heads(sp, grid, waves, h);
+  const int32_t g[6] = {sp.nb, sp.U, sp.R, sp.item, sp.qbase(), sp.nrecords()};
+  std::memcpy(geom, g, sizeof(g));
+  std::memcpy(heads, h, sizeof(h));
+  return AFX_OK;
+}
+
+extern "C" int afx_f3_ticket_runs(const int32_t* head, int t0, int count, int32_t* out) {
+  if (!head || !out || t0 < 0 || count < 0) { set_error("afx_f3_ticket_runs: null/invalid argument"); return AFX_ERR_INVALID; }
+  F3Head e;
+  std::memcpy(&e, head, sizeof(e));
+  for (int i = 0; i < count; ++i) {
+    int lo = -1, hi = -1;
+    if (!f3_head_run(e, t0 + i, lo, hi)) lo = hi = -1;
+    out[2 * i] = lo; out[2 * i + 1] = hi;
+  }
+  return AFX_OK;
+}
+
+extern "C" int afx_f3_next_head(int head, uint32_t mask) {
+  if (head < 0 || head >= kF3Heads) return -2;
+  return f3_next_head(head, mask | (1u << head));
+}
+
 extern "C" int afx_chroma_filters(int sr, double tuning, float* out) {
   if (!out) { set_error("afx_chroma_filters: null argument"); return AFX_ERR_INVALID; }
   if (sr <= 0 || !std::isfinite(tuning)) { set_error("afx_chroma_filters: sr must be positive and tuning finite"); return AFX_ERR_INVALID; }
diff --git a/audio_feature_extraction_amd/csrc/afx_misc.hip b/audio_feature_extraction_amd/csrc/afx_misc.hip
--- a/audio_feature_extraction_amd/csrc/afx_misc.hip
+++ b/audio_feature_extraction_amd/csrc/afx_misc.hip
@@ -42,15 +42,16 @@
   }
 }
 
-__global__ __launch_bounds__(1024) void k_finish(uint4* info, int n_info16, int* counters, unsigned* flag, unsigned seq) {
+__global__ __launch_bounds__(1024) void k_finish(uint4* info, int n_info16, int* counters, int n_counters, unsigned* flag, unsigned seq) {
   for (int i = threadIdx.x; i < n_info16; i += 1024) info[i] = uint4{0u, 0u, 0u, 0u};
-  if (counters && threadIdx.x < 4) counters[threadIdx.x] = 0;
+  if (counters && (int)threadIdx.x < n_counters) counters[threadIdx.x] = 0;
   __syncthreads();
   if (flag && threadIdx.x == 0) __hip_atomic_store(flag, seq, __ATOMIC_RELEASE, __HIP_MEMORY_SCOPE_SYSTEM);
 }
-hipError_t launch_finish(hipStream_t s, ClipInfo* info, int n_clips, int* counters, unsigned* flag_dev, unsigned seq) {
+hipError_t launch_finish(hipStream_t s, ClipInfo* info, int n_clips, int* counters, int n_counters, unsigned* flag_dev, unsigned seq) {
+  if (n_counters > 1024) return hipErrorInvalidValue;
   static_assert(sizeof(ClipInfo) == 32, "k_finish clears ClipInfo as two 16-byte words");
-  hipLaunchKernelGGL(k_finish, dim3(1), dim3(1024), 0, s, (uint4*)info, n_clips * 2, counters, flag_dev, seq);
+  hipLaunchKernelGGL(k_finish, dim3(1), dim3(1024), 0, s, (uint4*)info, n_clips * 2, counters, n_counters, flag_dev, seq);
   return hipGetLastError();
 }
 
diff --git a/audio_feature_extraction_amd/csrc/afx_plan.h b/audio_feature_extraction_amd/csrc/afx_plan.h
--- a/audio_feature_extraction_amd/csrc/afx_plan.h
+++ b/audio_feature_extraction_amd/csrc/afx_plan.h
@@ -70,6 +70,8 @@
   std::vector<ClipDesc> h_clips;
   std::vector<int64_t> h_rebased;
   int nblocks = 0, max_tblocks = 0, max_tmax = 0;
+  F3Split f3_sp;
+  int f3_spec_grid = 0;
   int64_t total_tpad = 0, total_tblk = 0;
   void* h_pin = nullptr;
   void* h_pin_dev = nullptr;
diff --git a/audio_feature_extraction_amd/csrc/afx_tickets.h b/audio_feature_extraction_amd/csrc/afx_tickets.h
--- /dev/null
+++ b/audio_feature_extraction_amd/csrc/afx_tickets.h
@@ -0,0 +1,87 @@
+#pragma once
+#include <cstdint>
+
+#include <hip/hip_runtime_api.h>
+
+namespace afx {
+
+constexpr int kF3Groups = 8;
+constexpr int kF3Heads = 2 * kF3Groups;
+constexpr int kF3HeadStride = 32;
+constexpr int kF3CounterInts = kF3HeadStride * (1 + kF3Heads);
+
+struct F3Head {
+  int32_t lo, hi;
+  int32_t wv;
+  int32_t cA, cB;
+  int32_t C0;
+  int32_t n;
+  int32_t empty;
+};
+static_assert(sizeof(F3Head) == 32, "F3Head: two to a 64-byte list record");
+constexpr int kF3TabRecs = kF3Heads * (int)sizeof(F3Head) / 64;
+
+__host__ __device__ inline bool f3_head_run(const F3Head& e, int t, int& lo, int& hi) {
+  int c = 1, p;
+  if (t < e.wv) { p = e.lo + e.cA * t; c = e.cA; }
+  else if (t < 2 * e.wv) { p = e.lo + e.cA * e.wv + e.cB * (t - e.wv); c = e.cB; }
+  else p = e.lo + (e.cA + e.cB) * e.wv + (t - 2 * e.wv);
+  if (t >= e.n || p >= e.hi) return false;
+  lo = p; hi = p + c < e.hi ? p + c : e.hi;
+  return true;
+}
+
+struct F3Split {
+  int32_t nb = 0, U = 0, R = 1, item = 16;
+  __host__ __device__ int32_t qbase() const { return nb + kF3TabRecs; }
+  __host__ __device__ int32_t nrecords() const { return nb + kF3TabRecs + (nb - U) * R; }
+};
+inline F3Split f3_split(int nb, int S, int item, int min_item) {
+  F3Split sp;
+  sp.nb = nb; sp.U = nb;
+  if (item != 8 && item != 4 && item != 2) item = 4;
+  if (item < min_item) item = min_item;
+  if (S > nb) S = nb;
+  if (S > (1 << 24)) S = 1 << 24;
+  if (S > 0) { sp.U = nb - S; sp.R = 16 / item; sp.item = item; }
+  return sp;
+}
+
+inline void f3_build_heads(const F3Split& sp, int G, int W, F3Head out[kF3Heads]) {
+  if (G < 1) G = 1;
+  const int64_t TW = (int64_t)G * W;
+  const int C0 = (int)(sp.U / (2 * TW));
+  const int64_t dyn0 = TW * C0, D = sp.U - dyn0, Q = (int64_t)(sp.nb - sp.U) * sp.R;
+  auto cum = [&](int g) { return (int64_t)(G >> 3) * g + ((G & 7) < g ? (G & 7) : g); };
+  int32_t empty = 0;
+  for (int g = 0; g < kF3Groups; ++g) {
+    const int64_t c0 = cum(g), c1 = cum(g + 1);
+    F3Head& a = out[2 * g];
+    a.lo = (int32_t)(dyn0 + D * c0 / G); a.hi = (int32_t)(dyn0 + D * c1 / G);
+    a.wv = (int32_t)((c1 - c0) * W);
+    a.cA = C0 / 2 > 1 ? C0 / 2 : 1; a.cB = C0 / 3 > 1 ? C0 / 3 : 1;
+    F3Head& q = out[2 * g + 1];
+    q.lo = (int32_t)(sp.qbase() + Q * c0 / G); q.hi = (int32_t)(sp.qbase() + Q * c1 / G);
+    q.wv = 0; q.cA = q.cB = 1;
+    for (F3Head* e : {&a, &q}) {
+      const int64_t len = e->hi - e->lo, nA = e->wv, runA = (int64_t)e->cA * nA, runB = (int64_t)e->cB * nA;
+      int64_t n;
+      if (len <= runA) n = (len + e->cA - 1) / e->cA;
+      else if (len <= runA + runB) n = nA + (len - runA + e->cB - 1) / e->cB;
+      else n = 2 * nA + (len - runA - runB);
+      e->n = (int32_t)n; e->C0 = C0;
+      if (n == 0) empty |= 1 << (int)(e - out);
+    }
+  }
+  for (int h = 0; h < kF3Heads; ++h) out[h].empty = empty;
+}
+
+__host__ __device__ inline int f3_next_head(int h, uint32_t mask) {
+  const uint32_t live = ~mask & 0xFFFFu;
+  if (live == 0) return -1;
+  const int s = (h + 1) & 15;
+  const uint32_t rot = ((live >> s) | (live << (16 - s))) & 0xFFFFu;
+  return (s + __builtin_ctz(rot)) & 15;
+}
+
+}
diff --git a/audio_feature_extraction_amd/csrc/afx_trim3.hip b/audio_feature_extraction_amd/csrc/afx_trim3.hip
--- a/audio_feature_extraction_amd/csrc/afx_trim3.hip
+++ b/audio_feature_extraction_amd/csrc/afx_trim3.hip
@@ -10,7 +10,7 @@
 __global__ __launch_bounds__(256) void k_trim_decide3(const ClipDesc* __restrict__ clips, ClipInfo* __restrict__ info,
                                                       const float* __restrict__ bsum, const float* __restrict__ blockmax,
                                                       BlockDesc* __restrict__ items, int* __restrict__ n_items, int max_items,
-                                                      float* __restrict__ rms_rows, KParams kp) {
+                                                      float* __restrict__ rms_rows, KParams kp, F3Split sp) {
   __shared__ float red_f[4];
   __shared__ long long red_a[4], red_b[4];
   const int clip = blockIdx.x, tid = threadIdx.x, wave = tid >> 6, lane = tid & 63;
@@ -34,7 +34,13 @@
   const int bHi = cutR ? (glast >= 17 ? (glast - 17) >> 4 : -1) : nblk - 1;
   float cm = -INFINITY;
   if (status == AFX_CLIP_OK)
-    for (int b = bLo + tid; b <= bHi; b += 256) cm = fmaxf(cm, blockmax[cd.blk_base + b]);
+    for (int b = bLo + tid; b <= bHi; b += 256) {
+      const int B = cd.blk_base + b;
+      if (B < sp.U) cm = fmaxf(cm, blockmax[B]);
+      else
+        for (int q = 0; q < sp.R; ++q)
+          if (16 * b + sp.item * q < cd.tmax) cm = fmaxf(cm, blockmax[sp.qbase() + (B - sp.U) * sp.R + q]);
+    }
   cm = wave_max(cm);
   if (lane == 0) red_f[wave] = cm;
   __syncthreads();
@@ -71,32 +77,29 @@
 }
 
 __global__ __launch_bounds__(64) void k_build_blocks3(const ClipDesc* __restrict__ clips, int n_clips,
-                                                      BlockDesc* __restrict__ blocks, int n_fft, int hop, int trim_hop, int per) {
+                                                      BlockDesc* __restrict__ blocks, int n_fft, int hop, int trim_hop, int per,
+                                                      F3Split sp, F3HeadTable tab) {
   const int clip = blockIdx.x;
   if (clip >= n_clips) return;
   const ClipDesc c = clips[clip];
   const int nb = c.tpad / kFramesPerBlock;
-  const int64_t ntb = (c.len + trim_hop - 1) / trim_hop;
-  for (int b = threadIdx.x; b < nb; b += 64) {
-    const int64_t gs = (int64_t)b * kFramesPerBlock * hop - n_fft / 2;
-    const int t0 = b * kFramesPerBlock;
-    blocks[c.blk_base + b] = make_block(c, clip, gs, t0, 0, c.len, c.len, t0, c.tmax, c.len >= 2 && t0 < c.tmax,
-                                        (int32_t)(c.tblk_base * per), (int32_t)(ntb * per));
-  }
+  for (int b = threadIdx.x; b < nb; b += 64) f3_spec_records(c, clip, b, n_fft, hop, trim_hop, per, sp, blocks);
+  if (clip == 0 && threadIdx.x < kF3Heads) reinterpret_cast<F3Head*>(blocks + sp.nb)[threadIdx.x] = tab.h[threadIdx.x];
 }
 
-hipError_t launch_build_blocks3(hipStream_t s, const ClipDesc* clips, int n_clips, int nblocks, BlockDesc* blocks,
-                                const KParams& kp) {
-  if (nblocks <= 0 || n_clips <= 0) return hipSuccess;
+hipError_t launch_build_blocks3(hipStream_t s, const ClipDesc* clips, int n_clips, BlockDesc* blocks, const KParams& kp,
+                                const F3Split& sp, const F3HeadTable& tab) {
+  if (sp.nb <= 0 || n_clips <= 0) return hipSuccess;
   hipLaunchKernelGGL(k_build_blocks3, dim3(n_clips), dim3(64), 0, s, clips, n_clips, blocks,
-                     kp.n_fft, kp.hop, kp.trim_hop, kp.rms_sub);
+                     kp.n_fft, kp.hop, kp.trim_hop, kp.rms_sub, sp, tab);
   return hipGetLastError();
 }
 
 hipError_t launch_trim_decide3(hipStream_t s, const ClipDesc* clips, ClipInfo* info, const float* bsum, const float* blockmax,
-                               BlockDesc* items, int* n_items, int max_items, float* rms_rows, int n_clips, const KParams& kp) {
+                               BlockDesc* items, int* n_items, int max_items, float* rms_rows, int n_clips, const KParams& kp,
+                               const F3Split& sp) {
   hipLaunchKernelGGL(k_trim_decide3, dim3(n_clips), dim3(256), 0, s, clips, info, bsum, blockmax, items, n_items, max_items,
-                     rms_rows, kp);
+                     rms_rows, kp, sp);
   return hipGetLastError();
 }
 
diff --git a/audio_feature_extraction_amd/csrc/f3_tickets_check.cpp b/audio_feature_extraction_amd/csrc/f3_tickets_check.cpp
--- /dev/null
+++ b/audio_feature_extraction_amd/csrc/f3_tickets_check.cpp
@@ -0,0 +1,139 @@
+#include <cstdint>
+#include <cstdio>
+#include <cstdlib>
+#include <cstring>
+#include <vector>
+
+#include "afx_device.h"
+#include "afx_frames3.h"
+#include "afx_tickets.h"
+
+using namespace afx;
+
+namespace {
+
+int g_fail = 0;
+#define CHECK(cond)                                                              \
+  do {                                                                           \
+    if (!(cond)) { if (g_fail < 20) std::fprintf(stderr, "f3_tickets_check: line %d: %s\n", __LINE__, #cond); ++g_fail; } \
+  } while (0)
+
+uint32_t g_rng = 12345u;
+uint32_t rnd() { g_rng = g_rng * 1664525u + 1013904223u; return g_rng >> 8; }
+
+std::vector<ClipDesc> clips_of(const std::vector<int64_t>& lens, int hop, int trim_hop, int& nblocks) {
+  std::vector<ClipDesc> out(lens.size());
+  int64_t off = 0, fb = 0, tb = 0, nblk = 0;
+  for (size_t i = 0; i < lens.size(); ++i) {
+    ClipDesc& c = out[i];
+    c.off = off; c.len = lens[i];
+    c.tmax = (int32_t)(1 + lens[i] / hop);
+    c.tpad = (c.tmax + kFramesPerBlock - 1) / kFramesPerBlock * kFramesPerBlock;
+    c.frame_base = fb; c.tblk_base = tb; c.blk_base = (int32_t)nblk; c.pad_ = 0;
+    fb += c.tpad; tb += (lens[i] + trim_hop - 1) / trim_hop; nblk += c.tpad / kFramesPerBlock;
+    off += (lens[i] + 3) / 4 * 4;
+  }
+  nblocks = (int)nblk;
+  return out;
+}
+
+void walk(const BlockDesc& bd, const std::vector<ClipDesc>& clips, int step, std::vector<int>& frames, std::vector<int>& sums,
+          int64_t total_frames) {
+  if (!bd.active) return;
+  const ClipDesc& c = clips[(size_t)bd.clip];
+  CHECK(bd.t0 < bd.T && bd.T <= c.tmax);
+  CHECK(bd.frame_slot == c.frame_base + bd.t0);
+  const int n = bd.T - bd.t0 >= 16 ? 16 : bd.T - bd.t0;
+  for (int f = 0; f < n; ++f) {
+    const int64_t slot = bd.frame_slot + f;
+    CHECK(slot >= 0 && slot < total_frames);
+    if (slot >= 0 && slot < total_frames) ++frames[(size_t)slot];
+  }
+  const int covered = (n + step - 1) / step * step;
+  for (int j = bd.t0 == 0 ? 0 : bd.t0 + 1; j <= bd.t0 + covered; ++j)
+    if (j < bd.bsum_n) ++sums[(size_t)(bd.bsum_base + j)];
+}
+
+void one_case(const std::vector<int64_t>& lens, int n_fft, int hop, int trim_hop, int grid, int waves, int S, int item, int step) {
+  int nb = 0;
+  const std::vector<ClipDesc> clips = clips_of(lens, hop, trim_hop, nb);
+  const int per = trim_hop / hop;
+  const F3Split sp = f3_split(nb, S, item, step > 2 ? 4 : 2);
+  CHECK(sp.U >= 0 && sp.U <= nb && sp.nrecords() == nb + kF3TabRecs + (nb - sp.U) * sp.R);
+  std::vector<BlockDesc> list((size_t)sp.nrecords());
+  for (size_t i = 0; i < clips.size(); ++i)
+    for (int b = 0; b < clips[i].tpad / kFramesPerBlock; ++b)
+      f3_spec_records(clips[i], (int)i, b, n_fft, hop, trim_hop, per, sp, list.data());
+  F3Head heads[kF3Heads];
+  f3_build_heads(sp, grid, waves, heads);
+  std::memcpy(list.data() + nb, heads, sizeof(heads));
+
+  int64_t total_frames = 0, total_sums = 0;
+  for (const ClipDesc& c : clips) { total_frames += c.tpad; total_sums += (c.len + trim_hop - 1) / trim_hop * per; }
+  std::vector<int> frames((size_t)total_frames, 0), sums((size_t)total_sums, 0), taken(list.size(), 0);
+  auto take = [&](int lo, int hi) {
+    CHECK(lo >= 0 && lo < hi && hi <= (int)list.size());
+    for (int b = lo; b < hi && b < (int)list.size(); ++b) {
+      CHECK(b < sp.U || b >= sp.qbase());
+      ++taken[(size_t)b];
+      walk(list[(size_t)b], clips, step, frames, sums, total_frames);
+    }
+  };
+  const int C0 = heads[0].C0;
+  for (int w = 0; w < grid * waves; ++w)
+    if (C0 > 0) take(w * C0, w * C0 + C0);
+  struct Wave { int h, fruitless; bool alive; };
+  std::vector<Wave> wv;
+  for (int b = 0; b < grid && b < 24; ++b) wv.push_back(Wave{2 * (b & 7), 0, true});
+  int counters[kF3Heads] = {};
+  uint32_t mask = 0;
+  size_t alive = wv.size();
+  const bool one_draws_all = (rnd() & 3) == 0;
+  while (alive > 0) {
+    size_t k = one_draws_all ? 0 : rnd() % wv.size();
+    while (!wv[k].alive) k = (k + 1) % wv.size();
+    Wave& w = wv[k];
+    const int t = counters[w.h]++;
+    int lo, hi;
+    if (f3_head_run(heads[w.h], t, lo, hi)) { take(lo, hi); continue; }
+    ++w.fruitless;
+    CHECK(w.fruitless <= kF3Heads);
+    mask |= 1u << w.h;
+    const int nh = f3_next_head(w.h, mask | (uint32_t)heads[w.h].empty);
+    if (nh < 0 || w.fruitless > kF3Heads) { w.alive = false; --alive; } else w.h = nh;
+  }
+  for (int b = 0; b < (int)list.size(); ++b) CHECK(taken[(size_t)b] == ((b < sp.U || b >= sp.qbase()) ? 1 : 0));
+  for (const ClipDesc& c : clips) {
+    for (int f = 0; f < c.tpad; ++f) CHECK(frames[(size_t)(c.frame_base + f)] == ((c.len >= 2 && f < c.tmax) ? 1 : 0));
+    const int64_t ns = (c.len + trim_hop - 1) / trim_hop * per;
+    for (int64_t j = 0; j < ns; ++j) {
+      const int want = (c.len >= 2 && j <= (c.tmax + step - 1) / step * step) ? 1 : 0;
+      CHECK(sums[(size_t)(c.tblk_base * per + j)] == want);
+    }
+  }
+}
+
+}
+
+int main() {
+  struct Shape { int n_fft, hop, trim_hop, step; };
+  const Shape shapes[] = {{1024, 256, 512, 2}, {2048, 512, 512, 1}, {512, 128, 512, 4}};
+  int cases = 0;
+  for (const Shape& sh : shapes)
+    for (int n_clips : {1, 3, 40, 300})
+      for (int rep = 0; rep < 6; ++rep) {
+        std::vector<int64_t> lens;
+        for (int i = 0; i < n_clips; ++i) {
+          const uint32_t r = rnd() % 10;
+          const int64_t fr = r == 0 ? 0 : (r < 4 ? 1 + rnd() % 24 : 1 + rnd() % 200);
+          lens.push_back(r == 1 ? (int64_t)(rnd() % 3) : fr * sh.hop + rnd() % sh.hop);
+        }
+        const int grid = 1 + (int)(rnd() % (rep < 3 ? 20 : 300)), waves = (rnd() & 1) ? 12 : 16;
+        const int items[] = {8, 4, 2, 5};
+        const int Ss[] = {0, 1, 7, 1 << 20, (int)(rnd() % 64)};
+        for (int S : Ss) { one_case(lens, sh.n_fft, sh.hop, sh.trim_hop, grid, waves, S, items[rnd() % 4], sh.step); ++cases; }
+      }
+  if (g_fail) { std::fprintf(stderr, "f3_tickets_check: %d check(s) failed in %d cases\n", g_fail, cases); return 1; }
+  std::printf("f3_tickets_check: %d cases ok\n", cases);
+  return 0;
+}
diff --git a/include/afx.h b/include/afx.h
--- a/include/afx.h
+++ b/include/afx.h
@@ -154,6 +154,10 @@
 
 int afx_f0_dispatch(int sr, int n_fft, int hop, double fmin, double fmax, int32_t* out);
 
+int afx_f3_tickets(int nblocks, int split, int item, int min_item, int grid, int waves, int32_t* geom, int32_t* heads);
+int afx_f3_ticket_runs(const int32_t* head , int t0, int count, int32_t* out );
+int afx_f3_next_head(int head, uint32_t mask);
+
 int afx_wav_probe(const char* const* paths, int n, int threads, int32_t* info , int64_t* frames,
                   int64_t* data_off, int32_t* status);
 int afx_wav_read_s16(const char* const* paths, int n, int threads, const int64_t* data_off, const int64_t* frames,
```

Result: no change. 1.297 billion frames/s (median of 2 runs) (+0.3%).
